# heng-hw/SpaCap3D

Hardware: AMD Instinct MI355X
Metric: scenes/sec (40k pts, 256 proposals) fwd+bwd (higher is better)
Workload: dtype f32; 1 GPU; cfg2: synthetic ScanRefer-shaped scans, 40000 pts x (xyz+1 ch), 256 proposals, 8 scenes/GPU; full training step (SpaCapNet fwd + loss + bwd + grad all-reduce + Adam); global_batch=8, parallelism=dp1, hip_graph=True, fps_prefetch_side_stream=True, prefetch_as_graph=True, reserved_cus_forward=8, geometry_prefetch=True, deferred_weight_gradients=True, params=9290918, allreduce_bytes=35572416

## Files before the change

### include/spacap_hip.h

```cpp
#ifndef SPACAP_HIP_H
#define SPACAP_HIP_H

#include <stddef.h>
#include <stdint.h>

#ifdef __cplusplus
extern "C" {
#endif

#define SPACAP_ABI_VERSION 5

#define SPACAP_OK 0
#define SPACAP_E_INVALID (-1)
#define SPACAP_E_LAUNCH (-2)
#define SPACAP_E_NO_DEVICE (-3)

typedef void *spacap_stream_t;

int spacap_abi_version(void);
const char *spacap_last_error(void);
int spacap_device_count(void);

int spacap_opt_n_threads(int work_size);

// ... 5 lines not shown
int spacap_gather_points_f32(const float *points, const int32_t *idx, int B, int C, int N, int m,
                             float *out, spacap_stream_t stream);
int spacap_gather_points_grad_f32(const float *grad_out, const int32_t *idx, int B, int C, int N,
                                  int m, float *grad_points, spacap_stream_t stream);


int spacap_ball_query_f32(const float *new_xyz, const float *xyz, int B, int N, int m,
                          float radius, int nsample, int32_t *idx, spacap_stream_t stream);

size_t spacap_ball_query_grid_workspace_bytes(int B, int N);
int spacap_ball_query_grid_f32(const float *new_xyz, const float *xyz, int B, int N, int m, float radius, int nsample,
                               int32_t *idx, void *workspace, size_t workspace_bytes, spacap_stream_t stream);


int spacap_group_points_f32(const float *points, const int32_t *idx, int B, int C, int N, int P,
                            int S, float *out, spacap_stream_t stream);
size_t spacap_group_points_grad_workspace_bytes(int B, int C, int N, int P, int S);
int spacap_group_points_grad_f32(const float *grad_out, const int32_t *idx, int B, int C, int N,
                                 int P, int S, float *grad_points, void *workspace,
                                 spacap_stream_t stream);


int spacap_group_max_f32(const float *x, long rows, int S, float *out, uint8_t *arg,
                         spacap_stream_t stream);
int spacap_group_max_grad_f32(const float *grad_out, const uint8_t *arg, long rows, int S,
                              float *grad_in, spacap_stream_t stream);


int spacap_three_nn_f32(const float *unknown, const float *known, int B, int n, int m,
                        float *dist2, int32_t *idx, spacap_stream_t stream);
int spacap_three_nn_weights_f32(const float *unknown, const float *known, int B, int n, int m,
                                float *weight, int32_t *idx, spacap_stream_t stream);
int spacap_gather_xyz_f32(const float *xyz, const int32_t *idx, int B, int N, int m, float *out, spacap_stream_t stream);
int spacap_three_interpolate_f32(const float *points, const int32_t *idx, const float *weight,
                                 int B, int C, int m, int n, float *out, spacap_stream_t stream);
int spacap_three_interpolate_grad_f32(const float *grad_out, const int32_t *idx,
                                      const float *weight, int B, int C, int n, int m,
                                      float *grad_points, spacap_stream_t stream);
int spacap_three_interpolate_grad_pm_f32(const float *grad_pm, const int32_t *idx, const float *weight, int B, int C,
                                         int n, int m, float *grad_points_pm, spacap_stream_t stream);
int spacap_fp_concat_fwd_f32(const float *known, int known_pm, const int32_t *idx, const float *weight, const float *skip, int B,
                             int K1, int K2, int m, int n, float *out, spacap_stream_t stream);
int spacap_fp_concat_bwd_f32(const float *g, int B, int K1, int K2, int n, float *g1, float *g2, spacap_stream_t stream);


int spacap_mha_fwd_f32(const float *q, const float *k, const float *v, long q_sb, long q_sh,
                       long q_sl, long k_sb, long k_sh, long k_sl, long v_sb, long v_sh, long v_sl,
                       const uint8_t *mask, long mask_sb, long mask_sq, const float *bias,
                       long bias_sb, long bias_sh, long bias_sq, int B, int h, int Lq, int Lk,
                       int d_k, float scale, float dropout_p, uint64_t seed, const uint64_t *seed_dev,
                       float *out, float *p_out, float *stats, spacap_stream_t stream);

size_t spacap_mha_bwd_workspace_bytes(int B, int h, int Lq);
int spacap_mha_bwd_f32(const float *q, const float *k, const float *v, long q_sb, long q_sh,
                       long q_sl, long k_sb, long k_sh, long k_sl, long v_sb, long v_sh, long v_sl,
                       const uint8_t *mask, long mask_sb, long mask_sq, const float *bias,
                       long bias_sb, long bias_sh, long bias_sq, int B, int h, int Lq, int Lk,
                       int d_k, float scale, float dropout_p, uint64_t seed, const uint64_t *seed_dev,
                       const float *stats, const float *d_out, const float *d_p, void *workspace,
                       float *dq, float *dk, float *dv, long grad_row_stride, spacap_stream_t stream);

int spacap_mha_bwd_delta_f32(const float *q, const float *k, const float *v, long q_sb, long q_sh,
                             long q_sl, long k_sb, long k_sh, long k_sl, long v_sb, long v_sh, long v_sl,
                             const uint8_t *mask, long mask_sb, long mask_sq, const float *bias,
                             long bias_sb, long bias_sh, long bias_sq, int B, int h, int Lq, int Lk,
                             int d_k, float scale, float dropout_p, uint64_t seed, const uint64_t *seed_dev,
// ... 161 lines not shown
                               float *out, spacap_stream_t stream);

int spacap_scene_aug_doubles(void);
int spacap_scene_sample_augment_f32(const float *const *scene_feat, const int32_t *const *scene_ins,
                                    const uint8_t *const *scene_isobj, const float *const *scene_color,
                                    const int32_t *choices, const double *aug, int B, int P, int C, int augment,
                                    float *pc, int32_t *ins_out, uint8_t *isobj_out, float *color_out,
                                    spacap_stream_t stream);
int spacap_scene_sample_augment_map_f32(const float *const *scene_feat, const int32_t *const *scene_ins,
                                        const uint8_t *const *scene_isobj, const float *const *scene_color,
                                        const int32_t *choices, const double *aug, int B, int P, int C, int augment,
                                        int C_out, const int *dst_off, float *pc, int32_t *ins_out, uint8_t *isobj_out,
                                        float *color_out, spacap_stream_t stream);
int spacap_scene_gather_rows_f32(const float *const *src, const int32_t *choices, int B, int P, int W, float *out,
                                 int out_stride, int out_off, spacap_stream_t stream);
size_t spacap_scene_votes_workspace_bytes(int B, int max_inst);
int spacap_scene_votes_f32(const float *pc, const int32_t *ins, const uint8_t *isobj, int B, int P, int C,
                           int max_inst, void *workspace, float *votes, int64_t *vmask, spacap_stream_t stream);

int spacap_adam_flat_f32(float *p, const float *g, float *m, float *v, long n, float lr, float beta1, float beta2,
                         float eps, float weight_decay, const float *step, float grad_scale,
                         const int64_t *skip_if_nonzero, spacap_stream_t stream);

int spacap_det_npart(void);
int spacap_det_losses_fwd_f32(const float *net, const float *center, const float *agg_xyz, const float *gt_center,
                              const float *box_mask, const int64_t *heading_cls_label, const float *heading_res_label,
                              const int64_t *size_cls_label, const float *size_res_label, const int64_t *sem_cls_label,
                              const float *mean_size, const float *seed_xyz, const float *vote_xyz,
                              const int32_t *seed_inds, const float *vote_label, const int64_t *vote_mask, int B, int K,
                              int M, int NSEED, int N, int NH, int NS, int NC, float near_thr, float far_thr, float w0,
                              float w1, int64_t *obj_label, float *obj_mask, int64_t *assignment, float *dnet_num,
                              float *dcenter_num, float *dvote_num, float *part, float *losses, float *inv_den,
                              spacap_stream_t stream);
int spacap_det_losses_bwd_f32(const float *dnet_num, const float *dcenter_num, const float *dvote_num,
                              const float *grad_losses, const float *inv_den, int B, int K, int NSEED, int NH, int NS,
                              int NC, float *dnet, float *dcenter, float *dvote, spacap_stream_t stream);

long spacap_rel_loss_nparts(int B, int K);
int spacap_rel_loss_fwd_f32(const float *pred, const int64_t *assignment, const int64_t *box_mask_int,
                            const int64_t *obj_label, const int64_t *x_label, const int64_t *y_label,
                            const int64_t *z_label, int B, int K, int M, float *dnum, float *part, float *out,
                            spacap_stream_t stream);
int spacap_rel_loss_bwd_f32(const float *dnum, const float *grad_losses, const float *out, int B, int K, float *dpred,
                            spacap_stream_t stream);

int spacap_sum_slabs_f32(const float *part, int nslab, long n, float *out, spacap_stream_t stream);
int spacap_sum_slabs_batched_f32(const float *const *parts, float *const *outs, const long *n, const int *nslabs, int nseg,
                                 spacap_stream_t stream);

int spacap_linear_dgrad_mask_f32(const float *g, const float *W, const float *y, float scale, long R, int CK, int CP,
                                 float *dx, spacap_stream_t stream);

int spacap_rel_tail_fwd_f32(const float *hid1, const float *W2, const float *b2, const float *W3, const float *b3, long R,
                            float *hid2, float *pred, spacap_stream_t stream);
int spacap_rel_tail_bwd_nparts(long R);
int spacap_rel_tail_bwd_f32(const float *dpred, const float *W3, const float *hid2, long R, float *dz2, float *part,
                            spacap_stream_t stream);

int spacap_conv1x1_wgrad_slabs(int B, int CO, int CI, int N);
int spacap_conv1x1_wgrad_f32(const float *g, const float *x, int B, int CO, int CI, int N, float *part,
                             spacap_stream_t stream);
int spacap_conv1x1_wgrad_slabs_batched(int B, int CO, int CI, int N);
int spacap_conv1x1_wgrad_batched_f32(const float *const *g, const float *const *x, const int *B, const int *CO, const int *CI,
                                     const int *N, const int *nslabs, const int *with_bias, float *const *part, int njobs,
                                     spacap_stream_t stream);

// ... 15 lines not shown

int spacap_gemm_bf3_supported(int K, int N);
int spacap_gemm_bf3_split_w_f32(const float *W, long ldw, int N, int K, int trans, void *Wp, spacap_stream_t stream);
int spacap_gemm_bf3_f32(const float *A, long lda, const void *Wp, const float *bias, long R, int K, int N, int relu, float *out, long ldo,
                        spacap_stream_t stream);
int spacap_gemm_bf3_wgrad_slabs(long R, int N, int K);
int spacap_rel_wide_tail_supported(int C);
int spacap_rel_wide_tail_nparts(long R);
int spacap_rel_wide_tail_bwd_f32(const float *dpred, const float *W3, const float *hid2, long R, int C, int nparts, float *dz2, float *part,
                                 spacap_stream_t stream);
int spacap_rel_wide_l1_supported(int H, int K, int C);
int spacap_rel_wide_transpose_f32(const float *in, float *out, int B, int H, int K, int to_t, spacap_stream_t stream);
int spacap_rel_wide_l1_fwd_f32(const float *Pt, const float *U, const float *b1, int B, int H, int K, int C, float *hid1,
                               spacap_stream_t stream);
int spacap_rel_wide_l1_bwd_f32(const float *dh1, const float *hid1, const float *Pt, const float *U, int B, int H, int K, int C,
                               float *dPt, float *dU, float *db_part, spacap_stream_t stream);

int spacap_linear_rows_supported(long R, int K, int CO);
int spacap_linear_rows_f32(const float *a, const float *W, const float *bias, long R, int K, int CO, int trans_w,
                           float *out, spacap_stream_t stream);

int spacap_l2norm_rows_fwd_f32(const float *x, long rows, int D, float *y, float *inv_norm, spacap_stream_t stream);
int spacap_l2norm_rows_bwd_f32(const float *g, const float *y, const float *inv_norm, long rows, int D, float *dx,
                               spacap_stream_t stream);

int spacap_cap_loss_fwd_f32(const float *logits, const int64_t *target, const uint8_t *good, int B, int W, int V, int tstride,
                            float *logp, float *rowstat, float *out, spacap_stream_t stream);
int spacap_cap_loss_bwd_f32(const float *logp, const int64_t *target, const uint8_t *good, const float *out, const float *gloss,
                            int B, int W, int V, int tstride, float *dlogits, spacap_stream_t stream);

int spacap_proposal_decode_fwd_f32(const float *net, const float *agg_xyz, const float *mean_size, const double *mean_size_f64,
                                   int B, int K, int NH, int NS, int NC, float *nt, float *center, float *heading_res, float *size_res, double *corners,
                                   int64_t *bbox_mask, int64_t *sem_cls, int64_t *size_cls, spacap_stream_t stream);
int spacap_proposal_decode_bwd_f32(const float *g_nt, const float *g_center, const float *g_heading_res, const float *g_size_res,
                                   const float *mean_size, int B, int K, int NH, int NS, int NC, float *d_net, spacap_stream_t stream);

int spacap_loss_tail_fwd_f32(const float *det, const float *cap, const float *rel, const int64_t *obj_label, const float *obj_mask,
                             const int64_t *bbox_mask, int n, float *out, float *loss, spacap_stream_t stream);
int spacap_loss_tail_bwd_f32(const float *g_loss, float *g_det, float *g_cap, float *g_rel, spacap_stream_t stream);

typedef struct {
  int mode;
  long R;
  const float *a1;
  const float *w1;
  const float *bias1;
  int k1;
  float drop_p;
  float eps;
  uint64_t seed;
  const uint64_t *seed_dev;
  const float *res;
  float *x_out;
  const float *ln_a;
  const float *ln_b;
  float *n_out;
  float *stats;
  const float *x_ln;
  const float *g;
  float *part;
  const float *w2;
  const float *bias2;
  float *out2;
  int n2;
  int nparts;
  const float *attn_out;
// ... 8 lines not shown
                      float drop_p, uint64_t seed, const uint64_t *seed_dev, float *hid, float *part, spacap_stream_t stream);
long spacap_tf_ffn_pieces_elems(int dff);
int spacap_tf_ffn_split_f32(const float *const *w1, const float *const *w2, void *const *pieces, int nlayers, int dff,
                            spacap_stream_t stream);
int spacap_tf_ffn_bf3_f32(int mode, const float *x, const void *pieces, const float *bias, const float *y, long R, int dff, float drop_p,
                          uint64_t seed, const uint64_t *seed_dev, float *hid, float *part, spacap_stream_t stream);
int spacap_decode_attn_f32(const float *qkv, float *kcache, float *vcache, long R, int h, int d_k, int T, int t, float scale,
                           float *out, spacap_stream_t stream);
size_t spacap_decode_word_workspace_bytes(long R, int V);
int spacap_decode_word_f32(const float *x, const void *Wp, const float *bias, long R, int V, const float *lut, float scale,
                           const float *pe_row, int64_t *ys, int ys_ld, int t_out, float *x_next, void *workspace,
                           spacap_stream_t stream);
size_t spacap_beam_topw_workspace_bytes(long rows, int V, int W);
int spacap_beam_topw_f32(const float *x, const void *Wp, const float *bias, long rows, int V, int W, float *top_logp, int32_t *top_word,
                         void *workspace, spacap_stream_t stream);
int spacap_decode_attn_beam_f32(const float *qkv, float *kcache, float *vcache, const int8_t *anc, long R, int W, int h, int d_k, int T,
                                int t, float scale, float *out, spacap_stream_t stream);
int spacap_beam_step_f32(const float *top_logp, const int32_t *top_word, long R, int W, int V, int T, int t, int eos, const float *score_in,
                         const int32_t *fin_in, const int32_t *len_in, float *score_out, int32_t *fin_out, int32_t *len_out,
                         const int8_t *anc_old, int8_t *anc_new, int8_t *trace_parent, int32_t *trace_word, const float *lut, float scale,
                         const float *pe_row, float *x_next, spacap_stream_t stream);
int spacap_beam_finish_f32(const float *score, const int32_t *len, const int8_t *trace_parent, const int32_t *trace_word, long R, int W,
                           int n_words, double alpha, int64_t *ys, float *best_score, int64_t *all_tokens, float *all_scores,
                           int32_t *all_len, spacap_stream_t stream);
int spacap_tf_gemm_splits(long R, int K, int N);
int spacap_tf_gemm_f32(const float *a, const float *W, long R, int K, int N, int trans_w, int nsplit, float *out,
                       spacap_stream_t stream);
int spacap_tf_dgrad_mask_f32(const float *g, const float *W, const float *y, float scale, long R, int K, int N, float *out,
                             spacap_stream_t stream);

int spacap_conv1x1_cm_supported(int CI, int CO, long N);
int spacap_conv1x1_cm_f32(int mode, const float *W, const float *in, const float *bias, int B, int CI, int CO, long N,
                          float *out, spacap_stream_t stream);

int spacap_vote_assemble_fwd_f32(const float *net, const float *seed_xyz, const float *seed_feat, int B, int C, int N,
                                 float *vote_xyz, float *vote_feat, spacap_stream_t stream);
int spacap_vote_assemble_bwd_f32(const float *g_xyz, const float *g_feat, int B, int C, int N, float *d_net, float *d_seed,
                                 spacap_stream_t stream);

int spacap_copy_batched(const void *const *src, void *const *dst, const long *nbytes, int njobs, spacap_stream_t stream);

int spacap_stream_delay(int microseconds, spacap_stream_t stream);
int spacap_stream_wait_ge(const int64_t *flag, int64_t value, int timeout_ms, int64_t *err, spacap_stream_t stream);
int spacap_stream_signal(int64_t *flag, const int64_t *value, spacap_stream_t stream);

int spacap_lab_stamp(uint64_t *slot, spacap_stream_t stream);


size_t spacap_points_in_box_workspace_bytes(int B, int N, int K);
int spacap_points_in_box_f32(const float *point_clouds, int B, int N, int C, const double *bbox_corner, int K, void *workspace,
                             size_t workspace_bytes, spacap_stream_t stream);

#define SPACAP_PP_REMOVE_EMPTY 1
#define SPACAP_PP_CLS_NMS 2
#define SPACAP_PP_OLD_TYPE 4
#define SPACAP_PP_GT_F32 8

int spacap_detection_nms_f32(const float *objectness, const int64_t *sem_cls, const float *sem_cls_scores, int NC,
                             const double *bbox_corner, const void *workspace, int B, int N, int K, const double *gt_corner,
                             int M, const int64_t *object_assignment, int flags, int min_points, double nms_iou,
                             float conf_thresh, double min_iou, float *obj_prob, int32_t *count, uint8_t *nonempty,
                             uint8_t *pred_mask, float *conf, uint8_t *valid, double *iou, uint8_t *good,
                             spacap_stream_t stream);


#define SPACAP_AP_EXISTS 0x80

int spacap_detection_match_f32(const double *bbox_corner, const uint8_t *valid, const float *conf, const float *obj_prob,
                               const int64_t *sem_cls, int B, int K, int NC, const double *gt_corner,
                               const int64_t *sem_cls_label, const uint8_t *box_label_mask, int M, const double *thresholds,
                               int T, float *score, uint8_t *flags, int16_t *index, int32_t *npos, spacap_stream_t stream);

int spacap_ap_curve_f64(const uint8_t *flags, int64_t L, const int64_t *count, const int32_t *npos, int NC, int T, double *rec,
// ... 60 lines not shown
```

### spacap3d_amd/_native.py

```python
import ctypes
import os

import torch

_HERE = os.path.dirname(os.path.abspath(__file__))
LIB_PATH = os.path.join(_HERE, "lib", "libspacap_hip.so")
ABI_VERSION = 5

_i = ctypes.c_int
_l = ctypes.c_long
_f = ctypes.c_float
_p = ctypes.c_void_p
_u64 = ctypes.c_uint64

SIGNATURES = {
    "spacap_abi_version": (_i, []),
    "spacap_last_error": (ctypes.c_char_p, []),
    "spacap_device_count": (_i, []),
    "spacap_opt_n_threads": (_i, [_i]),
    "spacap_fps_workspace_bytes": (ctypes.c_size_t, [_i, _i]),
    "spacap_fps_f32": (_i, [_p, _i, _i, _i, _p, _p, _p]),
    "spacap_gather_points_f32": (_i, [_p, _p, _i, _i, _i, _i, _p, _p]),
    "spacap_gather_points_grad_f32": (_i, [_p, _p, _i, _i, _i, _i, _p, _p]),
    "spacap_ball_query_f32": (_i, [_p, _p, _i, _i, _i, _f, _i, _p, _p]),
    "spacap_ball_query_grid_workspace_bytes": (ctypes.c_size_t, [_i, _i]),
    "spacap_ball_query_grid_f32": (_i, [_p, _p, _i, _i, _i, _f, _i, _p, _p, ctypes.c_size_t, _p]),
    "spacap_group_points_f32": (_i, [_p, _p, _i, _i, _i, _i, _i, _p, _p]),
    "spacap_group_points_grad_workspace_bytes": (ctypes.c_size_t, [_i, _i, _i, _i, _i]),
    "spacap_group_points_grad_f32": (_i, [_p, _p, _i, _i, _i, _i, _i, _p, _p, _p]),
    "spacap_group_max_f32": (_i, [_p, _l, _i, _p, _p, _p]),
    "spacap_group_max_grad_f32": (_i, [_p, _p, _l, _i, _p, _p]),
    "spacap_three_nn_f32": (_i, [_p, _p, _i, _i, _i, _p, _p, _p]),
    "spacap_three_nn_weights_f32": (_i, [_p, _p, _i, _i, _i, _p, _p, _p]),
    "spacap_gather_xyz_f32": (_i, [_p, _p, _i, _i, _i, _p, _p]),
    "spacap_three_interpolate_f32": (_i, [_p, _p, _p, _i, _i, _i, _i, _p, _p]),
    "spacap_three_interpolate_grad_f32": (_i, [_p, _p, _p, _i, _i, _i, _i, _p, _p]),
    "spacap_three_interpolate_grad_pm_f32": (_i, [_p, _p, _p, _i, _i, _i, _i, _p, _p]),
    "spacap_bn_workspace_bytes": (ctypes.c_size_t, [_i]),
    "spacap_bn_set_single_launch": (_i, [_i]),
    "spacap_bn_stats_f32": (_i, [_p, _i, _i, _l, _f, _f, _p, _p, _p, _p, _p]),
    "spacap_bn_relu_apply_f32": (_i, [_p, _p, _p, _p, _i, _i, _l, _p, _p]),
    "spacap_bn_relu_train_f32": (_i, [_p, _i, _i, _l, _f, _f, _p, _p, _p, _p, _p, _p, _p, _p]),
    "spacap_bn_relu_max_f32": (_i, [_p, _p, _p, _p, _i, _i, _i, _i, _p, _p, _p]),
    "spacap_bn_relu_bwd_f32": (_i, [_p, _p, _p, _p, _p, _i, _i, _l, _p, _p, _p, _p, _p]),
    "spacap_bn_relu_max_bwd_f32": (_i, [_p, _p, _p, _p, _p, _p, _i, _i, _i, _i, _p, _p, _p, _p, _p]),
    "spacap_relation_feature_fwd_f32": (_i, [_p, _p, _l, _l, _l, _i, _i, _i, _i, _p, _p]),
    "spacap_relation_feature_bwd_f32": (_i, [_p, _p, _p, _l, _l, _l, _i, _i, _i, _i, _p, _p, _p]),
    "spacap_relation_l1_isplit": (_i, []),
    "spacap_relation_l1_supported": (_i, [_i, _i, _i]),
    "spacap_relation_l1_blocks": (_i, [_i, _i, _i]),
    "spacap_relation_l1_fwd_f32": (_i, [_p, _p, _p, _i, _i, _i, _i, _p, _p]),
    "spacap_relation_l1_bwd_f32": (_i, [_p, _p, _p, _p, _i, _i, _i, _i, _p, _p, _p, _p]),
    "spacap_relation_fused_supported": (_i, [_i, _i, _i, _i]),
    "spacap_relation_fused_leave_cus": (_i, [_i]),
    "spacap_relation_fused_zsplit": (_i, [_i, _i, _i]),
    "spacap_relation_fused_nparts": (_i, [_i, _i]),
    "spacap_relation_fused_part_floats": (_i, []),
    "spacap_relation_fused_fwd_f32": (_i, [_p] * 7 + [_i, _i, _p, _p, _p]),
    "spacap_relation_fused_bwd_f32": (_i, [_p] * 7 + [_i, _i, _i, _i, _p, _p, _p, _p]),
    "spacap_caption_prep_fwd_f32": (_i, [_p] * 7 + [_i] * 5 + [_f, _u64, _p] + [_p] * 7 + [_p]),
    "spacap_caption_prep_bwd_f32": (_i, [_p] * 3 + [_i] * 5 + [_f, _u64, _p, _p, _p, _p]),
    "spacap_conv1x1_cm_supported": (_i, [_i, _i, _l]),
    "spacap_conv1x1_cm_f32": (_i, [_i, _p, _p, _p, _i, _i, _i, _l, _p, _p]),
    "spacap_sa_l1_stats_f32": (_i, [_p, _p, _p, _p, _p, _i, _f, _i, _i, _i, _i, _i, _p, _p, _p]),
    "spacap_sa_l1_moments_f32": (_i, [_p, _p, _p, _p, _f, _i, _i, _i, _i, _p, _p, _p]),
    "spacap_sa_l1_moments_finalize_f32": (_i, [_p, _p, _i, _i, _i, _l, _f, _f, _p, _p, _p, _p, _p, _p]),
    "spacap_sa_mid_fwd_l1in_f32": (_i, [_p, _p, _i, _i, _p, _p, _l, _p, _p, _p]),
    "spacap_sa_wgrad_l1in_f32": (_i, [_p, _p, _p, _p, _p, _i, _i, _p, _l, _p, _p]),
    "spacap_sa_dgrad_l1in_f32": (_i, [_p, _p, _p, _p, _p, _p, _i, _i, _p, _i, _i, _i, _p, _p, _p]),
    "spacap_sa_dgrad_wgrad_l1in_slabs": (_i, [_l]),
    "spacap_sa_dgrad_wgrad_l1in_f32": (_i, [_p, _p, _p, _p, _p, _p, _i, _i, _p, _i, _i, _i, _p, _p, _p, _p]),
    "spacap_sa_l1_dw_f32": (_i, [_p, _i, _p, _i, _i, _p, _p]),
    "spacap_vote_assemble_fwd_f32": (_i, [_p, _p, _p, _i, _i, _i, _p, _p, _p]),
    "spacap_vote_assemble_bwd_f32": (_i, [_p, _p, _i, _i, _i, _p, _p, _p]),
    "spacap_copy_batched": (_i, [_p, _p, _p, _i, _p]),
    "spacap_lab_stamp": (_i, [_p, _p]),
    "spacap_points_in_box_workspace_bytes": (ctypes.c_size_t, [_i, _i, _i]),
    "spacap_points_in_box_f32": (_i, [_p, _i, _i, _i, _p, _i, _p, ctypes.c_size_t, _p]),
    "spacap_detection_nms_f32": (_i, [_p, _p, _p, _i, _p, _p, _i, _i, _i, _p, _i, _p, _i, _i, ctypes.c_double, _f,
                                      ctypes.c_double] + [_p] * 8 + [_p]),
    "spacap_detection_match_f32": (_i, [_p] * 5 + [_i, _i, _i] + [_p] * 3 + [_i, _p, _i] + [_p] * 4 + [_p]),
    "spacap_ap_curve_f64": (_i, [_p, ctypes.c_int64, _p, _p, _i, _i] + [_p] * 4 + [_p]),
    "spacap_caption_select_i32": (_i, [_p] * 6 + [_i] * 4 + [_p] + [_i] * 5 + [_p] * 4 + [_p]),
    "spacap_caption_score_f64": (_i, [_p, _p, _i, _p, ctypes.c_int64, _p, _p, ctypes.c_int64, _p, _p, _p, _p,
                                      ctypes.c_double, _p, _p, _p, _p]),
    "spacap_dense_caption_select": (_i, [_p] * 5 + [_i] * 5 + [_p] * 7 + [_p]),
    "spacap_multiview_workspace_bytes": (ctypes.c_size_t, [_i]),
    "spacap_multiview_map_f32": (_i, [_p, _i, _p, _p, _i, _i, _i] + [_f] * 7 + [_p, _p, ctypes.c_size_t, _p, _p]),
    "spacap_multiview_features_f32": (_i, [_p, _i, _p, _p, _i, _i, _i] + [_f] * 7 + [_p, _p, _i, _i, _p, ctypes.c_size_t, _p, _p]),
    "spacap_multiview_vote_i32": (_i, [_p, _i, _p, _p, _i, _i, _i] + [_f] * 7 + [_p, _p, _p, ctypes.c_size_t, _p, _p, _p]),
    "spacap_enet_param_floats": (ctypes.c_size_t, []),
    "spacap_enet_bottleneck_param_floats": (ctypes.c_size_t, [_i, _i, _i]),
    "spacap_enet_workspace_bytes": (ctypes.c_size_t, [_i, _i, _i]),
    "spacap_enet_initial_f32": (_i, [_p, _i, _i, _i, _p, _p, _p]),
    "spacap_enet_bottleneck_f32": (_i, [_p, _i, _i, _i, _i, _i, _i, _i, _p, _p, ctypes.c_size_t, _p, _p]),
    "spacap_enet_encode_f32": (_i, [_p, _i, _i, _i, _p, ctypes.c_size_t, _p, ctypes.c_size_t, _p, _p]),
    "spacap_enet_encode_u8": (_i, [_p, _i, _i, _i] + [_f] * 6 + [_p, ctypes.c_size_t, _p, ctypes.c_size_t, _p, _p]),
    "spacap_stream_delay": (_i, [_i, _p]),
    "spacap_stream_wait_ge": (_i, [_p, _l, _i, _p, _p]),
    "spacap_stream_signal": (_i, [_p, _p, _p]),
    "spacap_sa_nparts": (_i, []),
    "spacap_sa_wgrad_slabs": (_i, [_l, _i, _i, _i]),
    "spacap_sa_mlp_supported": (_i, [_i, _i, _i]),
    "spacap_sa_l1_fwd_f32": (_i, [_p, _p, _p, _p, _p, _p, _i, _f, _i, _i, _i, _i, _i, _p, _p, _p]),
    "spacap_sa_bn_finalize_f32": (_i, [_p, _i, _l, _f, _f, _p, _p, _p, _p, _p, _p]),
    "spacap_sa_mid_fwd_f32": (_i, [_p, _p, _p, _l, _i, _i, _p, _p, _p]),
    "spacap_sa_pool_fwd_f32": (_i, [_p, _p, _l, _i, _i, _p, _p, _p]),
    "spacap_gemm_rows_supported": (_i, [_i, _i]),
# ... 26 lines not shown
    "spacap_rel_wide_l1_bwd_f32": (_i, [_p, _p, _p, _p, _i, _i, _i, _i, _p, _p, _p, _p]),
    "spacap_sa_l3bwd_part_floats": (_l, [_i, _i]),
    "spacap_sa_l3bwd_dw_f32": (_i, [_p, _i, _p, _p, _i, _i, _p, _p, _p]),
    "spacap_sa_wgrad_pool_supported": (_i, [_i, _i, _i]),
    "spacap_sa_wgrad_pool_parts": (_i, [_l, _i, _i, _i]),
    "spacap_sa_wgrad_pool_f32": (_i, [_p, _p, _i, _p, _p, _p, _l, _i, _i, _p, _p]),
    "spacap_sa_bwd_finalize_f32": (_i, [_p, _i, _l, _p, _p, _p, _p, _p]),
    "spacap_sa_dgrad_f32": (_i, [_p, _p, _i, _p, _p, _p, _p, _p, _l, _i, _i, _p, _p, _p]),
    "spacap_sa_dgrad_l1_f32": (_i, [_p] * 10 + [_f] + [_i] * 6 + [_p, _p, _p]),
    "spacap_sa_wgrad_f32": (_i, [_p, _p, _i, _p, _p, _p, _p, _l, _i, _i, _p, _p]),
    "spacap_sa_l1_bwd_f32": (_i, [_p, _p, _p, _p, _p, _p, _p, _p, _i, _f, _i, _i, _i, _i, _i, _p, _p, _i, _p]),
    "spacap_sa_rows_scatter_workspace_bytes": (ctypes.c_size_t, [_i, _i, _l]),
    "spacap_sa_rows_scatter_f32": (_i, [_p, _p, _i, _i, _l, _i, _p, _p, _p]),
    "spacap_sa_rows_index_f32": (_i, [_p, _i, _i, _l, _p, _p]),
    "spacap_sa_rows_gather_f32": (_i, [_p, _i, _i, _l, _i, _p, _p, _p]),
    "spacap_sa_drel_sums_f32": (_i, [_p, _i, _i, _i, _i, _p, _p, _p, _p]),
    "spacap_sa_dw1_assemble_f32": (_i, [_p, _i, _p, _i, _i, _i, _p, _p]),
    "spacap_relu_dropout_fwd_f32": (_i, [_p, _l, _f, _u64, _p, _p, _p]),
    "spacap_relu_dropout_bwd_f32": (_i, [_p, _p, _l, _f, _p, _p]),
    "spacap_dropout_add_fwd_f32": (_i, [_p, _p, _l, _f, _u64, _p, _p, _p]),
    "spacap_dropout_add_bwd_f32": (_i, [_p, _l, _f, _u64, _p, _p, _p]),
    "spacap_scene_aug_doubles": (_i, []),
    "spacap_scene_sample_augment_f32": (_i, [_p, _p, _p, _p, _p, _p, _i, _i, _i, _i, _p, _p, _p, _p, _p]),
    "spacap_scene_sample_augment_map_f32": (_i, [_p, _p, _p, _p, _p, _p, _i, _i, _i, _i, _i, _p, _p, _p, _p, _p, _p]),
    "spacap_scene_gather_rows_f32": (_i, [_p, _p, _i, _i, _i, _p, _i, _i, _p]),
    "spacap_l2norm_rows_fwd_f32": (_i, [_p, _l, _i, _p, _p, _p]),
    "spacap_l2norm_rows_bwd_f32": (_i, [_p, _p, _p, _l, _i, _p, _p]),
    "spacap_cap_loss_fwd_f32": (_i, [_p, _p, _p, _i, _i, _i, _i, _p, _p, _p, _p]),
    "spacap_cap_loss_bwd_f32": (_i, [_p, _p, _p, _p, _p, _i, _i, _i, _i, _p, _p]),
    "spacap_scene_votes_workspace_bytes": (ctypes.c_size_t, [_i, _i]),
    "spacap_scene_votes_f32": (_i, [_p, _p, _p, _i, _i, _i, _i, _p, _p, _p, _p]),
    "spacap_det_npart": (_i, []),
    "spacap_det_losses_fwd_f32": (_i, [_p] * 16 + [_i] * 8 + [_f] * 4 + [_p] * 9 + [_p]),
    "spacap_det_losses_bwd_f32": (_i, [_p] * 5 + [_i] * 6 + [_p] * 3 + [_p]),
    "spacap_rel_loss_nparts": (_l, [_i, _i]),
    "spacap_rel_loss_fwd_f32": (_i, [_p] * 7 + [_i] * 3 + [_p] * 3 + [_p]),
    "spacap_rel_loss_bwd_f32": (_i, [_p] * 3 + [_i] * 2 + [_p, _p]),
    "spacap_sum_slabs_f32": (_i, [_p, _i, _l, _p, _p]),
    "spacap_sum_slabs_batched_f32": (_i, [_p, _p, _p, _p, _i, _p]),
    "spacap_adam_flat_f32": (_i, [_p, _p, _p, _p, _l, _f, _f, _f, _f, _f, _p, _f, _p, _p]),
    "spacap_linear_dgrad_mask_f32": (_i, [_p, _p, _p, _f, _l, _i, _i, _p, _p]),
    "spacap_rel_tail_fwd_f32": (_i, [_p, _p, _p, _p, _p, _l, _p, _p, _p]),
    "spacap_rel_tail_bwd_nparts": (_i, [_l]),
    "spacap_rel_tail_bwd_f32": (_i, [_p, _p, _p, _l, _p, _p, _p]),
    "spacap_conv1x1_wgrad_slabs": (_i, [_i, _i, _i, _i]),
    "spacap_conv1x1_wgrad_f32": (_i, [_p, _p, _i, _i, _i, _i, _p, _p]),
    "spacap_conv1x1_wgrad_slabs_batched": (_i, [_i, _i, _i, _i]),
    "spacap_conv1x1_wgrad_batched_f32": (_i, [_p, _p, _p, _p, _p, _p, _p, _p, _p, _i, _p]),
    "spacap_linear_rows_supported": (_i, [_l, _i, _i]),
    "spacap_linear_rows_f32": (_i, [_p, _p, _p, _l, _i, _i, _i, _p, _p]),
    "spacap_linear_wgrad_slabs": (_i, [_l, _i, _i]),
    "spacap_linear_wgrad_f32": (_i, [_p, _p, _l, _i, _i, _i, _p, _p]),
    "spacap_linear_wgrad_nslab_f32": (_i, [_p, _p, _l, _i, _i, _i, _i, _p, _p]),
    "spacap_linear_wgrad_slabs_batched": (_i, [_l, _i, _i]),
    "spacap_linear_wgrad_batched_f32": (_i, [_p, _p, _p, _p, _p, _p, _p, _p, _i, _p]),
    "spacap_layernorm_fwd_f32": (_i, [_p, _p, _p, _l, _i, _f, _p, _p, _p]),
    "spacap_layernorm_bwd_workspace_bytes": (ctypes.c_size_t, [_l, _i]),
    "spacap_layernorm_bwd_f32": (_i, [_p, _p, _p, _p, _l, _i, _f, _p, _p, _p, _p, _p]),
    "spacap_layernorm_bwd_add_f32": (_i, [_p, _p, _p, _p, _p, _l, _i, _f, _p, _p, _p, _p, _p]),
    "spacap_proposal_decode_fwd_f32": (_i, [_p, _p, _p, _p, _i, _i, _i, _i, _i, _p, _p, _p, _p, _p, _p, _p, _p, _p]),
    "spacap_proposal_decode_bwd_f32": (_i, [_p, _p, _p, _p, _p, _i, _i, _i, _i, _i, _p, _p]),
    "spacap_loss_tail_fwd_f32": (_i, [_p, _p, _p, _p, _p, _p, _i, _p, _p, _p]),
    "spacap_loss_tail_bwd_f32": (_i, [_p, _p, _p, _p, _p]),
    "spacap_tf_rows_f32": (_i, [_p, _p]),
    "spacap_tf_rows_parts": (_i, [_l]),
    "spacap_tf_ffn1_f32": (_i, [_p, _p, _p, _l, _i, _f, _u64, _p, _p, _p]),
    "spacap_tf_ffn_f32": (_i, [_i, _p, _p, _p, _p, _p, _l, _i, _f, _u64, _p, _p, _p, _p]),
    "spacap_tf_ffn_pieces_elems": (_l, [_i]),
    "spacap_tf_ffn_split_f32": (_i, [_p, _p, _p, _i, _i, _p]),
    "spacap_tf_ffn_bf3_f32": (_i, [_i, _p, _p, _p, _p, _l, _i, _f, _u64, _p, _p, _p, _p]),
    "spacap_decode_attn_f32": (_i, [_p, _p, _p, _l, _i, _i, _i, _i, _f, _p, _p]),
    "spacap_decode_word_workspace_bytes": (ctypes.c_size_t, [_l, _i]),
    "spacap_decode_word_f32": (_i, [_p, _p, _p, _l, _i, _p, _f, _p, _p, _i, _i, _p, _p, _p]),
    "spacap_beam_topw_workspace_bytes": (ctypes.c_size_t, [_l, _i, _i]),
    "spacap_beam_topw_f32": (_i, [_p, _p, _p, _l, _i, _i, _p, _p, _p, _p]),
    "spacap_decode_attn_beam_f32": (_i, [_p, _p, _p, _p, _l, _i, _i, _i, _i, _i, _f, _p, _p]),
    "spacap_beam_step_f32": (_i, [_p, _p, _l, _i, _i, _i, _i, _i] + [_p] * 6 + [_p] * 4 + [_p, _f, _p, _p, _p]),
    "spacap_beam_finish_f32": (_i, [_p, _p, _p, _p, _l, _i, _i, ctypes.c_double, _p, _p, _p, _p, _p, _p]),
    "spacap_tf_gemm_splits": (_i, [_l, _i, _i]),
    "spacap_tf_gemm_f32": (_i, [_p, _p, _l, _i, _i, _i, _i, _p, _p]),
    "spacap_tf_dgrad_mask_f32": (_i, [_p, _p, _p, _f, _l, _i, _i, _p, _p]),
    "spacap_mha_fwd_f32": (_i, [_p, _p, _p] + [_l] * 9 + [_p, _l, _l, _p, _l, _l, _l]
                           + [_i] * 5 + [_f, _f, _u64, _p, _p, _p, _p, _p]),
    "spacap_mha_bwd_workspace_bytes": (ctypes.c_size_t, [_i, _i, _i]),
    "spacap_mha_bwd_delta_f32": (_i, [_p, _p, _p] + [_l] * 9 + [_p, _l, _l, _p, _l, _l, _l]
                                 + [_i] * 5 + [_f, _f, _u64, _p, _p, _p, _p, _p, _p, _p, _l, _p]),
    "spacap_mha_bwd_f32": (_i, [_p, _p, _p] + [_l] * 9 + [_p, _l, _l, _p, _l, _l, _l]
                           + [_i] * 5 + [_f, _f, _u64, _p, _p, _p, _p, _p, _p, _p, _p, _l, _p]),
}


class TfRowsArgs(ctypes.Structure):
    _fields_ = [("mode", _i), ("R", _l), ("a1", _p), ("w1", _p), ("bias1", _p), ("k1", _i), ("drop_p", _f), ("eps", _f),
                ("seed", _u64), ("seed_dev", _p), ("res", _p), ("x_out", _p), ("ln_a", _p), ("ln_b", _p), ("n_out", _p),
                ("stats", _p), ("x_ln", _p), ("g", _p), ("part", _p), ("w2", _p), ("bias2", _p), ("out2", _p), ("n2", _i), ("nparts", _i), ("attn_out", _p), ("delta_out", _p), ("lq", _i)]


def _load():
    if not os.path.exists(LIB_PATH):
        raise ImportError(
            f"{LIB_PATH} not found: the HIP extension is not built. Run "
            "`python -c 'import __graft_entry__ as g; g.build()'` (or `make -C spacap3d_amd/csrc`). "
            "spacap3d_amd has no CPU or PyTorch fallback for its native operators.")
    lib = ctypes.CDLL(LIB_PATH)
    for name, (res, args) in SIGNATURES.items():
        fn = getattr(lib, name)
        fn.restype = res
        fn.argtypes = args
    got = lib.spacap_abi_version()
    if got != ABI_VERSION:
        raise ImportError(f"libspacap_hip.so ABI {got} != expected {ABI_VERSION}: rebuild the extension")
    return lib


lib = _load()


def check(rc: int, what: str) -> None:
    if rc != 0:
        msg = lib.spacap_last_error().decode("utf-8", "replace")
        raise RuntimeError(f"{what} failed (code {rc}): {msg}")


_DEFERRED = None


class deferred_slab_sums:

# ... 151 lines not shown

def conv1x1_wgrad_partials(g, x, B, CO, CI, N, deferrable=False, with_bias=False):
    import torch
    with torch.cuda.device(g.device):
        if deferrable and _DEFERRED is not None:
            nb = int(lib.spacap_conv1x1_wgrad_slabs_batched(B, CO, CI, N))
            part = torch.empty(nb, CO * CI + (((CO + 3) // 4) * 4 if with_bias else 0), dtype=torch.float32, device=g.device)
            _DEFERRED.conv_jobs.append((g, x, (B, CO, CI, N), part, bool(with_bias)))
            return part
        nslab = int(lib.spacap_conv1x1_wgrad_slabs(B, CO, CI, N))
        part = torch.empty(nslab, CO * CI, dtype=torch.float32, device=g.device)
        check(lib.spacap_conv1x1_wgrad_f32(g.data_ptr(), x.data_ptr(), B, CO, CI, N, part.data_ptr(),
                                           torch.cuda.current_stream(g.device).cuda_stream), "spacap_conv1x1_wgrad_f32")
    return part


def copy_batched(dsts, srcs):
    import torch
    ok = len(dsts) == len(srcs) and len(dsts) > 0 and all(
        d.is_cuda and s.is_cuda and d.device == s.device and d.dtype == s.dtype and d.shape == s.shape and d.is_contiguous()
        and s.is_contiguous() for d, s in zip(dsts, srcs))
    if not ok:
        if dsts:
            torch._foreach_copy_(list(dsts), list(srcs), non_blocking=True)
        return
    n = len(dsts)
    PA, LA = ctypes.c_void_p * n, ctypes.c_long * n
    src = PA(*[s.data_ptr() for s in srcs])
    dst = PA(*[d.data_ptr() for d in dsts])
    nb = LA(*[d.numel() * d.element_size() for d in dsts])
    dev = dsts[0].device
    with torch.cuda.device(dev):
        check(lib.spacap_copy_batched(src, dst, nb, n, torch.cuda.current_stream(dev).cuda_stream), "spacap_copy_batched")
```

### spacap3d_amd/attention.py

```python
import math

import torch
from torch.autograd import Function

from ._native import check, lib, sum_slabs


def _strides3(t):
    assert t.stride(3) == 1, "last (d_k) dimension must be contiguous"
    return t.stride(0), t.stride(1), t.stride(2)


def _prep_mask(mask, B, Lq, Lk):
    if mask is None:
        return None, 0, 0
    for ent in _MASK_CACHE:
        if ent[0] is mask and ent[1] == (mask._version, B, Lq, Lk):
            return ent[2]
    res = _prep_mask_uncached(mask, B, Lq, Lk)
    _MASK_CACHE.insert(0, (mask, (mask._version, B, Lq, Lk), res))
    del _MASK_CACHE[4:]
    return res


_MASK_CACHE = []


def _prep_mask_uncached(mask, B, Lq, Lk):
    m = mask
    if m.dim() == 4:
        assert m.size(1) == 1, "per-head masks are not used by the reference"
        m = m[:, 0]
    assert m.dim() == 3 and m.size(-1) == Lk and m.size(1) in (1, Lq)
    if m.dtype == torch.uint8 and m.size(0) == B and m.is_contiguous():
        return m, m.stride(0), (0 if m.size(1) == 1 else m.stride(1))
    m = (m != 0).to(torch.uint8)
    if m.size(0) != B:
        m = m.expand(B, -1, -1)
    m = m.contiguous()
    return m, m.stride(0), (0 if m.size(1) == 1 else m.stride(1))


_RNG_STATE = {}
_CALL_COUNTER = [None]


def rng_state(device):
    device = torch.device(device)
    if device.type == "cuda" and device.index is None:
        device = torch.device("cuda", torch.cuda.current_device())
    st = _RNG_STATE.get(device)
    if st is None:
        st = torch.zeros(1, dtype=torch.int64, device=device)
        _RNG_STATE[device] = st
    return st


def advance_rng(device):
    rng_state(device).add_(1)


def _next_seed():
# ... 321 lines not shown
```

### spacap3d_amd/backend.py

```python
import contextlib

_current = None


class HipBackend:

    name = "hip"

    def __init__(self):
        from . import ext
        from . import attention as _att
        self._ext = ext
        for n in ("gather_points", "gather_points_grad", "furthest_point_sampling", "three_nn",
                  "three_interpolate", "three_interpolate_grad", "ball_query", "group_points",
                  "group_points_grad", "group_max", "group_max_grad", "three_interpolate_grad_pm"):
            setattr(self, n, getattr(ext, n))
        self.attention = _att.attention
        self.self_attention_packed = _att.self_attention_packed
        self.layer_norm = _att.layer_norm
        self.layer_norm_residual = _att.layer_norm_residual
        self.relation_feature = _att.relation_feature
        self.relation_layer1 = _att.relation_layer1
        from . import fused_bn as _fbn
        self.bn_relu_train = _fbn.bn_relu_train
        self.bn_relu_eval = _fbn.bn_relu_eval
        from . import fused_losses as _fl
        self.detection_losses = _fl.detection_losses
        self.relation_losses = _fl.relation_losses
        self.caption_head_loss = _fl.caption_head_loss
        self.loss_tail = _fl.loss_tail
        self.proposal_decode = _fl.proposal_decode
        self.l2norm_rows = _fl.l2norm_rows
        self.vote_assemble = _fl.vote_assemble
        from . import fused_dropout as _fd
        self.relu_dropout = _fd.relu_dropout
        self.dropout_add = _fd.dropout_add
        from . import linear as _lin
        self.linear = _lin.linear
        self.ffn_tail = _lin.ffn_tail
        self.conv1x1 = _lin.conv1x1
        self.relation_tail = _lin.relation_tail
        self.relation_head = _lin.relation_head
        self.vocab_projection = _lin.vocab_projection
        from . import caption_prep as _cp
        self.caption_prep = _cp.caption_prep
        from . import tf_layer as _tf
        self.tf_stack = _tf
        from . import caption_decode as _cd
        self.caption_decode = _cd
        from . import sa_mlp as _sa
        self.sa_mlp_train = _sa.sa_mlp_train
        self.sa_mlp_eval = _sa.sa_mlp_eval


def ops():
    global _current
    if _current is None:
        _current = HipBackend()
    return _current


def set_backend(b):
    global _current
    prev = _current
    _current = b
    return prev


@contextlib.contextmanager
def use_backend(b):
    prev = set_backend(b)
    try:
        yield b
# ... 3 lines not shown
```

### spacap3d_amd/csrc/conv1x1.hip

```cpp
#include <stdlib.h>

#include "common.hpp"
#include "launch.hpp"
#include "mfma.hpp"

namespace {

using namespace spacap::mfma;

constexpr int TM = 64, TN = 64, KC = 32, LDN = TN + 4, LDW = TM + 4;

template <bool TRANS_A>
__global__ __launch_bounds__(256) void conv1x1_cm_kernel(const float *__restrict__ W, int lda, const float *__restrict__ in,
                                                         const float *__restrict__ bias, int M, int K, int N,
                                                         float *__restrict__ out) {
  __shared__ __attribute__((aligned(16))) float s_in[2][KC * LDN];
  __shared__ __attribute__((aligned(16))) float s_w[TRANS_A ? 2 * KC * LDW : 4];
  const int tid = threadIdx.x, lane = tid & 63, w = tid >> 6, l15 = lane & 15, lg = lane >> 4;
  const int n0 = blockIdx.x * TN, m0 = blockIdx.y * TM, b = blockIdx.z;
  const float *inb = in + (size_t)b * K * N;
  const int sr = tid >> 4, sc = (tid & 15) * 4;
  f32x4 pin[2], pw[2];
  auto request = [&](int k0) {
#pragma unroll
    for (int e = 0; e < 2; ++e) {
      const int k = k0 + sr + 16 * e;
      const f32x4 v = ld4(inb + (size_t)min(k, K - 1) * N + n0 + sc);
      pin[e] = k < K ? v : f32x4{0.f, 0.f, 0.f, 0.f};
      if (TRANS_A) {
        const float *p = W + (size_t)min(k, K - 1) * lda;
        f32x4 t;
        if (m0 + sc + 3 < M && (lda & 3) == 0) {
          t = ld4(p + m0 + sc);
        } else {
#pragma unroll
          for (int u = 0; u < 4; ++u) t[u] = p[min(m0 + sc + u, M - 1)];
        }
#pragma unroll
        for (int u = 0; u < 4; ++u) t[u] = (k < K && m0 + sc + u < M) ? t[u] : 0.f;
        pw[e] = t;
      }
    }
  };
  auto store = [&](int buf) {
#pragma unroll
    for (int e = 0; e < 2; ++e) {
      st4(&s_in[buf][(sr + 16 * e) * LDN + sc], pin[e]);
      if (TRANS_A) st4(&s_w[buf * KC * LDW + (sr + 16 * e) * LDW + sc], pw[e]);
// ... 6 lines not shown
  const int nchunks = (K + KC - 1) / KC;
  request(0);
  for (int c = 0; c < nchunks; ++c) {
    const int buf = c & 1, k0 = c * KC;
    store(buf);
    f32x4 a0, a1;
    if (!TRANS_A) {
      const float *p = W + (size_t)mrow * lda + k0 + 8 * lg;
      if (k0 + KC <= K && (lda & 3) == 0) {
        a0 = ld4(p), a1 = ld4(p + 4);
      } else {
#pragma unroll
        for (int u = 0; u < 4; ++u) {
          a0[u] = k0 + 8 * lg + u < K ? p[u] : 0.f;
          a1[u] = k0 + 8 * lg + 4 + u < K ? p[4 + u] : 0.f;
        }
      }
    }
    if (c + 1 < nchunks) request(k0 + KC);
    __syncthreads();
    const float *si = &s_in[buf][(8 * lg) * LDN + l15];
    if (TRANS_A) {
      const float *sw = &s_w[buf * KC * LDW + (8 * lg) * LDW + 16 * w + l15];
#pragma unroll
      for (int u = 0; u < 4; ++u) a0[u] = sw[u * LDW], a1[u] = sw[(4 + u) * LDW];
    }
#pragma unroll
    for (int s = 0; s < 8; ++s) {
      const float av = s < 4 ? a0[s] : a1[s - 4];
#pragma unroll
      for (int t = 0; t < 4; ++t) acc[t] = MFMA16(av, si[s * LDN + 16 * t], acc[t]);
    }
  }
#pragma unroll
  for (int u = 0; u < 4; ++u) {
    const int m = m0 + 16 * w + 4 * lg + u;
    if (m < M) {
      const float bv = bias ? bias[m] : 0.f;
      float *o = out + ((size_t)b * M + m) * N + n0 + l15;
#pragma unroll
      for (int t = 0; t < 4; ++t) o[16 * t] = acc[t][u] + bv;
    }
  }
}


constexpr int BLD = TN + 8;
constexpr int BIMG = KC * BLD;


template <bool TRANS_A>
__global__ __launch_bounds__(256) void conv1x1_cm_bf3_kernel(const float *__restrict__ W, int lda, const float *__restrict__ in,
                                                             const float *__restrict__ bias, int M, int K, int N,
                                                             float *__restrict__ out) {
  __shared__ __attribute__((aligned(16))) __bf16 s_b[2][3 * BIMG];
  __shared__ __attribute__((aligned(16))) __bf16 s_a[TRANS_A ? 2 * 3 * BIMG : 8];
  const int tid = threadIdx.x, lane = tid & 63, w = tid >> 6, l15 = lane & 15, lg = lane >> 4;
  const int n0 = blockIdx.x * TN, m0 = blockIdx.y * TM, b = blockIdx.z;
  const float *inb = in + (size_t)b * K * N;
  const int sr = tid >> 4, sc = (tid & 15) * 4;
  f32x4 pin[2], pw[2];
  auto request = [&](int k0) {
#pragma unroll
    for (int e = 0; e < 2; ++e) {
      const int k = k0 + sr + 16 * e;
      const f32x4 v = ld4(inb + (size_t)min(k, K - 1) * N + n0 + sc);
      pin[e] = k < K ? v : f32x4{0.f, 0.f, 0.f, 0.f};
      if (TRANS_A) {
        const float *p = W + (size_t)min(k, K - 1) * lda;
        f32x4 t;
        if (m0 + sc + 3 < M && (lda & 3) == 0) {
          t = ld4(p + m0 + sc);
        } else {
#pragma unroll
          for (int u = 0; u < 4; ++u) t[u] = p[min(m0 + sc + u, M - 1)];
        }
#pragma unroll
        for (int u = 0; u < 4; ++u) t[u] = (k < K && m0 + sc + u < M) ? t[u] : 0.f;
        pw[e] = t;
      }
    }
  };
  auto store = [&](int buf) {
#pragma unroll
    for (int e = 0; e < 2; ++e) {
      const int o = (sr + 16 * e) * BLD + sc;
      bf16x4 p0, p1, p2;
// ... 29 lines not shown
    }
  };
  request(0);
  wrequest(0);
  for (int c = 0; c < nchunks; ++c) {
    const int buf = c & 1, k0 = c * KC;
    store(buf);
    bf16x8 a[3];
    if (!TRANS_A) {
      bf16x4 l0, l1, l2, h0, h1, h2;
      split4(na0, l0, l1, l2);
      split4(na1, h0, h1, h2);
      a[0] = bf16x8{l0[0], l0[1], l0[2], l0[3], h0[0], h0[1], h0[2], h0[3]};
      a[1] = bf16x8{l1[0], l1[1], l1[2], l1[3], h1[0], h1[1], h1[2], h1[3]};
      a[2] = bf16x8{l2[0], l2[1], l2[2], l2[3], h2[0], h2[1], h2[2], h2[3]};
    }
    if (c + 1 < nchunks) {
      request(k0 + KC);
      wrequest(k0 + KC);
    }
    __syncthreads();
    if (TRANS_A) {
#pragma unroll
      for (int q = 0; q < 3; ++q) a[q] = tr_frag<BLD>(&s_a[buf * 3 * BIMG + q * BIMG], 16 * w, lane);
    }
#pragma unroll
    for (int t = 0; t < 4; ++t) {
      bf16x8 bq[3];
#pragma unroll
      for (int q = 0; q < 3; ++q) bq[q] = tr_frag<BLD>(&s_b[buf][q * BIMG], 16 * t, lane);
#pragma unroll
      for (int q = 0; q < 6; ++q) acc[t] = MFMA_B(a[PA[q]], bq[PB[q]], acc[t]);
    }
  }
#pragma unroll
  for (int u = 0; u < 4; ++u) {
    const int m = m0 + 16 * w + 4 * lg + u;
    if (m < M) {
      const float bv = bias ? bias[m] : 0.f;
      float *o = out + ((size_t)b * M + m) * N + n0 + l15;
#pragma unroll
      for (int t = 0; t < 4; ++t) o[16 * t] = acc[t][u] + bv;
    }
  }
}

}

extern "C" int spacap_conv1x1_cm_supported(int CI, int CO, long N) { return CI >= 1 && CO >= 1 && N >= 64 && N % 64 == 0; }

extern "C" int spacap_conv1x1_cm_f32(int mode, const float *W, const float *in, const float *bias, int B, int CI, int CO, long N,
                                     float *out, spacap_stream_t stream) {
  const char *what = "spacap_conv1x1_cm_f32";
  SPACAP_REQUIRE((mode == 0 || mode == 1 || mode == 2) && B >= 0 && spacap_conv1x1_cm_supported(CI, CO, N) && N <= 2147483647L && B <= 65535,
                 "%s: (mode=%d, B=%d, CI=%d, CO=%d, N=%ld) unsupported", what, mode, B, CI, CO, N);
  if (B == 0) return SPACAP_OK;
  SPACAP_REQUIRE(W && in && out && spacap::aligned16(in, out),
                 "%s: null or unaligned pointer", what);
  const bool f32fwd = mode == 2;
  if (f32fwd) mode = 0;
  const int M = mode == 0 ? CO : CI, K = mode == 0 ? CI : CO;
  const dim3 grid((unsigned)(N / TN), (unsigned)((M + TM - 1) / TM), (unsigned)B);
  hipStream_t s = spacap::as_stream(stream);
  if (mode == 0 && !f32fwd && !spacap::sa_f32_mfma_only())
    hipLaunchKernelGGL(conv1x1_cm_bf3_kernel<false>, grid, dim3(256), 0, s, W, CI, in, bias, M, K, (int)N, out);
  else if (mode == 0) hipLaunchKernelGGL(conv1x1_cm_kernel<false>, grid, dim3(256), 0, s, W, CI, in, bias, M, K, (int)N, out);
  else hipLaunchKernelGGL(conv1x1_cm_kernel<true>, grid, dim3(256), 0, s, W, CI, in, (const float *)nullptr, M, K, (int)N, out);
  SPACAP_CHECK_LAUNCH(what);
  return SPACAP_OK;
}
```

### spacap3d_amd/csrc/elementwise.hip

```cpp
#include "common.hpp"
#include "dropout.hpp"
#include "mfma.hpp"

namespace {

using namespace spacap;
using spacap::mfma::f32x4;

template <int MODE>
__global__ __launch_bounds__(256) void drop_kernel(const float *__restrict__ x, const float *__restrict__ res, long n,
                                                   unsigned thresh, float scale, unsigned long long seed,
                                                   const unsigned long long *__restrict__ seed_dev, float *__restrict__ out) {
  const DropSeed sd = make_seed(seed, seed_dev);
  const long n4 = n >> 2;
  for (long i = (long)blockIdx.x * 256 + threadIdx.x; i < n4; i += (long)gridDim.x * 256) {
    f32x4 v = *reinterpret_cast<const f32x4 *>(x + 4 * i);
    f32x4 r = {0.f, 0.f, 0.f, 0.f};
    if (MODE == 1) r = *reinterpret_cast<const f32x4 *>(res + 4 * i);
#pragma unroll
    for (int u = 0; u < 4; ++u) {
      const bool keep = thresh == 0u || hash32((unsigned long long)(4 * i + u), sd) >= thresh;
      float a = MODE == 0 ? fmaxf(v[u], 0.f) : v[u];
      a = keep ? a * scale : 0.f;
      v[u] = MODE == 1 ? r[u] + a : a;
// ... 300 lines not shown
  if (J.vec) {
    for (long o = beg + 16 * threadIdx.x; o < end; o += 16 * 256)
      *reinterpret_cast<f32x4 *>(J.dst + o) = *reinterpret_cast<const f32x4 *>(J.src + o);
  } else {
    for (long o = beg + threadIdx.x; o < end; o += 256) J.dst[o] = J.src[o];
  }
}
}
extern "C" int spacap_copy_batched(const void *const *src, void *const *dst, const long *nbytes, int njobs, spacap_stream_t stream) {
  const char *what = "spacap_copy_batched";
  SPACAP_REQUIRE(njobs >= 0 && (njobs == 0 || (src && dst && nbytes)), "%s: bad arguments", what);
  hipStream_t s = spacap::as_stream(stream);
  int i = 0;
  while (i < njobs) {
    CopyTable T;
    T.njobs = 0, T.pad = 0;
    long blocks = 0;
    for (; i < njobs && T.njobs < CPJ_MAX; ++i) {
      SPACAP_REQUIRE(nbytes[i] >= 0 && (nbytes[i] == 0 || (src[i] && dst[i])), "%s: job %d: null pointer or negative size", what, i);
      if (nbytes[i] == 0) continue;
      CopyJob &J = T.job[T.njobs++];
      J.src = static_cast<const char *>(src[i]), J.dst = static_cast<char *>(dst[i]), J.nbytes = nbytes[i], J.block0 = (int)blocks;
      J.vec = ((reinterpret_cast<uintptr_t>(src[i]) | reinterpret_cast<uintptr_t>(dst[i]) | (uintptr_t)nbytes[i]) & 15) == 0;
      blocks += (nbytes[i] + CPJ_BLOCK_BYTES - 1) / CPJ_BLOCK_BYTES;
      SPACAP_REQUIRE(blocks < 2147483647L, "%s: too many blocks", what);
    }
    if (T.njobs) hipLaunchKernelGGL(copy_batched_kernel, dim3((unsigned)blocks), dim3(256), 0, s, T);
  }
  SPACAP_CHECK_LAUNCH(what);
  return SPACAP_OK;
}

namespace {
__global__ void delay_kernel(unsigned long long ticks) {
  const unsigned long long t0 = wall_clock64();
  while (wall_clock64() - t0 < ticks) __builtin_amdgcn_s_sleep(8);
}
}
extern "C" int spacap_stream_delay(int microseconds, spacap_stream_t stream) {
  SPACAP_REQUIRE(microseconds >= 0 && microseconds <= 100000, "spacap_stream_delay: %d us out of range", microseconds);
  if (microseconds == 0) return SPACAP_OK;
  hipLaunchKernelGGL(delay_kernel, dim3(1), dim3(1), 0, spacap::as_stream(stream), (unsigned long long)microseconds * 100ull);
  SPACAP_CHECK_LAUNCH("spacap_stream_delay");
  return SPACAP_OK;
}

namespace {
__global__ void wait_ge_kernel(const long long *flag, long long value, unsigned long long ticks, unsigned long long *err) {
  const unsigned long long t0 = wall_clock64();
  while (__hip_atomic_load(flag, __ATOMIC_ACQUIRE, __HIP_MEMORY_SCOPE_AGENT) < value) {
    if (wall_clock64() - t0 > ticks) {
      atomicCAS(err, 0ull, (unsigned long long)(value > 0 ? value : 1));
      __threadfence_system();
      return;
    }
    __builtin_amdgcn_s_sleep(16);
  }
}
__global__ void signal_set_kernel(long long *flag, const long long *value) {
  __hip_atomic_store(flag, *value, __ATOMIC_RELEASE, __HIP_MEMORY_SCOPE_AGENT);
}
}
extern "C" int spacap_stream_wait_ge(const int64_t *flag, int64_t value, int timeout_ms, int64_t *err, spacap_stream_t stream) {
  SPACAP_REQUIRE(flag && err && timeout_ms >= 1 && timeout_ms <= 600000, "spacap_stream_wait_ge: bad arguments");
  hipLaunchKernelGGL(wait_ge_kernel, dim3(1), dim3(1), 0, spacap::as_stream(stream), reinterpret_cast<const long long *>(flag),
                     (long long)value, (unsigned long long)timeout_ms * 100000ull, reinterpret_cast<unsigned long long *>(err));
// ... 21 lines not shown
```

### spacap3d_amd/csrc/interpolate.hip

```cpp
#include <math.h>

#include "common.hpp"

#pragma clang fp contract(off)

namespace {

template <bool WEIGHTS>
__global__ __launch_bounds__(64) void three_nn_kernel(const float *__restrict__ unknown_all,
                                                      const float *__restrict__ known_all, int n, int m,
                                                      float *__restrict__ dist2_all,
                                                      int32_t *__restrict__ idx_all) {
  constexpr int KT = 512;
  __shared__ float s_k[KT * 3];
  const int b = blockIdx.y;
  const int j = blockIdx.x * 64 + threadIdx.x;
  const float *__restrict__ known = known_all + (size_t)b * m * 3;
  const int jj = j < n ? j : n - 1;
  const float *__restrict__ u = unknown_all + ((size_t)b * n + jj) * 3;
  const float ux = u[0], uy = u[1], uz = u[2];
  float best1 = INFINITY, best2 = INFINITY, best3 = INFINITY;
  int besti1 = 0, besti2 = 0, besti3 = 0;
  for (int k0 = 0; k0 < m; k0 += KT) {
    const int kn = min(KT, m - k0);
// ... 7 lines not shown
      const int kk = k0 + k;
      const bool l1 = d < best1, l2 = d < best2, l3 = d < best3;
      best3 = l2 ? best2 : (l3 ? d : best3);
      besti3 = l2 ? besti2 : (l3 ? kk : besti3);
      best2 = l1 ? best1 : (l2 ? d : best2);
      besti2 = l1 ? besti1 : (l2 ? kk : besti2);
      best1 = l1 ? d : best1;
      besti1 = l1 ? kk : besti1;
    }
  }
  if (j < n) {
    float *__restrict__ dd = dist2_all + ((size_t)b * n + j) * 3;
    int32_t *__restrict__ ii = idx_all + ((size_t)b * n + j) * 3;
    if (WEIGHTS) {
      const float r1 = 1.0f / (sqrtf(best1) + 1e-8f), r2 = 1.0f / (sqrtf(best2) + 1e-8f), r3 = 1.0f / (sqrtf(best3) + 1e-8f);
      const float norm = (r1 + r3) + r2;
      dd[0] = r1 / norm; dd[1] = r2 / norm; dd[2] = r3 / norm;
    } else {
      dd[0] = best1; dd[1] = best2; dd[2] = best3;
    }
    ii[0] = besti1; ii[1] = besti2; ii[2] = besti3;
  }
}

__global__ __launch_bounds__(256) void gather_xyz_kernel(const float *__restrict__ xyz, const int32_t *__restrict__ idx, int N, int m,
                                                         long total, float *__restrict__ out) {
  const long i = (long)blockIdx.x * 256 + threadIdx.x;
  if (i >= total) return;
  const long b = i / m;
  const float *p = xyz + ((size_t)b * N + idx[i]) * 3;
  out[i * 3 + 0] = p[0], out[i * 3 + 1] = p[1], out[i * 3 + 2] = p[2];
}

constexpr int CHUNK = 8;

__global__ __launch_bounds__(256) void three_interpolate_kernel(const float *__restrict__ points,
                                                                const int32_t *__restrict__ idx,
                                                                const float *__restrict__ weight, int C,
                                                                int m, int n, float *__restrict__ out) {
  const int b = blockIdx.z;
  const int j = blockIdx.x * 256 + threadIdx.x;
  if (j >= n) return;
  const size_t r = ((size_t)b * n + j) * 3;
  const float w1 = weight[r + 0], w2 = weight[r + 1], w3 = weight[r + 2];
  const int i1 = idx[r + 0], i2 = idx[r + 1], i3 = idx[r + 2];
  const int c0 = blockIdx.y * CHUNK, c1 = min(c0 + CHUNK, C);
  const float *__restrict__ p = points + ((size_t)b * C + c0) * m;
  float *__restrict__ o = out + ((size_t)b * C + c0) * n + j;
  for (int c = c0; c < c1; ++c, p += m, o += n) *o = p[i1] * w1 + p[i2] * w2 + p[i3] * w3;
}

__global__ __launch_bounds__(256) void three_interpolate_grad_kernel(const float *__restrict__ grad_out,
                                                                     const int32_t *__restrict__ idx,
                                                                     const float *__restrict__ weight,
                                                                     int C, int n, int m,
                                                                     float *__restrict__ grad_points) {
  const int b = blockIdx.z;
  const int j = blockIdx.x * 256 + threadIdx.x;
  if (j >= n) return;
  const size_t r = ((size_t)b * n + j) * 3;
  const float w1 = weight[r + 0], w2 = weight[r + 1], w3 = weight[r + 2];
  const int i1 = idx[r + 0], i2 = idx[r + 1], i3 = idx[r + 2];
  const int c0 = blockIdx.y * CHUNK, c1 = min(c0 + CHUNK, C);
  float *__restrict__ g = grad_points + ((size_t)b * C + c0) * m;
  const float *__restrict__ go = grad_out + ((size_t)b * C + c0) * n + j;
  for (int c = c0; c < c1; ++c, g += m, go += n) {
// ... 155 lines not shown
  SPACAP_REQUIRE(B >= 0 && n >= 0 && m >= 0, "%s: bad sizes", what);
  if (B == 0 || n == 0) return SPACAP_OK;
  SPACAP_REQUIRE(unknown && out && idx && (known || m == 0), "%s: null pointer", what);
  SPACAP_REQUIRE(B <= 65535, "%s: B out of range", what);
  dim3 grid((n + 63) / 64, B);
  if (weights) hipLaunchKernelGGL(three_nn_kernel<true>, grid, dim3(64), 0, spacap::as_stream(stream), unknown, known, n, m, out, idx);
  else hipLaunchKernelGGL(three_nn_kernel<false>, grid, dim3(64), 0, spacap::as_stream(stream), unknown, known, n, m, out, idx);
  SPACAP_CHECK_LAUNCH(what);
  return SPACAP_OK;
}

extern "C" int spacap_three_nn_f32(const float *unknown, const float *known, int B, int n, int m,
                                   float *dist2, int32_t *idx, spacap_stream_t stream) {
  return three_nn_launch("spacap_three_nn_f32", false, unknown, known, B, n, m, dist2, idx, stream);
}

extern "C" int spacap_three_nn_weights_f32(const float *unknown, const float *known, int B, int n, int m,
                                           float *weight, int32_t *idx, spacap_stream_t stream) {
  return three_nn_launch("spacap_three_nn_weights_f32", true, unknown, known, B, n, m, weight, idx, stream);
}

extern "C" int spacap_gather_xyz_f32(const float *xyz, const int32_t *idx, int B, int N, int m, float *out, spacap_stream_t stream) {
  const char *what = "spacap_gather_xyz_f32";
  SPACAP_REQUIRE(B >= 0 && N >= 0 && m >= 0, "%s: bad sizes", what);
  const long total = (long)B * m;
  if (total == 0) return SPACAP_OK;
  SPACAP_REQUIRE(xyz && idx && out && N > 0, "%s: null pointer", what);
  hipLaunchKernelGGL(gather_xyz_kernel, dim3((unsigned)((total + 255) / 256)), dim3(256), 0, spacap::as_stream(stream), xyz, idx, N, m,
                     total, out);
  SPACAP_CHECK_LAUNCH(what);
  return SPACAP_OK;
}

extern "C" int spacap_three_interpolate_f32(const float *points, const int32_t *idx, const float *weight,
                                            int B, int C, int m, int n, float *out,
                                            spacap_stream_t stream) {
  SPACAP_REQUIRE(B >= 0 && C >= 0 && m >= 0 && n >= 0, "spacap_three_interpolate_f32: bad sizes");
  if (B == 0 || C == 0 || n == 0) return SPACAP_OK;
  SPACAP_REQUIRE(points && idx && weight && out, "spacap_three_interpolate_f32: null pointer");
  SPACAP_REQUIRE(B <= 65535, "spacap_three_interpolate_f32: B out of range");
  dim3 grid((n + 255) / 256, (C + CHUNK - 1) / CHUNK, B);
  hipLaunchKernelGGL(three_interpolate_kernel, grid, dim3(256), 0, spacap::as_stream(stream), points, idx,
                     weight, C, m, n, out);
  SPACAP_CHECK_LAUNCH("spacap_three_interpolate_f32");
  return SPACAP_OK;
}

extern "C" int spacap_three_interpolate_grad_f32(const float *grad_out, const int32_t *idx,
                                                 const float *weight, int B, int C, int n, int m,
                                                 float *grad_points, spacap_stream_t stream) {
  SPACAP_REQUIRE(B >= 0 && C >= 0 && m >= 0 && n >= 0, "spacap_three_interpolate_grad_f32: bad sizes");
  if (B == 0 || C == 0 || m == 0) return SPACAP_OK;
  SPACAP_REQUIRE(grad_points, "spacap_three_interpolate_grad_f32: null pointer");
  hipStream_t s = spacap::as_stream(stream);
  if (n == 0) {
    SPACAP_CHECK_HIP(hipMemsetAsync(grad_points, 0, sizeof(float) * (size_t)B * C * m, s),
                     "spacap_three_interpolate_grad_f32(memset)");
    return SPACAP_OK;
  }
  SPACAP_REQUIRE(grad_out && idx && weight, "spacap_three_interpolate_grad_f32: null pointer");
  SPACAP_REQUIRE(B <= 65535, "spacap_three_interpolate_grad_f32: B out of range");
  hipLaunchKernelGGL(three_interpolate_grad_gather_kernel, dim3((m + IG_JT - 1) / IG_JT, B), dim3(256), 0, s, grad_out, idx,
                     weight, C, n, m, grad_points);
  SPACAP_CHECK_LAUNCH("spacap_three_interpolate_grad_f32");
  return SPACAP_OK;
}
// ... 97 lines not shown
```

### spacap3d_amd/csrc/losses.hip

```cpp
#include <math.h>

#include "common.hpp"

namespace {

constexpr int MAXM = 256;
constexpr int NPARTL = 12;

struct DetArgs {
  const float *net;
  const float *center;
  const float *agg_xyz;
  const float *gt_center;
  const float *box_mask;
  const int64_t *heading_cls_label, *size_cls_label, *sem_cls_label;
  const float *heading_res_label;
  const float *size_res_label;
  const float *mean_size;
  int B, K, M, CH, NH, NS, NC;
  float near_thr, far_thr, w0, w1, heading_scale;
  int64_t *obj_label, *assignment;
  float *obj_mask;
  float *dnet;
  float *dcenter;
// ... 166 lines not shown
      }
      num_sr += sr / 3.0f * obj;
    } else if (l4 == 2) {
      num_sc += ce_grad(row + o_ss, A.NS, s_sl[i1], obj, g + o_ss) * obj;
    } else {
      num_sem += ce_grad(row + o_sem, A.NC, s_se[i1], obj, g + o_sem) * obj;
    }
  }
  const float v[NPARTL] = {0.f, num_obj, num_c1, num_c2, num_hc, num_hr, num_sc, num_sr, num_sem, n_obj, n_mask, n_box};
#pragma unroll
  for (int i = 1; i < NPARTL; ++i) {
    const float w = spacap::wave_sum(v[i]);
    if ((tid & 63) == 0) s_red[tid >> 6][i] = w;
  }
  __syncthreads();
  if (STAGED) {
    float *dst = A.dnet + (size_t)b * K * CH;
    if ((((size_t)K * CH) & 3) == 0 && (reinterpret_cast<uintptr_t>(dst) & 15) == 0 && (reinterpret_cast<uintptr_t>(s_net) & 15) == 0) {
      for (int i = tid; i < K * CH / 4; i += DET_THREADS)
        reinterpret_cast<float4 *>(dst)[i] = reinterpret_cast<const float4 *>(s_net)[i];
    } else {
      for (int i = tid; i < K * CH; i += DET_THREADS) dst[i] = s_net[i];
    }
  }
  if (tid >= 1 && tid < NPARTL) {
    float a = 0.f;
#pragma unroll
    for (int w = 0; w < 16; ++w) a += s_red[w][tid];
    A.part[(size_t)b * NPARTL + tid] = a;
  }
}

__global__ __launch_bounds__(256) void det_vote_kernel(const float *__restrict__ seed_xyz, const float *__restrict__ vote_xyz,
                                                       const int32_t *__restrict__ seed_inds,
                                                       const float *__restrict__ vote_label,
                                                       const int64_t *__restrict__ vote_mask, int NS, int N,
                                                       float *__restrict__ dvote, float *__restrict__ part) {
  __shared__ float s_red[4];
  const int b = blockIdx.x;
  float num = 0.f, cnt = 0.f;
  for (int s = threadIdx.x; s < NS; s += 256) {
    const size_t bs = (size_t)b * NS + s;
    const int p = seed_inds[bs];
    const float m = (float)vote_mask[(size_t)b * N + p];
    const float *vl = vote_label + ((size_t)b * N + p) * 9, *sx = seed_xyz + bs * 3, *vx = vote_xyz + bs * 3;
    float best = INFINITY;
    int bi = 0;
    for (int v = 0; v < 3; ++v) {
      const float d = (fabsf(vx[0] - (vl[3 * v] + sx[0])) + fabsf(vx[1] - (vl[3 * v + 1] + sx[1]))) +
                      fabsf(vx[2] - (vl[3 * v + 2] + sx[2]));
      if (d < best) best = d, bi = v;
    }
    num += best * m;
    cnt += m;
    for (int d = 0; d < 3; ++d) {
      const float e = vx[d] - (vl[3 * bi + d] + sx[d]);
      dvote[bs * 3 + d] = (e > 0.f ? 1.f : (e < 0.f ? -1.f : 0.f)) * m;
    }
  }
  const float a = block_sum(num, s_red), c = block_sum(cnt, s_red);
  if (threadIdx.x == 0) part[(size_t)b * 2] = a, part[(size_t)b * 2 + 1] = c;
}

__global__ void det_finalize_kernel(const float *__restrict__ part, const float *__restrict__ vpart, int B,
                                    float *__restrict__ losses, float *__restrict__ inv_den) {
  if (threadIdx.x != 0) return;
  float s[NPARTL] = {0.f}, vn = 0.f, vc = 0.f;
  for (int b = 0; b < B; ++b) {
    for (int i = 1; i < NPARTL; ++i) s[i] += part[(size_t)b * NPARTL + i];
    vn += vpart[2 * b], vc += vpart[2 * b + 1];
  }
  const float d_vote = vc + 1e-6f, d_mask = s[10] + 1e-6f, d_obj = s[9] + 1e-6f, d_box = s[11] + 1e-6f;
  losses[0] = vn / d_vote;
  losses[1] = s[1] / d_mask;
  losses[2] = s[2] / d_obj + s[3] / d_box;
  losses[3] = s[4] / d_obj;
// ... 107 lines not shown
extern "C" long spacap_rel_loss_nparts(int B, int K) { return (long)B * (((long)K * K + REL_THREADS - 1) / REL_THREADS); }

extern "C" int spacap_rel_loss_fwd_f32(const float *pred, const int64_t *assignment, const int64_t *box_mask_int,
                                       const int64_t *obj_label, const int64_t *x_label, const int64_t *y_label,
                                       const int64_t *z_label, int B, int K, int M, float *dnum, float *part, float *out,
                                       spacap_stream_t stream) {
  const char *what = "spacap_rel_loss_fwd_f32";
  SPACAP_REQUIRE(B >= 1 && K >= 1 && M >= 1 && B <= 65535, "%s: bad sizes", what);
  SPACAP_REQUIRE(pred && assignment && box_mask_int && obj_label && x_label && y_label && z_label && dnum && part && out,
                 "%s: null pointer", what);
  hipStream_t s = spacap::as_stream(stream);
  const unsigned gx = (unsigned)(((long)K * K + REL_THREADS - 1) / REL_THREADS);
  hipLaunchKernelGGL(rel_loss_kernel, dim3(gx, B), dim3(REL_THREADS), 0, s, pred, assignment, box_mask_int, obj_label, x_label,
                     y_label, z_label, K, M, dnum, part);
  hipLaunchKernelGGL(rel_finalize_kernel, dim3(1), dim3(256), 0, s, part, (int)(gx * B), out);
  SPACAP_CHECK_LAUNCH(what);
  return SPACAP_OK;
}

extern "C" int spacap_rel_loss_bwd_f32(const float *dnum, const float *grad_losses, const float *out, int B, int K,
                                       float *dpred, spacap_stream_t stream) {
  const char *what = "spacap_rel_loss_bwd_f32";
  SPACAP_REQUIRE(dnum && grad_losses && out && dpred && B >= 1 && K >= 1, "%s: bad arguments", what);
  const long n = (long)B * K * K * 9;
  long g = (n + 255) / 256;
  if (g > 4096) g = 4096;
  hipLaunchKernelGGL(rel_scale_kernel, dim3((unsigned)g), dim3(256), 0, spacap::as_stream(stream), dnum, grad_losses, out, n, dpred);
  SPACAP_CHECK_LAUNCH(what);
  return SPACAP_OK;
}

extern "C" int spacap_det_npart(void) { return NPARTL; }

extern "C" int spacap_det_losses_fwd_f32(
    const float *net, const float *center, const float *agg_xyz, const float *gt_center, const float *box_mask,
    const int64_t *heading_cls_label, const float *heading_res_label, const int64_t *size_cls_label,
    const float *size_res_label, const int64_t *sem_cls_label, const float *mean_size, const float *seed_xyz,
    const float *vote_xyz, const int32_t *seed_inds, const float *vote_label, const int64_t *vote_mask, int B, int K,
    int M, int NSEED, int N, int NH, int NS, int NC, float near_thr, float far_thr, float w0, float w1,
    int64_t *obj_label, float *obj_mask, int64_t *assignment, float *dnet_num, float *dcenter_num, float *dvote_num,
    float *part, float *losses, float *inv_den, spacap_stream_t stream) {
  const char *what = "spacap_det_losses_fwd_f32";
  SPACAP_REQUIRE(B >= 1 && K >= 1 && M >= 1 && M <= MAXM && NSEED >= 1 && NH >= 1 && NS >= 1 && NC >= 1 && B <= 65535,
                 "%s: bad sizes", what);
  SPACAP_REQUIRE(net && center && agg_xyz && gt_center && box_mask && heading_cls_label && heading_res_label &&
                     size_cls_label && size_res_label && sem_cls_label && mean_size && seed_xyz && vote_xyz && seed_inds &&
                     vote_label && vote_mask && obj_label && obj_mask && assignment && dnet_num && dcenter_num &&
                     dvote_num && part && losses && inv_den, "%s: null pointer", what);
  DetArgs A;
  A.net = net; A.center = center; A.agg_xyz = agg_xyz; A.gt_center = gt_center; A.box_mask = box_mask;
  A.heading_cls_label = heading_cls_label; A.size_cls_label = size_cls_label; A.sem_cls_label = sem_cls_label;
  A.heading_res_label = heading_res_label; A.size_res_label = size_res_label; A.mean_size = mean_size;
  A.B = B; A.K = K; A.M = M; A.NH = NH; A.NS = NS; A.NC = NC; A.CH = 5 + 2 * NH + 4 * NS + NC;
  A.near_thr = near_thr; A.far_thr = far_thr; A.w0 = w0; A.w1 = w1; A.heading_scale = (float)(M_PI / NH);
  A.obj_label = obj_label; A.assignment = assignment; A.obj_mask = obj_mask; A.dnet = dnet_num; A.dcenter = dcenter_num;
  A.part = part;
  hipStream_t s = spacap::as_stream(stream);
  const size_t lds = sizeof(float) * (12 * (size_t)M + 6 * (size_t)K + 3 * (size_t)NS + 4);
  SPACAP_REQUIRE(lds <= 60000, "%s: K=%d too large", what, K);
  const size_t lds_staged = lds + sizeof(float) * (size_t)K * A.CH;
  if (lds_staged <= 150 * 1024) {
    static unsigned long long lds_ok = 0;
    SPACAP_CHECK_HIP(spacap::allow_dynamic_lds(reinterpret_cast<const void *>(&det_proposal_kernel<true>), 150 * 1024, lds_ok), what);
    hipLaunchKernelGGL(det_proposal_kernel<true>, dim3(B), dim3(DET_THREADS), lds_staged, s, A);
  } else {
    hipLaunchKernelGGL(det_proposal_kernel<false>, dim3(B), dim3(DET_THREADS), lds, s, A);
  }
  float *vpart = part + (size_t)B * NPARTL;
  hipLaunchKernelGGL(det_vote_kernel, dim3(B), dim3(256), 0, s, seed_xyz, vote_xyz, seed_inds, vote_label, vote_mask, NSEED, N,
                     dvote_num, vpart);
  hipLaunchKernelGGL(det_finalize_kernel, dim3(1), dim3(64), 0, s, part, vpart, B, losses, inv_den);
  SPACAP_CHECK_LAUNCH(what);
  return SPACAP_OK;
}

extern "C" int spacap_det_losses_bwd_f32(const float *dnet_num, const float *dcenter_num, const float *dvote_num,
                                         const float *grad_losses, const float *inv_den, int B, int K, int NSEED, int NH,
                                         int NS, int NC, float *dnet, float *dcenter, float *dvote,
                                         spacap_stream_t stream) {
  const char *what = "spacap_det_losses_bwd_f32";
  SPACAP_REQUIRE(dnet_num && dcenter_num && dvote_num && grad_losses && inv_den && dnet && dcenter && dvote && B >= 1 && K >= 1,
                 "%s: bad arguments", what);
  const int CH = 5 + 2 * NH + 4 * NS + NC;
  const long rows = (long)B * K, nvote = (long)B * NSEED * 3, total = rows * CH + rows * 3 + nvote;
  long g = (total + 255) / 256;
  if (g > 2048) g = 2048;
  hipLaunchKernelGGL(det_scale_kernel, dim3((unsigned)g), dim3(256), 0, spacap::as_stream(stream), dnet_num, dcenter_num,
                     dvote_num, grad_losses, inv_den, rows, CH, NH, NS, nvote, dnet, dcenter, dvote);
  SPACAP_CHECK_LAUNCH(what);
  return SPACAP_OK;
}

namespace {
constexpr int CAP_T = 256;
__global__ __launch_bounds__(CAP_T) void cap_rows_kernel(const float *__restrict__ logits, const int64_t *__restrict__ target,
                                                        const uint8_t *__restrict__ good, int W, int V, int tstride,
                                                        float *__restrict__ logp, float *__restrict__ rowstat) {
  __shared__ float s_f[CAP_T / 64];
  __shared__ int s_i[CAP_T / 64];
  const int r = blockIdx.x, tid = threadIdx.x, lane = tid & 63, wv = tid >> 6;
  const float *x = logits + (size_t)r * V;
  float m = -INFINITY;
  int am = 0;
  for (int v = tid; v < V; v += CAP_T) {
    const float a = x[v];
    if (a > m) m = a, am = v;
// ... 146 lines not shown
```

### spacap3d_amd/csrc/proposal_decode.hip

```cpp
#include <math.h>

#include "common.hpp"

namespace {

__global__ __launch_bounds__(256) void proposal_decode_fwd_kernel(const float *__restrict__ net, const float *__restrict__ agg_xyz,
                                                                  const float *__restrict__ msa, const double *__restrict__ msa64,
                                                                  int K, int NH, int NS, int NC,
                                                                  float *__restrict__ nt, float *__restrict__ center,
                                                                  float *__restrict__ hres, float *__restrict__ sres,
                                                                  double *__restrict__ corners, int64_t *__restrict__ bbox_mask,
                                                                  int64_t *__restrict__ sem_cls, int64_t *__restrict__ size_cls) {
  extern __shared__ float s_x[];
  const int b = blockIdx.y, k0 = blockIdx.x * 64, tid = threadIdx.x;
  const int CH = 5 + 2 * NH + 4 * NS + NC, LD = CH + 1, nk = min(64, K - k0);
  float *s_c = s_x + 64 * LD;
  for (int i = tid; i < CH * 64; i += 256) {
    const int c = i >> 6, kk = i & 63;
    if (kk < nk) s_x[kk * LD + c] = net[((size_t)b * CH + c) * K + k0 + kk];
  }
  __syncthreads();
  for (int i = tid; i < nk * CH; i += 256) nt[((size_t)b * K + k0) * CH + i] = s_x[(i / CH) * LD + i % CH];
  if (tid < nk) {
    const float *row = s_x + tid * LD;
    const size_t p = (size_t)b * K + k0 + tid;
    bbox_mask[p] = row[1] > row[0] ? 1 : 0;
#pragma unroll
    for (int d = 0; d < 3; ++d) {
      const float c = agg_xyz[p * 3 + d] + row[2 + d];
      center[p * 3 + d] = c;
      s_c[tid * 4 + d] = c;
    }
    const float *ss = row + 5 + 2 * NH;
    int sc = 0;
    float best = ss[0];
    for (int j = 1; j < NS; ++j)
      if (ss[j] > best) best = ss[j], sc = j;
    size_cls[p] = sc;
    s_c[tid * 4 + 3] = __int_as_float(sc);
    const float *cl = ss + 4 * NS;
    int am = 0;
    best = cl[0];
    for (int j = 1; j < NC; ++j)
      if (cl[j] > best) best = cl[j], am = j;
    sem_cls[p] = am;
  }
  __syncthreads();
  const float hs = (float)(M_PI / (double)NH);
  const size_t p0 = (size_t)b * K + k0;
  for (int i = tid; i < nk * NH; i += 256) hres[p0 * NH + i] = s_x[(i / NH) * LD + 5 + NH + i % NH] * hs;
  const int S3 = 3 * NS, so = 5 + 2 * NH + NS;
  for (int i = tid; i < nk * S3; i += 256) sres[p0 * S3 + i] = s_x[(i / S3) * LD + so + i % S3] * msa[i % S3];
  for (int i = tid; i < nk * 24; i += 256) {
    const int kk = i / 24, e = i % 24, c = e / 3, d = e % 3;
    const int sc = __float_as_int(s_c[kk * 4 + 3]);
    const float mine = s_x[kk * LD + so + 3 * sc + d] * msa[3 * sc + d];
    const double half = ((msa64 ? msa64[3 * sc + d] : (double)msa[3 * sc + d]) + (double)mine) / 2.0;
    const double sgn = d == 0 ? ((c & 3) < 2 ? 1.0 : -1.0) : d == 1 ? (((c & 3) == 0 || (c & 3) == 3) ? 1.0 : -1.0) : (c < 4 ? 1.0 : -1.0);
    corners[p0 * 24 + i] = (double)s_c[kk * 4 + d] + sgn * half;
  }
}

__global__ __launch_bounds__(256) void proposal_decode_bwd_kernel(const float *__restrict__ g_nt, const float *__restrict__ g_center,
                                                                 const float *__restrict__ g_hres, const float *__restrict__ g_sres,
                                                                 const float *__restrict__ msa, int K, int NH, int NS, int NC,
                                                                 float *__restrict__ d_net) {
  extern __shared__ float s_x[];
  const int b = blockIdx.y, k0 = blockIdx.x * 64;
  const int CH = 5 + 2 * NH + 4 * NS + NC, LD = CH + 1, nk = min(64, K - k0);
  const float hs = (float)(M_PI / (double)NH);
  const int s0 = 5 + 2 * NH + NS;
  for (int i = threadIdx.x; i < nk * CH; i += 256) {
    const int kk = i / CH, c = i % CH;
    const size_t p = (size_t)b * K + k0 + kk;
    float v = g_nt ? g_nt[p * CH + c] : 0.f;
    if (g_center && c >= 2 && c < 5) v += g_center[p * 3 + (c - 2)];
    if (g_hres && c >= 5 + NH && c < 5 + 2 * NH) v += g_hres[p * NH + (c - 5 - NH)] * hs;
    if (g_sres && c >= s0 && c < s0 + 3 * NS) v += g_sres[p * NS * 3 + (c - s0)] * msa[c - s0];
    s_x[kk * LD + c] = v;
  }
  __syncthreads();
  for (int i = threadIdx.x; i < CH * 64; i += 256) {
    const int c = i >> 6, kk = i & 63;
    if (kk < nk) d_net[((size_t)b * CH + c) * K + k0 + kk] = s_x[kk * LD + c];
  }
}

}

extern "C" int spacap_proposal_decode_fwd_f32(const float *net, const float *agg_xyz, const float *mean_size,
                                              const double *mean_size_f64, int B, int K, int NH, int NS, int NC, float *nt, float *center, float *heading_res, float *size_res,
                                              double *corners, int64_t *bbox_mask, int64_t *sem_cls, int64_t *size_cls,
                                              spacap_stream_t stream) {
  const char *what = "spacap_proposal_decode_fwd_f32";
  SPACAP_REQUIRE(B >= 0 && K >= 1 && NH >= 1 && NS >= 1 && NC >= 1, "%s: bad sizes", what);
  if (B == 0) return SPACAP_OK;
  SPACAP_REQUIRE(net && agg_xyz && mean_size && nt && center && heading_res && size_res && corners && bbox_mask && sem_cls && size_cls,
                 "%s: null pointer", what);
  const int CH = 5 + 2 * NH + 4 * NS + NC;
  SPACAP_REQUIRE((size_t)64 * (CH + 1) * sizeof(float) <= 64 * 1024, "%s: too many channels (%d)", what, CH);
  hipLaunchKernelGGL(proposal_decode_fwd_kernel, dim3((K + 63) / 64, B), dim3(256), (size_t)(64 * (CH + 1) + 256) * sizeof(float),
                     spacap::as_stream(stream), net, agg_xyz, mean_size,
                     mean_size_f64, K, NH, NS, NC, nt, center, heading_res, size_res, corners, bbox_mask, sem_cls, size_cls);
  SPACAP_CHECK_LAUNCH(what);
  return SPACAP_OK;
}

extern "C" int spacap_proposal_decode_bwd_f32(const float *g_nt, const float *g_center, const float *g_heading_res,
                                              const float *g_size_res, const float *mean_size, int B, int K, int NH, int NS, int NC,
                                              float *d_net, spacap_stream_t stream) {
  const char *what = "spacap_proposal_decode_bwd_f32";
  SPACAP_REQUIRE(B >= 0 && K >= 1 && NH >= 1 && NS >= 1 && NC >= 1, "%s: bad sizes", what);
  if (B == 0) return SPACAP_OK;
  SPACAP_REQUIRE(mean_size && d_net, "%s: null pointer", what);
  const int CH = 5 + 2 * NH + 4 * NS + NC;
  SPACAP_REQUIRE((size_t)64 * (CH + 1) * sizeof(float) <= 64 * 1024, "%s: too many channels (%d)", what, CH);
  hipLaunchKernelGGL(proposal_decode_bwd_kernel, dim3((K + 63) / 64, B), dim3(256), (size_t)64 * (CH + 1) * sizeof(float),
                     spacap::as_stream(stream), g_nt, g_center,
                     g_heading_res, g_size_res, mean_size, K, NH, NS, NC, d_net);
  SPACAP_CHECK_LAUNCH(what);
  return SPACAP_OK;
}

namespace {
__global__ __launch_bounds__(256) void vote_assemble_fwd_kernel(const float *__restrict__ net, const float *__restrict__ seed_xyz,
                                                                const float *__restrict__ seed_feat, int C, int N,
                                                                float *__restrict__ vote_xyz, float *__restrict__ vote_feat) {
  __shared__ float s[32][33];
  const int b = blockIdx.z, c0 = blockIdx.y * 32, n0 = blockIdx.x * 32, tx = threadIdx.x & 31, ty = threadIdx.x >> 5;
  const float *nb = net + (size_t)b * (3 + C) * N;
#pragma unroll
  for (int i = 0; i < 4; ++i) {
    const int c = c0 + ty + 8 * i, n = n0 + tx;
    s[ty + 8 * i][tx] = (c < C && n < N) ? seed_feat[((size_t)b * C + c) * N + n] + nb[(size_t)(3 + c) * N + n] : 0.f;
  }
  __syncthreads();
#pragma unroll
  for (int i = 0; i < 4; ++i) {
// ... 61 lines not shown
```

### spacap3d_amd/detector.py

```python
import math

import numpy as np
import torch
import torch.nn as nn
import torch.nn.functional as F

from .pointnet2_modules import PointnetFPModule, PointnetSAModuleVotes
from .layout import ChannelMajorOf, point_major_of


SA_NPOINTS = (2048, 1024, 512, 256)


def sampling_pyramid(xyz, npoints=SA_NPOINTS):
    from . import pointnet2_utils as pu
    inds_all = []
    cur = xyz
    for n in npoints:
        inds = pu.furthest_point_sample(cur, n)
        inds_all.append(inds)
        cur = pu.gather_operation(cur.transpose(1, 2).contiguous(), inds).transpose(1, 2).contiguous()
    return inds_all


# ... 16 lines not shown
        inds = pu.furthest_point_sample(cur, n)
        new_xyz = _centres(cur, inds)
        idx_all.append(pu.ball_query(r, ns, cur, new_xyz))
        inds_all.append(inds)
        xyzs.append(new_xyz)
        cur = new_xyz
    fp1 = PointnetFPModule.neighbours(xyzs[3], xyzs[4])
    fp2 = PointnetFPModule.neighbours(xyzs[2], xyzs[3])
    out = tuple(inds_all) + tuple(idx_all) + (fp1[0], fp1[1], fp2[0], fp2[1])
    if xyz.is_cuda:
        from .sa_mlp import rows_index
        out = out + tuple(rows_index(idx_all[l], xyzs[l].shape[1]) for l in (1, 2, 3))
        out = out + tuple(x.contiguous() for x in xyzs[1:])
    return out


class Pointnet2Backbone(nn.Module):

    def __init__(self, input_feature_dim=0):
        super().__init__()
        self.input_feature_dim = input_feature_dim
        self.sa1 = PointnetSAModuleVotes(npoint=2048, radius=0.2, nsample=64,
                                         mlp=[input_feature_dim, 64, 64, 128], use_xyz=True, normalize_xyz=True)
        self.sa2 = PointnetSAModuleVotes(npoint=1024, radius=0.4, nsample=32,
                                         mlp=[128, 128, 128, 256], use_xyz=True, normalize_xyz=True)
        self.sa3 = PointnetSAModuleVotes(npoint=512, radius=0.8, nsample=16,
                                         mlp=[256, 128, 128, 256], use_xyz=True, normalize_xyz=True)
        self.sa4 = PointnetSAModuleVotes(npoint=256, radius=1.2, nsample=16,
                                         mlp=[256, 128, 128, 256], use_xyz=True, normalize_xyz=True)
        self.fp1 = PointnetFPModule(mlp=[256 + 256, 256, 256])
        self.fp2 = PointnetFPModule(mlp=[256 + 256, 256, 256])

    @staticmethod
    def _break_up_pc(pc):
        xyz = pc[..., :3].contiguous()
        if pc.size(-1) <= 3:
            return xyz, None
        if pc.is_cuda and pc.size(-1) > 4 and pc.is_contiguous() and not pc.requires_grad:
            from .layout import ChannelMajorOf
            return xyz, ChannelMajorOf.wrap(pc[..., 3:])
        return xyz, pc[..., 3:].transpose(1, 2).contiguous()

    overlap_sampling = True
    _side_streams = {}

    def _sample_ahead(self, xyz):
        from . import pointnet2_utils as pu
        dev = xyz.device
        side = Pointnet2Backbone._side_streams.get(dev)
        if side is None:
            side = Pointnet2Backbone._side_streams[dev] = torch.cuda.Stream(device=dev)
        side.wait_stream(torch.cuda.current_stream(dev))
        levels = []
        from ._native import check, lib
        check(lib.spacap_sa_reserve_cus(min(64, int(xyz.shape[0]))), "spacap_sa_reserve_cus")
        with torch.cuda.stream(side), torch.no_grad():
            cur = xyz
            for n in SA_NPOINTS:
                inds = pu.furthest_point_sample(cur, n)
                cur = _centres(cur, inds)
                ev = torch.cuda.Event()
                ev.record(side)
                levels.append((inds, cur, ev))
        return levels

    def forward(self, data_dict):
        xyz, features = self._break_up_pc(data_dict["point_clouds"])
        pyr = tuple(data_dict.get("fps_pyramid") or ())
        pyr = pyr + (None,) * (19 - len(pyr))
        if pyr[0] is None and xyz.is_cuda and self.overlap_sampling and not xyz.requires_grad:
            levels = self._sample_ahead(xyz)
            data_dict["_sampling_levels"] = levels
            cur = torch.cuda.current_stream(xyz.device)
            pyr = list(pyr)
            for l, (inds, new_xyz, ev) in enumerate(levels):
                pyr[l], pyr[15 + l] = inds, new_xyz
            waits = [ev for _, _, ev in levels]
        else:
            waits = [None] * 4
            cur = None
        if waits[0] is not None:
            cur.wait_event(waits[0])
        xyz, features, fps_inds = self.sa1(xyz, features, pyr[0], pyr[4], None, pyr[15])
        data_dict["sa1_inds"], data_dict["sa1_xyz"], data_dict["sa1_features"] = fps_inds, xyz, features
        if waits[1] is not None:
            cur.wait_event(waits[1])
        xyz, features, fps_inds = self.sa2(xyz, features, pyr[1], pyr[5], pyr[12], pyr[16])
        data_dict["sa2_inds"], data_dict["sa2_xyz"], data_dict["sa2_features"] = fps_inds, xyz, features
        if waits[2] is not None:
            cur.wait_event(waits[2])
        xyz, features, fps_inds = self.sa3(xyz, features, pyr[2], pyr[6], pyr[13], pyr[17])
        data_dict["sa3_xyz"], data_dict["sa3_features"] = xyz, features
        if waits[3] is not None:
            cur.wait_event(waits[3])
        xyz, features, fps_inds = self.sa4(xyz, features, pyr[3], pyr[7], pyr[14], pyr[18])
        data_dict["sa4_xyz"], data_dict["sa4_features"] = xyz, features
        features = self.fp1(data_dict["sa3_xyz"], data_dict["sa4_xyz"], data_dict["sa3_features"],
                            data_dict["sa4_features"], nn=(pyr[8], pyr[9]) if pyr[8] is not None else None)
        features = self.fp2(data_dict["sa2_xyz"], data_dict["sa3_xyz"], data_dict["sa2_features"], features,
                            nn=(pyr[10], pyr[11]) if pyr[10] is not None else None)
# ... 177 lines not shown
```

### spacap3d_amd/engine.py

```python
import os

import torch

from . import synthetic as S
from .detector import geometry_pyramid, sampling_pyramid
from .distributed import FlatGradBucket, broadcast_parameters, used_parameters
from .loss_helper import get_scene_cap_loss, start_detection_losses


_STREAMS = {}


def _role_stream(device, role):
    device = torch.device(device)
    key = (device.type, device.index if device.index is not None else torch.cuda.current_device())
    if key not in _STREAMS:
        dev = torch.device("cuda", key[1])
        _STREAMS[key] = {r: torch.cuda.Stream(device=dev) for r in ("side", "capture", "comm", "wgrad", "relation")}
    return _STREAMS[key][role]


class Trainer:
    def __init__(self, model: torch.nn.Module, mean_size_arr, lr: float = 1e-3, weight_decay: float = 1e-5,
                 use_relation: bool = True, split_optimizer: bool = False,
                 adam_eps: float = 1e-8):
        self.model = model
        self.mean_size_arr = mean_size_arr
        self.use_relation = use_relation
        self.lr, self.weight_decay, self.adam_eps = lr, weight_decay, adam_eps
        self.bucket = None
        self.optimizer = None
        self.side_stream = None
        self.prefetch_geometry = True
        self.prefetch_skew_us = 80
        self.graph = None
        self.graph_error = None
        self._static = None
        self._static_loss = None
        self._eager_steps = 0
        self._eager_checks = 2
        self._graph_grads = None
        self._capture_stream = None
        self.last_losses = {}
        self._bn_counters = None
        self._grad_slots = {}
        self.grad_scale = 1.0
        self._recapture = False
        self._overlap_armed = False
        self.split_optimizer = split_optimizer
        self.prefetch_graph = os.environ.get("SPACAP_PREFETCH_GRAPH", "1") != "0"
        self.fork_relation = os.environ.get("SPACAP_FORK_RELATION", "1") != "0"
        self.flush_mid = os.environ.get("SPACAP_FLUSH_MID", "1") != "0"
        self._flush_mid, self._mid_done = False, 0
        self._mid_stream = None
        self.overlap_allreduce = os.environ.get("SPACAP_OVERLAP_ALLREDUCE", "0") == "1"
        self.overlap_timeout_ms = 20000
        self._cap_start = None
        self._comm_stream = None
        self._sig = None
        self._sig_host = 0
        self._sig_resync = False
        self._err_host = None
        self._err_event = None
        self._boundary_done = False
        self._armed_step = False
        self.boundary_launches = 0
        self.force_comm_wait = False
        if next(model.parameters()).is_cuda:
            from ._native import check, lib
            check(lib.spacap_sa_reserve_cus(0), "spacap_sa_reserve_cus")
            self._fork_relation(next(model.parameters()).device)
        self._prefetch_graph_key = self._prefetch_graph_obj = self._prefetch_in = self._prefetch_out = None
        broadcast_parameters(model)

    def prefetch(self, next_data):
        pc = next_data["point_clouds"]
        if not pc.is_cuda:
            return
        if self.side_stream is None:
            self.side_stream = _role_stream(pc.device, "side")
            from ._native import check, lib
            check(lib.spacap_sa_reserve_cus(min(64, int(pc.shape[0]))), "spacap_sa_reserve_cus")
        cur = torch.cuda.current_stream(pc.device)
        self.side_stream.wait_stream(cur)
        fn = geometry_pyramid if self.prefetch_geometry else sampling_pyramid
        if self.graph is not None and self.prefetch_graph and not torch.cuda.is_current_stream_capturing():
            key = (tuple(pc.shape), fn is geometry_pyramid)
            if self._prefetch_graph_key != key:
                with torch.cuda.stream(self.side_stream), torch.no_grad():
                    self._prefetch_in = pc[..., :3].contiguous().clone()
                    for _ in range(2):
                        fn(self._prefetch_in)
                self.side_stream.synchronize()
                g = torch.cuda.CUDAGraph()
                with torch.no_grad(), torch.cuda.graph(g, stream=self.side_stream):
                    self._prefetch_out = fn(self._prefetch_in)
                self._prefetch_graph_obj, self._prefetch_graph_key = g, key
                self.side_stream.wait_stream(cur)
            with torch.cuda.stream(self.side_stream), torch.no_grad():
                self._prefetch_in.copy_(pc[..., :3], non_blocking=True)
                skew = int(self.prefetch_skew_us)
                if skew > 0:
                    from ._native import check, lib
                    check(lib.spacap_stream_delay(skew, self.side_stream.cuda_stream), "spacap_stream_delay")
                self._prefetch_graph_obj.replay()
                ev = torch.cuda.Event()
                ev.record(self.side_stream)
            next_data["_fps_prefetch"] = (self._prefetch_out, ev)
            return
        with torch.cuda.stream(self.side_stream), torch.no_grad():
            pyr = fn(pc[..., :3].contiguous())
            ev = torch.cuda.Event()
            ev.record(self.side_stream)
        next_data["_fps_prefetch"] = (pyr, ev)

    @staticmethod
    def _consume_prefetch(data_dict):
        pre = data_dict.pop("_fps_prefetch", None)
        if pre is None:
            return data_dict
        pyr, ev = pre
        cur = torch.cuda.current_stream(pyr[0].device)
        cur.wait_event(ev)
        for t in pyr:
            t.record_stream(cur)
        d = dict(data_dict)
        d["fps_pyramid"] = pyr
        return d

    def loss(self, data_dict):
        kw = dict(num_heading_bin=S.NUM_HEADING_BIN, num_size_cluster=S.NUM_SIZE_CLUSTER, mean_size_arr=self.mean_size_arr)
        need = ("vote_label", "center_label")
        early = (lambda d: start_detection_losses(d, **kw)) if all(k in data_dict for k in need) else None
        d = self.model(dict(data_dict), after_proposal=early)
        det_vec = d.get("_det_vec")
        d = get_scene_cap_loss(d, use_relation=self.use_relation, **kw)
        if self._overlap_armed or self._flush_mid:
            marks = [t for t in (det_vec, d.get("aggregated_vote_features"), d.get("aggregated_vote_xyz"))
                     if torch.is_tensor(t) and t.requires_grad]
            for t in marks:
                t.register_hook(self._boundary_hook if self._overlap_armed else self._mid_flush_hook)
        return d

    def _mid_flush_hook(self, grad):
# ... 81 lines not shown
            if all(id(p) in pos for p in ws + bs):
                groups.append(ws + bs)
                moved.update(id(p) for p in ws + bs)
        rest = [p for p in used if id(p) not in moved]
        return rest + [p for g in groups for p in g]

    def _register_grad_slots(self):
        self._grad_slots = {}
        ps, flat, offs = self.bucket.params, self.bucket.flat, self.bucket.offsets
        pos = {id(p): i for i, p in enumerate(ps)}
        for m in self.model.modules():
            if isinstance(m, torch.nn.Linear) and m.bias is not None:
                iw, ib = pos.get(id(m.weight)), pos.get(id(m.bias))
                if iw is not None and ib == iw + 1 and offs[ib] == offs[iw] + m.weight.numel():
                    self._grad_slots[m.weight.data_ptr()] = flat[offs[iw]:offs[iw] + m.weight.numel() + m.bias.numel()]
        for m in self._attention_modules():
            pk = getattr(m, "_packed_qkv", None)
            ws, bs = [l.weight for l in m.linears[:3]], [l.bias for l in m.linears[:3]]
            if pk is None or not all(id(t) in pos for t in ws + bs):
                continue
            i0 = pos[id(ws[0])]
            n = sum(t.numel() for t in ws + bs)
            if [pos[id(t)] for t in ws + bs] == list(range(i0, i0 + 6)) and offs[i0 + 5] + bs[2].numel() == offs[i0] + n:
                self._grad_slots[pk[0].data_ptr()] = flat[offs[i0]:offs[i0] + n]

    def _attach_packed_qkv(self):
        from .linear import packed_views
        for m in self._attention_modules():
            pk = packed_views(self.optimizer.flat_p, [l.weight for l in m.linears[:3]], [l.bias for l in m.linears[:3]])
            m._packed_qkv = pk

    def _core(self, data_dict, with_optimizer=True):
        pc = data_dict["point_clouds"]
        if pc.is_cuda:
            from .attention import advance_rng
            advance_rng(pc.device)
        self.bucket.zero()
        if self._bn_counters is not None:
            self._bn_counters.add_(1)
        self._overlap_armed = self._overlap_possible(pc)
        if pc.is_cuda and (self.fork_relation and self.use_relation and not self._overlap_armed) != getattr(self, "_fork_on", False):
            self._fork_relation(pc.device, armed=self._overlap_armed)
        self._armed_step = self._overlap_armed
        self._boundary_done = False
        self._mid_done, self._mid_stream = 0, None
        self._flush_mid = self.flush_mid and pc.is_cuda and not self._overlap_armed
        if self._overlap_armed:
            self._sig[:1].add_(1)
        d = self.loss(data_dict)
        if pc.is_cuda:
            from ._native import deferred_slab_sums, grad_slots
            if all(p.grad is None for p in self.bucket.params):
                with grad_slots(getattr(self, "_grad_slots", None)), deferred_slab_sums() as dq:
                    d["loss"].backward(self._seed_grad(d["loss"]))
                    if self._mid_stream is not None:
                        torch.cuda.current_stream(pc.device).wait_stream(self._mid_stream)
                        self._mid_stream = None
                    if self._eager_checks > 0:
                        self._eager_checks -= 1
                        spans = sorted((g.data_ptr(), g.data_ptr() + g.numel() * g.element_size())
                                       for g in (p.grad for p in self.model.parameters()) if g is not None)
                        merged = []
                        for lo, hi in spans:
                            if merged and lo <= merged[-1][1]:
                                merged[-1][1] = max(merged[-1][1], hi)
                            else:
                                merged.append([lo, hi])
                        def covered(o):
                            lo, hi = o.data_ptr(), o.data_ptr() + o.numel() * o.element_size()
                            got = sum(max(0, min(hi, b) - max(lo, a)) for a, b in merged)
                            return got >= (hi - lo) - 15 * o.element_size()
                        lost = [tuple(o.shape) for o in dq.outputs() if not covered(o)]
                        if lost:
                            raise RuntimeError(f"deferred weight-gradient sums did not land in a leaf .grad: {lost}")
            else:
                d["loss"].backward()
        else:
            d["loss"].backward()
        self._overlap_armed = False
        if with_optimizer:
            self._optimizer_step(None)
        self.last_losses = {k: d[k].detach() for k in ("loss", "vote_loss", "objectness_loss", "box_loss", "sem_cls_loss",
                                                       "cap_loss", "relation_loss") if k in d and torch.is_tensor(d[k])}
        return d["loss"].detach()

    def _seed_grad(self, loss):
        one = getattr(self, "_one", None)
        if one is None or one.device != loss.device or one.dtype != loss.dtype or one.shape != loss.shape:
            one = self._one = torch.ones_like(loss)
        return one

    def _optimizer_step(self, sources):
        flat = not isinstance(self.optimizer, torch.optim.Optimizer)
        if getattr(self, "_armed_step", False):
            if self._sig_resync:
                torch.cuda.synchronize(self._sig.device)
                self._sig_host = int(self._sig[0].item())
                self._sig_resync = False
            else:
                self._sig_host += 1
        if flat and self._boundary_done:
            self._overlapped_tail(sources)
            return
        scale = self.bucket.all_reduce(sources=sources, force_pack=self.split_optimizer or flat, average=not flat)
        self.grad_scale = scale
        if flat:
            self.optimizer.step(grad_scale=scale)
        else:
            self.optimizer.step()

    def _find_captioner_suffix(self):
        names = {id(p): n for n, p in self.model.named_parameters()}
        ps = self.bucket.params
        i = len(ps)
        while i > 0 and names.get(id(ps[i - 1]), "").startswith("caption."):
            i -= 1
        ok = 0 < i < len(ps) and not any(names.get(id(p), "").startswith("caption.") for p in ps[:i])
        self._cap_start = i if ok else None

    def _overlap_possible(self, pc):
        if not (self.overlap_allreduce and pc.is_cuda and self._cap_start is not None and self.bucket is not None
                and not self.bucket.views_mode and not isinstance(self.optimizer, torch.optim.Optimizer)):
            return False
        import torch.distributed as dist
        multi = dist.is_available() and dist.is_initialized() and dist.get_world_size() > 1
        if not (multi or self.split_optimizer):
            return False
        return self._sig is not None

    def _boundary_hook(self, grad):
        if self._overlap_armed and not self._boundary_done:
            self._boundary_done = True
            self._boundary()
        return None

    def _boundary(self):
        from . import _native
        from ._native import check, copy_batched, lib
        dq = _native._DEFERRED
        if dq is not None:
# ... 12 lines not shown

    def _overlapped_tail(self, sources):
        import torch.distributed as dist
        from ._native import check, copy_batched, lib
        b, i0 = self.bucket, self._cap_start
        dev = b.flat.device
        multi = dist.is_available() and dist.is_initialized() and dist.get_world_size() > 1
        off = b.offsets[i0]
        main = torch.cuda.current_stream(dev)
        err = self._sig[2:3]
        if multi or self.force_comm_wait:
            comm = self._comm_stream
            with torch.cuda.stream(comm):
                check(lib.spacap_stream_wait_ge(self._sig[1:2].data_ptr(), self._sig_host, int(self.overlap_timeout_ms),
                                                err.data_ptr(), comm.cuda_stream), "spacap_stream_wait_ge")
                if multi:
                    dist.all_reduce(b.flat[off:], op=dist.ReduceOp.SUM)
                    dist.all_reduce(err, op=dist.ReduceOp.MAX)
        if sources is None:
            sources = [p.grad for p in b.params]
        pairs = [(v, s_) for v, s_ in zip(b.views[:i0], sources[:i0]) if s_ is not None and s_.data_ptr() != v.data_ptr()]
        if pairs:
            copy_batched([v for v, _ in pairs], [s_.contiguous() for _, s_ in pairs])
        none = [v for v, s_ in zip(b.views[:i0], sources[:i0]) if s_ is None]
        if none:
            torch._foreach_zero_(none)
        for p, v in zip(b.params, b.views):
            p.grad = v
        if multi:
            dist.all_reduce(b.flat[:off], op=dist.ReduceOp.SUM)
        if multi or self.force_comm_wait:
            main.wait_stream(self._comm_stream)
        self.grad_scale = 1.0 / dist.get_world_size() if multi else 1.0
        self.optimizer.step(grad_scale=self.grad_scale, skip_word=err)
        self._err_host.copy_(err, non_blocking=True)
        self._err_event = torch.cuda.Event()
        self._err_event.record(main)

    def check_health(self, wait=True):
        if self._sig is None or self._err_event is None:
            return
        if wait:
            self._err_event.synchronize()
        elif not self._err_event.query():
            return
        bad = int(self._err_host[0])
        if bad:
            raise RuntimeError(
                f"overlapped gradient all-reduce: the wait for step {bad}'s captioner gradients timed out after "
                f"{self.overlap_timeout_ms} ms on some rank; that step's optimizer update was skipped on every rank and "
                "the exchange cannot be trusted any more (set SPACAP_OVERLAP_ALLREDUCE=0 for the serial tail)")

    def enable_graph(self, example, warmup=3):
        import torch.distributed as dist
        dev = example["point_clouds"].device
        if dev.type != "cuda":
            return False
        world = dist.get_world_size() if (dist.is_available() and dist.is_initialized()) else 1
        self._graph_with_opt = (world == 1) and not self.split_optimizer
        try:
            if self.bucket is None:
                self._setup({k: v for k, v in example.items() if k != "_fps_prefetch"})
            ex = self._consume_prefetch(dict(example))
            static = {}
            for k, v in ex.items():
                if k == "fps_pyramid":
                    static[k] = [t.clone() for t in v]
# ... 242 lines not shown
```

### spacap3d_amd/ext.py

```python
import torch

from . import _native
from ._native import check, lib


def _chk_contig(t, name):
    if not t.is_contiguous():
        raise RuntimeError(f"{name} must be a contiguous tensor")


def _chk_float(t, name):
    if t.dtype != torch.float32:
        raise RuntimeError(f"{name} must be a float tensor")


def _chk_int(t, name):
    if t.dtype != torch.int32:
        raise RuntimeError(f"{name} must be an int tensor")


def _chk_gpu(t, name, like=None):
    if not t.is_cuda:
        if like is None:
            raise RuntimeError("CPU not supported")
# ... 58 lines not shown
    m = knows.shape[1]
    with torch.cuda.device(unknowns.device):
        idx = torch.empty(B, n, 3, dtype=torch.int32, device=unknowns.device)
        dist2 = torch.empty(B, n, 3, dtype=torch.float32, device=unknowns.device)
        check(lib.spacap_three_nn_f32(unknowns.data_ptr(), knows.data_ptr(), B, n, m, dist2.data_ptr(),
                                      idx.data_ptr(), _stream(unknowns)), "three_nn")
    return [dist2, idx]


def three_nn_weights(unknowns, knows):
    _chk_contig(unknowns, "unknowns"); _chk_contig(knows, "knows")
    _chk_float(unknowns, "unknowns"); _chk_float(knows, "knows")
    _chk_gpu(unknowns, "unknowns"); _chk_gpu(knows, "knows", unknowns)
    B, n, _ = unknowns.shape
    m = knows.shape[1]
    with torch.cuda.device(unknowns.device):
        idx = torch.empty(B, n, 3, dtype=torch.int32, device=unknowns.device)
        weight = torch.empty(B, n, 3, dtype=torch.float32, device=unknowns.device)
        check(lib.spacap_three_nn_weights_f32(unknowns.data_ptr(), knows.data_ptr(), B, n, m, weight.data_ptr(),
                                              idx.data_ptr(), _stream(unknowns)), "three_nn_weights")
    return idx, weight


def gather_xyz(xyz, idx):
    _chk_contig(xyz, "xyz"); _chk_contig(idx, "idx")
    _chk_float(xyz, "xyz"); _chk_int(idx, "idx")
    _chk_gpu(xyz, "xyz"); _chk_gpu(idx, "idx", xyz)
    B, N, _ = xyz.shape
    m = idx.shape[1]
    with torch.cuda.device(xyz.device):
        out = torch.empty(B, m, 3, dtype=torch.float32, device=xyz.device)
        check(lib.spacap_gather_xyz_f32(xyz.data_ptr(), idx.data_ptr(), B, N, m, out.data_ptr(), _stream(xyz)), "gather_xyz")
    return out


def three_interpolate(points, idx, weight):
    _chk_contig(points, "points"); _chk_contig(idx, "idx"); _chk_contig(weight, "weight")
    _chk_float(points, "points"); _chk_int(idx, "idx"); _chk_float(weight, "weight")
    _chk_gpu(points, "points"); _chk_gpu(idx, "idx", points); _chk_gpu(weight, "weight", points)
    B, C, m = points.shape
    n = idx.shape[1]
    with torch.cuda.device(points.device):
        out = torch.empty(B, C, n, dtype=torch.float32, device=points.device)
        check(lib.spacap_three_interpolate_f32(points.data_ptr(), idx.data_ptr(), weight.data_ptr(), B, C, m, n,
                                               out.data_ptr(), _stream(points)), "three_interpolate")
    return out


def three_interpolate_grad(grad_out, idx, weight, m):
    _chk_contig(grad_out, "grad_out"); _chk_contig(idx, "idx"); _chk_contig(weight, "weight")
    _chk_float(grad_out, "grad_out"); _chk_int(idx, "idx"); _chk_float(weight, "weight")
    _chk_gpu(grad_out, "grad_out"); _chk_gpu(idx, "idx", grad_out); _chk_gpu(weight, "weight", grad_out)
    B, C, n = grad_out.shape
    with torch.cuda.device(grad_out.device):
        out = torch.empty(B, C, int(m), dtype=torch.float32, device=grad_out.device)
        check(lib.spacap_three_interpolate_grad_f32(grad_out.data_ptr(), idx.data_ptr(), weight.data_ptr(), B, C,
                                                    n, int(m), out.data_ptr(), _stream(grad_out)),
              "three_interpolate_grad")
    return out


def three_interpolate_grad_pm(grad_pm, idx, weight, m):
    _chk_contig(grad_pm, "grad_pm"); _chk_contig(idx, "idx"); _chk_contig(weight, "weight")
    _chk_float(grad_pm, "grad_pm"); _chk_float(weight, "weight")
    _chk_gpu(grad_pm, "grad_pm"); _chk_gpu(idx, "idx", grad_pm); _chk_gpu(weight, "weight", grad_pm)
    B, n, C = grad_pm.shape
# ... 83 lines not shown
```

### spacap3d_amd/fused_losses.py

```python
import torch
from torch.autograd import Function

from ._native import check, lib


class DetectionLosses(Function):

    @staticmethod
    def forward(ctx, net, center, vote_xyz, agg_xyz, gt_center, box_mask, heading_cls_label, heading_res_label,
                size_cls_label, size_res_label, sem_cls_label, mean_size, seed_xyz, seed_inds, vote_label, vote_mask,
                NH, NS, near_thr, far_thr, w0, w1):
        dev = net.device
        net, center, vote_xyz = net.contiguous(), center.contiguous(), vote_xyz.contiguous()
        B, K, CH = net.shape
        M, NSEED, N = gt_center.shape[1], seed_xyz.shape[1], vote_label.shape[1]
        NC = CH - 5 - 2 * NH - 4 * NS
        f32 = dict(dtype=torch.float32, device=dev)
        c = lambda t: t.contiguous()
        with torch.cuda.device(dev):
            obj_label = torch.empty(B, K, dtype=torch.int64, device=dev)
            assignment = torch.empty(B, K, dtype=torch.int64, device=dev)
            obj_mask = torch.empty(B, K, **f32)
            dnet_n = torch.empty(B, K, CH, **f32)
            dcen_n = torch.empty(B, K, 6, **f32)
            dvote_n = torch.empty(B, NSEED, 3, **f32)
            part = torch.empty(B * (int(lib.spacap_det_npart()) + 2), **f32)
            losses = torch.empty(8, **f32)
            inv_den = torch.empty(4, **f32)
            args = [c(agg_xyz), c(gt_center[:, :, 0:3]), c(box_mask), c(heading_cls_label), c(heading_res_label),
                    c(size_cls_label), c(size_res_label), c(sem_cls_label), c(mean_size), c(seed_xyz)]
            si, vl, vm = c(seed_inds.to(torch.int32)), c(vote_label), c(vote_mask)
            check(lib.spacap_det_losses_fwd_f32(
                net.data_ptr(), center.data_ptr(), *[a.data_ptr() for a in args], vote_xyz.data_ptr(), si.data_ptr(),
                vl.data_ptr(), vm.data_ptr(), B, K, M, NSEED, N, int(NH), int(NS), int(NC), float(near_thr), float(far_thr),
                float(w0), float(w1), obj_label.data_ptr(), obj_mask.data_ptr(), assignment.data_ptr(), dnet_n.data_ptr(),
                dcen_n.data_ptr(), dvote_n.data_ptr(), part.data_ptr(), losses.data_ptr(), inv_den.data_ptr(),
                torch.cuda.current_stream(dev).cuda_stream), "spacap_det_losses_fwd_f32")
        ctx.save_for_backward(dnet_n, dcen_n, dvote_n, inv_den)
        ctx.meta = (B, K, NSEED, int(NH), int(NS), int(NC))
        ctx.mark_non_differentiable(obj_label, obj_mask, assignment)
        ctx.set_materialize_grads(False)
        return losses, obj_label, obj_mask, assignment

    @staticmethod
    def backward(ctx, g_losses, _a, _b, _c):
        dnet_n, dcen_n, dvote_n, inv_den = ctx.saved_tensors
        B, K, NSEED, NH, NS, NC = ctx.meta
        dev = dnet_n.device
        g = g_losses.contiguous()
        with torch.cuda.device(dev):
            dnet = torch.empty_like(dnet_n)
            dcenter = torch.empty(B, K, 3, dtype=torch.float32, device=dev)
            dvote = torch.empty_like(dvote_n)
            check(lib.spacap_det_losses_bwd_f32(dnet_n.data_ptr(), dcen_n.data_ptr(), dvote_n.data_ptr(), g.data_ptr(),
                                                inv_den.data_ptr(), B, K, NSEED, NH, NS, NC, dnet.data_ptr(),
                                                dcenter.data_ptr(), dvote.data_ptr(),
                                                torch.cuda.current_stream(dev).cuda_stream), "spacap_det_losses_bwd_f32")
        return (dnet, dcenter, dvote) + (None,) * 19


def detection_losses(d, num_heading_bin, num_size_cluster, mean_size_f32, near_thr, far_thr, w):
    losses, label, mask, oa = DetectionLosses.apply(
        d["_proposal_net"], d["center"], d["vote_xyz"], d["aggregated_vote_xyz"], d["center_label"], d["box_label_mask"],
        d["heading_class_label"], d["heading_residual_label"], d["size_class_label"], d["size_residual_label"],
        d["sem_cls_label"], mean_size_f32, d["seed_xyz"], d["seed_inds"], d["vote_label"], d["vote_label_mask"],
        num_heading_bin, num_size_cluster, near_thr, far_thr, w[0], w[1])
    d["_det_vec"] = losses
    vote, objn, center, hcls, hreg, scls, sreg, sem = losses.unbind(0)
    return vote, objn, label, mask, oa, center, hcls, hreg, scls, sreg, sem, None

# ... 18 lines not shown
        ctx.save_for_backward(dnum, out)
        ctx.bk = (B, K)
        return out

    @staticmethod
    def backward(ctx, g):
        dnum, out = ctx.saved_tensors
        B, K = ctx.bk
        g3 = g[0:3].contiguous()
        with torch.cuda.device(dnum.device):
            dpred = torch.empty_like(dnum)
            check(lib.spacap_rel_loss_bwd_f32(dnum.data_ptr(), g3.data_ptr(), out.data_ptr(), B, K, dpred.data_ptr(),
                                              torch.cuda.current_stream(dnum.device).cuda_stream), "spacap_rel_loss_bwd_f32")
        return dpred, None, None, None, None, None, None


def relation_losses(d):
    out = RelationLoss.apply(d["relation_pred"], d["object_assignment"], d["box_label_mask_int"], d["objectness_label"],
                             d["x_label"], d["y_label"], d["z_label"])
    d["_rel_vec"] = out
    return {"x_loss": out[0], "y_loss": out[1], "z_loss": out[2], "x_acc": out[3], "y_acc": out[4], "z_acc": out[5]}


class CaptionHeadLoss(Function):

    @staticmethod
    def forward(ctx, logits, lang_ids, good):
        if not logits.is_cuda:
            raise RuntimeError("CPU not supported")
        logits = logits.contiguous()
        B, W, V = logits.shape
        ids = lang_ids.contiguous()
        assert ids.dtype == torch.int64 and ids.shape[0] == B and ids.shape[1] >= W + 1
        g8 = good.to(torch.uint8).contiguous()
        dev = logits.device
        with torch.cuda.device(dev):
            logp = torch.empty_like(logits)
            rowstat = torch.empty(B * W, 4, dtype=torch.float32, device=dev)
            out = torch.empty(4, dtype=torch.float32, device=dev)
            check(lib.spacap_cap_loss_fwd_f32(logits.data_ptr(), ids.data_ptr() + 8, g8.data_ptr(), B, W, V, ids.shape[1],
                                              logp.data_ptr(), rowstat.data_ptr(), out.data_ptr(),
                                              torch.cuda.current_stream(dev).cuda_stream), "spacap_cap_loss_fwd_f32")
        ctx.save_for_backward(logp, ids, g8, out)
        ctx.mark_non_differentiable(logp)
        ctx.set_materialize_grads(False)
        return logp, out

    @staticmethod
    def backward(ctx, _g_logp, g_out):
        logp, ids, g8, out = ctx.saved_tensors
        B, W, V = logp.shape
        dev = logp.device
        gl = g_out[0:1].contiguous()
        with torch.cuda.device(dev):
            dlogits = torch.empty_like(logp)
            check(lib.spacap_cap_loss_bwd_f32(logp.data_ptr(), ids.data_ptr() + 8, g8.data_ptr(), out.data_ptr(), gl.data_ptr(),
                                              B, W, V, ids.shape[1], dlogits.data_ptr(),
                                              torch.cuda.current_stream(dev).cuda_stream), "spacap_cap_loss_bwd_f32")
        return dlogits, None, None


def caption_head_loss(logits, lang_ids, good):
    logp, out = CaptionHeadLoss.apply(logits, lang_ids, good)
    return logp, out[0], out[1], out


class ProposalDecode(Function):

    @staticmethod
    def forward(ctx, net, agg_xyz, mean_size, mean_size_f64, NH, NS):
        if not net.is_cuda:
            raise RuntimeError("CPU not supported")
        net, agg, msa = net.contiguous(), agg_xyz.contiguous(), mean_size.contiguous()
        B, CH, K = net.shape
        NC = CH - 5 - 2 * NH - 4 * NS
        dev = net.device
        f32 = dict(dtype=torch.float32, device=dev)
        i64 = dict(dtype=torch.int64, device=dev)
        with torch.cuda.device(dev):
            nt, center = torch.empty(B, K, CH, **f32), torch.empty(B, K, 3, **f32)
            hres, sres = torch.empty(B, K, NH, **f32), torch.empty(B, K, NS, 3, **f32)
            corners = torch.empty(B, K, 8, 3, dtype=torch.float64, device=dev)
            bm, sem, sc = torch.empty(B, K, **i64), torch.empty(B, K, **i64), torch.empty(B, K, **i64)
            check(lib.spacap_proposal_decode_fwd_f32(net.data_ptr(), agg.data_ptr(), msa.data_ptr(),
                                                     mean_size_f64.contiguous().data_ptr() if mean_size_f64 is not None else None, B, K, int(NH), int(NS), int(NC),
                                                     nt.data_ptr(), center.data_ptr(), hres.data_ptr(), sres.data_ptr(),
                                                     corners.data_ptr(), bm.data_ptr(), sem.data_ptr(), sc.data_ptr(),
                                                     torch.cuda.current_stream(dev).cuda_stream), "spacap_proposal_decode_fwd_f32")
        ctx.save_for_backward(msa)
        ctx.meta = (B, K, CH, int(NH), int(NS), int(NC))
        ctx.mark_non_differentiable(corners, bm, sem, sc)
        ctx.set_materialize_grads(False)
        return nt, center, hres, sres, corners, bm, sem, sc

    @staticmethod
    def backward(ctx, g_nt, g_center, g_hres, g_sres, *_):
        (msa,) = ctx.saved_tensors
        B, K, CH, NH, NS, NC = ctx.meta
        dev = msa.device
        c = lambda t: t.contiguous() if t is not None else None
        g_nt, g_center, g_hres, g_sres = c(g_nt), c(g_center), c(g_hres), c(g_sres)
        p = lambda t: t.data_ptr() if t is not None else None
        with torch.cuda.device(dev):
            d_net = torch.empty(B, CH, K, dtype=torch.float32, device=dev)
            check(lib.spacap_proposal_decode_bwd_f32(p(g_nt), p(g_center), p(g_hres), p(g_sres), msa.data_ptr(), B, K, NH, NS, NC,
                                                     d_net.data_ptr(), torch.cuda.current_stream(dev).cuda_stream),
                  "spacap_proposal_decode_bwd_f32")
        return d_net, g_center, None, None, None, None


def proposal_decode(net, agg_xyz, mean_size, mean_size_f64, NH, NS):
    return ProposalDecode.apply(net, agg_xyz, mean_size, mean_size_f64, NH, NS)


class LossTail(Function):

    @staticmethod
    def forward(ctx, det, cap, rel, obj_label, obj_mask, bbox_mask):
        dev = det.device
        with torch.cuda.device(dev):
            out = torch.empty(8, dtype=torch.float32, device=dev)
            loss = torch.empty((), dtype=torch.float32, device=dev)
            ol = obj_label.to(torch.int64).contiguous().view(-1)
            om = obj_mask.to(torch.float32).contiguous().view(-1)
            bm = bbox_mask.to(torch.int64).contiguous().view(-1)
            if not (ol.numel() == om.numel() == bm.numel()):
                raise RuntimeError("loss_tail: objectness_label, objectness_mask and bbox_mask must have one entry per proposal")
            check(lib.spacap_loss_tail_fwd_f32(det.contiguous().data_ptr(), cap.contiguous().data_ptr(),
                                               rel.contiguous().data_ptr() if rel is not None else None, ol.data_ptr(),
                                               om.data_ptr(), bm.data_ptr(), ol.numel(), out.data_ptr(), loss.data_ptr(),
                                               torch.cuda.current_stream(dev).cuda_stream), "spacap_loss_tail_fwd_f32")
        ctx.has_rel = rel is not None
        ctx.mark_non_differentiable(out)
        ctx.set_materialize_grads(False)
        return loss, out

    @staticmethod
    def backward(ctx, g_loss, _g_out):
        dev = g_loss.device
        with torch.cuda.device(dev):
            gdet = torch.empty(8, dtype=torch.float32, device=dev)
            gcap = torch.empty(4, dtype=torch.float32, device=dev)
            grel = torch.empty(7, dtype=torch.float32, device=dev) if ctx.has_rel else None
            check(lib.spacap_loss_tail_bwd_f32(g_loss.contiguous().data_ptr(), gdet.data_ptr(), gcap.data_ptr(),
                                               grel.data_ptr() if grel is not None else None,
# ... 79 lines not shown
```

### spacap3d_amd/linear.py

```python
import torch
import torch.nn.functional as F
from torch.autograd import Function

from ._native import check, conv1x1_wgrad_partials, grad_slot, lib, linear_wgrad_partials, sum_slabs


def rows_product(a2, W, bias, trans_w):
    R, K = a2.shape
    CO = W.shape[0] if trans_w else W.shape[1]
    dev = a2.device
    with torch.cuda.device(dev):
        out = torch.empty(R, CO, dtype=torch.float32, device=dev)
        check(lib.spacap_linear_rows_f32(a2.data_ptr(), W.data_ptr(), bias.data_ptr() if bias is not None else None, R, K, CO,
                                         1 if trans_w else 0, out.data_ptr(), torch.cuda.current_stream(dev).cuda_stream),
              "spacap_linear_rows_f32")
    return out


def use_rows(R, K, CO):
    return bool(lib.spacap_linear_rows_supported(R, K, CO)) and _ROWS_RULE(R, K, CO)


_ROWS_RULE = lambda R, K, CO: R <= 512

# ... 148 lines not shown
        else:
            s = sum_slabs(part, deferrable=True, out=grad_slot(weight, CK * CP + CK))
            dw, db = s[:CK * CP].view(CK, CP), s[CK * CP:]
        a, b, _ = ctx.split
        return (dx, None, None, dw[:a], dw[a:a + b], dw[a + b:], db[:a], db[a:a + b], db[a + b:])


def packed_views(flat, params_w, params_b):
    def adjacent(ps):
        lo, hi = flat.data_ptr(), flat.data_ptr() + flat.numel() * flat.element_size()
        return all(p.is_contiguous() and lo <= p.data_ptr() < hi for p in ps) and \
            all(ps[i + 1].data_ptr() == ps[i].data_ptr() + ps[i].numel() * ps[i].element_size() for i in range(len(ps) - 1))
    if not (adjacent(params_w) and adjacent(params_b)) or any(p.shape[1:] != params_w[0].shape[1:] for p in params_w):
        return None
    rows, cols = sum(p.shape[0] for p in params_w), params_w[0].shape[1]
    ow = (params_w[0].data_ptr() - flat.data_ptr()) // flat.element_size()
    ob = (params_b[0].data_ptr() - flat.data_ptr()) // flat.element_size()
    return flat[ow:ow + rows * cols].view(rows, cols), flat[ob:ob + rows]


class Conv1x1(Function):

    @staticmethod
    def forward(ctx, x, weight, bias):
        ctx.save_for_backward(x, weight)
        ctx.has_bias = bias is not None
        y = conv1x1_cm(0, weight, x, bias, weight.shape[0])
        if y is not None:
            return y
        return F.conv2d(x, weight, bias) if x.dim() == 4 else F.conv1d(x, weight, bias)

    @staticmethod
    def backward(ctx, g):
        x, weight = ctx.saved_tensors
        B, CI = x.shape[0], x.shape[1]
        CO = weight.shape[0]
        N = x.numel() // (B * CI)
        g = g.contiguous()
        dx = None
        if ctx.needs_input_grad[0]:
            dx = conv1x1_cm(1, weight, g, None, CI)
            if dx is None:
                dx = torch.ops.aten.convolution_backward(g, x, weight, None, [1] * (x.dim() - 2), [0] * (x.dim() - 2),
                                                         [1] * (x.dim() - 2), False, [0] * (x.dim() - 2), 1,
                                                         [True, False, False])[0]
        if not ctx.needs_input_grad[1]:
            db = g.sum(dim=[0] + list(range(2, g.dim()))) if (ctx.has_bias and ctx.needs_input_grad[2]) else None
            return dx, None, db
        if int(lib.spacap_conv1x1_wgrad_slabs(B, CO, CI, N)):
            part = conv1x1_wgrad_partials(g, x, B, CO, CI, N, deferrable=True, with_bias=ctx.has_bias)
            s = sum_slabs(part, deferrable=True)
            if part.shape[1] != CO * CI:
                return dx, s[:CO * CI].view_as(weight), s[CO * CI:CO * CI + CO]
            dw = s.view_as(weight)
        else:
            dw = torch.ops.aten.convolution_backward(g, x, weight, None, [1] * (x.dim() - 2), [0] * (x.dim() - 2),
                                                     [1] * (x.dim() - 2), False, [0] * (x.dim() - 2), 1,
                                                     [False, True, False])[1]
        db = g.sum(dim=[0] + list(range(2, g.dim()))) if ctx.has_bias else None
        return dx, dw, db


CONV_FWD_EXACT_F32 = False


def conv1x1_cm(mode, weight, t, bias, M):
    B, C = t.shape[0], t.shape[1]
    N = t.numel() // max(B * C, 1)
    CO, CI = weight.shape[0], weight.shape[1]
    if not (t.is_cuda and t.dtype == torch.float32 and t.is_contiguous() and weight.is_contiguous() and B > 0 and
            lib.spacap_conv1x1_cm_supported(CI, CO, N)) or t.data_ptr() % 16:
        return None
    with torch.cuda.device(t.device):
        out = torch.empty((B, M) + tuple(t.shape[2:]), dtype=torch.float32, device=t.device)
        check(lib.spacap_conv1x1_cm_f32(2 if (mode == 0 and CONV_FWD_EXACT_F32) else mode, weight.data_ptr(), t.data_ptr(),
                                        bias.data_ptr() if bias is not None else None,
                                        B, CI, CO, N, out.data_ptr(), torch.cuda.current_stream(t.device).cuda_stream),
              "spacap_conv1x1_cm_f32")
    return out


def conv1x1(x, conv):
    if not (x.is_cuda and x.dtype == torch.float32) or any(k != 1 for k in conv.kernel_size) or not x.is_contiguous():
        return None
    needs = torch.is_grad_enabled() and (x.requires_grad or conv.weight.requires_grad
                                         or (conv.bias is not None and conv.bias.requires_grad))
    if not needs:
        return conv1x1_cm(0, conv.weight, x, conv.bias, conv.out_channels)
    B, CI = x.shape[0], x.shape[1]
    N = x.numel() // max(B * CI, 1)
    if int(lib.spacap_conv1x1_wgrad_slabs(B, conv.out_channels, CI, N)) == 0:
        return None
    return Conv1x1.apply(x, conv.weight, conv.bias)
# ... 309 lines not shown
```

### spacap3d_amd/optim.py

```python
import torch

from ._native import check, lib


class FlatAdam:
    def __init__(self, bucket, lr=1e-3, betas=(0.9, 0.999), eps=1e-8, weight_decay=0.0):
        self.bucket = bucket
        self.lr, self.betas, self.eps, self.weight_decay = float(lr), (float(betas[0]), float(betas[1])), float(eps), float(weight_decay)
        flat_g = bucket.flat
        if not flat_g.is_cuda:
            raise RuntimeError("CPU not supported")
        self.flat_p = torch.zeros_like(flat_g)
        with torch.no_grad():
            for p, off in zip(bucket.params, bucket.offsets):
                view = self.flat_p[off:off + p.numel()].view_as(p)
                view.copy_(p)
                p.data = view
        self.m = torch.zeros_like(flat_g)
        self.v = torch.zeros_like(flat_g)
        self.step_t = torch.zeros((), dtype=torch.float32, device=flat_g.device)

    @torch.no_grad()
    def step(self, grad_scale=1.0, skip_word=None):
        dev = self.flat_p.device
        self.step_t += 1
        with torch.cuda.device(dev):
            check(lib.spacap_adam_flat_f32(self.flat_p.data_ptr(), self.bucket.flat.data_ptr(), self.m.data_ptr(),
                                           self.v.data_ptr(), self.flat_p.numel(), self.lr, self.betas[0], self.betas[1],
                                           self.eps, self.weight_decay, self.step_t.data_ptr(), float(grad_scale),
                                           skip_word.data_ptr() if skip_word is not None else None,
                                           torch.cuda.current_stream(dev).cuda_stream), "spacap_adam_flat_f32")
```

### spacap3d_amd/pointnet2_modules.py

```python
from typing import List

import torch
import torch.nn as nn
import torch.nn.functional as F

from . import pointnet2_utils


class _BN2d(nn.Sequential):

    def __init__(self, channels: int):
        super().__init__()
        self.add_module("bn", nn.BatchNorm2d(channels))
        nn.init.constant_(self[0].weight, 1.0)
        nn.init.constant_(self[0].bias, 0.0)


class _ConvBNReLU2d(nn.Sequential):

    def __init__(self, cin: int, cout: int, bn: bool):
        super().__init__()
        conv = nn.Conv2d(cin, cout, kernel_size=(1, 1), stride=(1, 1), padding=(0, 0), bias=not bn)
        nn.init.kaiming_normal_(conv.weight)
        if not bn:
# ... 37 lines not shown
        return x


class PointnetSAModuleVotes(nn.Module):

    def __init__(self, *, mlp: List[int], npoint: int = None, radius: float = None, nsample: int = None,
                 bn: bool = True, use_xyz: bool = True, pooling: str = "max", normalize_xyz: bool = False):
        super().__init__()
        assert pooling == "max", "only max pooling is on the SpaCap3D path"
        assert npoint is not None, "GroupAll is not on the SpaCap3D path"
        self.npoint, self.radius, self.nsample = npoint, radius, nsample
        self.use_xyz, self.normalize_xyz = use_xyz, normalize_xyz
        self.grouper = pointnet2_utils.QueryAndGroup(radius, nsample, use_xyz=use_xyz, ret_grouped_xyz=True,
                                                     normalize_xyz=normalize_xyz)
        mlp_spec = list(mlp)
        if use_xyz and len(mlp_spec) > 0:
            mlp_spec[0] += 3
        self.mlp_module = SharedMLP(mlp_spec, bn=bn)

    def forward(self, xyz: torch.Tensor, features: torch.Tensor = None, inds: torch.Tensor = None,
                idx: torch.Tensor = None, rows_idx: torch.Tensor = None, new_xyz: torch.Tensor = None):
        if inds is None:
            inds = pointnet2_utils.furthest_point_sample(xyz, self.npoint)
        else:
            assert inds.shape[1] == self.npoint
        from .backend import ops
        fused = getattr(ops(), "sa_mlp_train", None) if self.training else None
        if new_xyz is not None and not xyz.requires_grad:
            assert new_xyz.shape == (xyz.shape[0], self.npoint, 3)
        elif fused is not None and xyz.is_cuda:
            if not xyz.requires_grad and inds.dtype == torch.int32:
                from . import ext
                new_xyz = ext.gather_xyz(xyz.contiguous(), inds.contiguous())
            else:
                new_xyz = torch.gather(xyz, 1, inds.long().unsqueeze(-1).expand(-1, -1, 3))
        else:
            xyz_flipped = xyz.transpose(1, 2).contiguous()
            new_xyz = pointnet2_utils.gather_operation(xyz_flipped, inds).transpose(1, 2).contiguous()
        if idx is None:
            idx = pointnet2_utils.ball_query(self.radius, self.nsample, xyz, new_xyz)
        else:
            assert idx.shape[1:] == (self.npoint, self.nsample)
        if fused is not None:
            out = fused(xyz, new_xyz, features, idx, self.mlp_module, self.radius if self.normalize_xyz else 1.0,
                        self.use_xyz, rows_idx)
            if out is not None:
                return new_xyz, out, inds
        fused_eval = getattr(ops(), "sa_mlp_eval", None) if (not self.training and not torch.is_grad_enabled()) else None
        if fused_eval is not None and xyz.is_cuda:
            out = fused_eval(xyz, new_xyz, features, idx, self.mlp_module, self.radius if self.normalize_xyz else 1.0,
                             self.use_xyz)
            if out is not None:
                return new_xyz, out, inds
        if features is not None:
            features = features.contiguous()
        grouped_features, _grouped_xyz = self.grouper(xyz, new_xyz, features, idx=idx)
        new_features = self.mlp_module(grouped_features, pool=True)
        return new_xyz, new_features, inds


class PointnetFPModule(nn.Module):

    def __init__(self, *, mlp: List[int], bn: bool = True):
        super().__init__()
        self.mlp = SharedMLP(list(mlp), bn=bn)

# ... 26 lines not shown
```

### spacap3d_amd/transformer_captioner.py

```python
import copy
import math

import torch
import torch.nn as nn
import torch.nn.functional as F

from .backend import ops
from .loss_helper import nn_distance

MAX_DES_LEN = 30
PROPOSAL_FEATURE_DIM = 128


def subsequent_mask(size, device=None):
    return torch.ones(1, size, size, dtype=torch.bool, device=device).tril()


def clones(module, N):
    return nn.ModuleList([copy.deepcopy(module) for _ in range(N)])


def attention(query, key, value, mask=None, dropout=None, need_p=True):
    p = dropout.p if dropout is not None else 0.0
    training = dropout.training if dropout is not None else False
# ... 175 lines not shown


class PositionalEncoding(nn.Module):
    def __init__(self, d_model, dropout, max_len=5000):
        super().__init__()
        self.dropout = nn.Dropout(p=dropout)
        pe = torch.zeros(max_len, d_model)
        position = torch.arange(0, max_len).unsqueeze(1).float()
        div_term = torch.exp(torch.arange(0, d_model, 2).float() * -(math.log(10000.0) / d_model))
        pe[:, 0::2] = torch.sin(position * div_term)
        pe[:, 1::2] = torch.cos(position * div_term)
        self.register_buffer("pe", pe.unsqueeze(0))

    def forward(self, x, src_pos=None):
        return self.dropout(x + self.pe[:, :x.size(1)])


class PositionalEncodingLearned(nn.Module):
    def __init__(self, input_channel, d_model=128):
        super().__init__()
        self.position_embedding_head = nn.Sequential(
            nn.Conv1d(input_channel, d_model, kernel_size=1), nn.BatchNorm1d(d_model), nn.ReLU(inplace=True),
            nn.Conv1d(d_model, d_model, kernel_size=1))

    def forward(self, x, xyz):
        h = self.position_embedding_head
        t = xyz.transpose(1, 2).contiguous()
        if self.training and t.is_cuda and getattr(ops(), "bn_relu_train", None) is not None:
            conv = getattr(ops(), "conv1x1", None)

            def c(m, v):
                y = conv(v, m) if conv is not None else None
                return m(v) if y is None else y
            t = c(h[3], ops().bn_relu_train(c(h[0], t), h[1]))
        elif t.is_cuda and not torch.is_grad_enabled() and getattr(ops(), "conv1x1", None) is not None:
            conv = ops().conv1x1

            def c(m, v):
                y = conv(v, m)
                return m(v) if y is None else y
            g = getattr(ops(), "bn_relu_eval", None)
            u = c(h[0], t)
            v = g(u, h[1]) if g is not None else None
            t = c(h[3], h[2](h[1](u)) if v is None else v)
        else:
            t = h(t)
        return x + t.transpose(1, 2).contiguous()


class Encoder(nn.Module):
    def __init__(self, layer, N):
        super().__init__()
        self.layers = clones(layer, N)
        self.norm = LayerNorm(layer.size)

    def forward(self, x, mask):
        st = getattr(ops(), "tf_stack", None)
        if st is not None and st.stack_supported(self.layers, x):
            return st.run_stack(self.layers, self.norm, x, mask)
        for layer in self.layers:
            x = layer(x, mask)
        return self.norm(x)


class EncoderLayer(nn.Module):
    def __init__(self, size, self_attn, feed_forward, dropout):
        super().__init__()
# ... 145 lines not shown
            if isinstance(m, nn.BatchNorm1d):
                m.momentum = bn_momentum
        return model

    def _prepare_feature(self, seq):
        seq = seq[:, :-1] if self.early_guide else seq[:, 1:-1]
        seq_mask = (seq > 0).unsqueeze(-2)
        seq_mask = seq_mask & subsequent_mask(seq.size(-1), device=seq.device)
        return (seq[:, 1:] if self.early_guide else seq), seq_mask

    def forward(self, data_dict, is_eval=False):
        return self.forward_eval(data_dict) if is_eval else self.forward_train(data_dict)

    def _src_pos(self, ep):
        if self.src_pos_type == "xyz":
            return ep["aggregated_vote_xyz"]
        if self.src_pos_type == "center":
            return ep["center"]
        if self.src_pos_type == "loc":
            return torch.cat([ep["center"], ep["pred_size"]], -1)
        return None

    def relation_feature(self):
        sa = self.model.encoder.layers[-1].self_attn
        return ops().relation_feature(sa.attn, sa.value)

    def forward_train(self, ep):
        src = ep["aggregated_vote_features"]
        if self.token_proj is not None:
            src = _linear(src, self.token_proj)
        src_pos = self._src_pos(ep)
        prep = getattr(ops(), "caption_prep", None) if (src.is_cuda and self.early_guide and self.model.encoder is not None) else None
        src_mask = ep["bbox_mask"].unsqueeze(1)
        x0 = out_full = None
        if prep is not None:
            memory = self.model.encode(src, src_pos, src_mask)
            if self.check_relation:
                self._relation_head_forked(ep)
            te = self.model.tgt_embed
            got = prep(ep["aggregated_vote_xyz"], ep["ref_center_label"], src, memory, ep["lang_label"], te[0], te[1])
            if got is not None:
                x0, m8, idx1, dist, good, pred_ious = got
                ep["match_idx"] = idx1
                out_full = self.model.decoder(x0, None, None, m8)
                out = out_full[:, 1:, :]
        if x0 is None:
            _, _, target_ious, idx = nn_distance(ep["aggregated_vote_xyz"], ep["ref_center_label"].unsqueeze(1))
            ep["match_idx"] = idx.squeeze(1)
            ref_obj_feature = torch.gather(src, 1, idx.repeat(1, src.size(-1)).unsqueeze(1))
            seq, seq_mask = self._prepare_feature(ep["lang_label"])
            if prep is None:
                memory = None
                if self.model.encoder is not None:
                    memory = self.model.encode(src, src_pos, src_mask)
                    if self.check_relation:
                        self._relation_head(ep)
            out = self.model(src=src, tgt=seq, src_mask=src_mask, tgt_mask=seq_mask,
                             obj_indicator=ref_obj_feature, src_pos=src_pos,
                             obj_idx=idx if self.use_transformer_encoder else None, memory=memory)
            out = out[:, 1:, :] if self.early_guide else out
            good = (target_ious > -1).squeeze(1)
            pred_ious = (target_ious.squeeze(1) * good).sum() / good.sum().clamp(min=1)
        fused = getattr(ops(), "caption_head_loss", None) if (out.is_cuda and self.training and "lang_ids" in ep) else None
        if fused is not None and ep["lang_ids"].shape[1] >= out.shape[1] + 1:
            vp = getattr(ops(), "vocab_projection", None) if out_full is not None else None
            logits = vp(out_full, self.model.generator.proj, 1) if vp is not None else None
# ... 166 lines not shown
```

Baseline: 1166 scenes/s.

## Fuse positional-encoding conv with residual add, add glue batching and misc kernel fusions

Adds a conv1x1 variant that writes point-major output with the bias and residual added in its epilogue, so the positional encoding skips a separate transpose, contiguous copy and add. The proposal decoder now also emits a uint8 bbox mask that attention uses directly instead of converting the int64 mask. Also adds a custom gather_xyz backward kernel, a det-loss entry point that takes a leading dimension for seed indices, a batched glue kernel for small copies and adds, and an optional step bump in Adam. These cut small kernel launches and conversions in the training step, at the cost of more native code paths and attaching side tensors to masks through ad-hoc attributes.

```diff
diff --git a/include/spacap_hip.h b/include/spacap_hip.h
--- a/include/spacap_hip.h
+++ b/include/spacap_hip.h
@@ -61,6 +61,8 @@
 int spacap_three_nn_weights_f32(const float *unknown, const float *known, int B, int n, int m,
                                 float *weight, int32_t *idx, spacap_stream_t stream);
 int spacap_gather_xyz_f32(const float *xyz, const int32_t *idx, int B, int N, int m, float *out, spacap_stream_t stream);
+int spacap_gather_xyz_grad_f32(const float *g, long g_sb, long g_sj, long g_sc, const int32_t *idx, int B, int N, int m, float *dxyz,
+                               spacap_stream_t stream);
 int spacap_three_interpolate_f32(const float *points, const int32_t *idx, const float *weight,
                                  int B, int C, int m, int n, float *out, spacap_stream_t stream);
 int spacap_three_interpolate_grad_f32(const float *grad_out, const int32_t *idx,
@@ -288,6 +290,15 @@
                               float w1, int64_t *obj_label, float *obj_mask, int64_t *assignment, float *dnet_num,
                               float *dcenter_num, float *dvote_num, float *part, float *losses, float *inv_den,
                               spacap_stream_t stream);
+int spacap_det_losses_fwd_ld_f32(const float *net, const float *center, const float *agg_xyz, const float *gt_center,
+                                 const float *box_mask, const int64_t *heading_cls_label, const float *heading_res_label,
+                                 const int64_t *size_cls_label, const float *size_res_label, const int64_t *sem_cls_label,
+                                 const float *mean_size, const float *seed_xyz, const float *vote_xyz,
+                                 const int32_t *seed_inds, int seed_inds_ld, const float *vote_label, const int64_t *vote_mask,
+                                 int B, int K, int M, int NSEED, int N, int NH, int NS, int NC, float near_thr, float far_thr,
+                                 float w0, float w1, int64_t *obj_label, float *obj_mask, int64_t *assignment, float *dnet_num,
+                                 float *dcenter_num, float *dvote_num, float *part, float *losses, float *inv_den,
+                                 spacap_stream_t stream);
 int spacap_det_losses_bwd_f32(const float *dnet_num, const float *dcenter_num, const float *dvote_num,
                               const float *grad_losses, const float *inv_den, int B, int K, int NSEED, int NH, int NS,
                               int NC, float *dnet, float *dcenter, float *dvote, spacap_stream_t stream);
@@ -369,6 +380,10 @@
 int spacap_proposal_decode_fwd_f32(const float *net, const float *agg_xyz, const float *mean_size, const double *mean_size_f64,
                                    int B, int K, int NH, int NS, int NC, float *nt, float *center, float *heading_res, float *size_res, double *corners,
                                    int64_t *bbox_mask, int64_t *sem_cls, int64_t *size_cls, spacap_stream_t stream);
+int spacap_proposal_decode_fwd_mask_f32(const float *net, const float *agg_xyz, const float *mean_size, const double *mean_size_f64,
+                                        int B, int K, int NH, int NS, int NC, float *nt, float *center, float *heading_res,
+                                        float *size_res, double *corners, int64_t *bbox_mask, int64_t *sem_cls, int64_t *size_cls,
+                                        uint8_t *bbox_mask_u8, spacap_stream_t stream);
 int spacap_proposal_decode_bwd_f32(const float *g_nt, const float *g_center, const float *g_heading_res, const float *g_size_res,
                                    const float *mean_size, int B, int K, int NH, int NS, int NC, float *d_net, spacap_stream_t stream);
 
@@ -443,6 +458,8 @@
 int spacap_conv1x1_cm_supported(int CI, int CO, long N);
 int spacap_conv1x1_cm_f32(int mode, const float *W, const float *in, const float *bias, int B, int CI, int CO, long N,
                           float *out, spacap_stream_t stream);
+int spacap_conv1x1_cm_pm_f32(int mode, const float *W, const float *in, const float *bias, const float *addend_pm, int B, int CI,
+                             int CO, long N, float *out_pm, spacap_stream_t stream);
 
 int spacap_vote_assemble_fwd_f32(const float *net, const float *seed_xyz, const float *seed_feat, int B, int C, int N,
                                  float *vote_xyz, float *vote_feat, spacap_stream_t stream);
@@ -450,6 +467,15 @@
                                  spacap_stream_t stream);
 
 int spacap_copy_batched(const void *const *src, void *const *dst, const long *nbytes, int njobs, spacap_stream_t stream);
+
+enum { SPACAP_GLUE_COPY = 0, SPACAP_GLUE_ADD_I64 = 1, SPACAP_GLUE_ADD_F32 = 2, SPACAP_GLUE_COLS_32 = 3 };
+typedef struct spacap_glue_job {
+  const void *src;
+  void *dst;
+  long n, imm;
+  int kind, w, ld, c0;
+} spacap_glue_job;
+int spacap_glue_batched(const spacap_glue_job *jobs, int njobs, spacap_stream_t stream);
 
 int spacap_stream_delay(int microseconds, spacap_stream_t stream);
 int spacap_stream_wait_ge(const int64_t *flag, int64_t value, int timeout_ms, int64_t *err, spacap_stream_t stream);
diff --git a/spacap3d_amd/_native.py b/spacap3d_amd/_native.py
--- a/spacap3d_amd/_native.py
+++ b/spacap3d_amd/_native.py
@@ -33,6 +33,7 @@
     "spacap_three_nn_f32": (_i, [_p, _p, _i, _i, _i, _p, _p, _p]),
     "spacap_three_nn_weights_f32": (_i, [_p, _p, _i, _i, _i, _p, _p, _p]),
     "spacap_gather_xyz_f32": (_i, [_p, _p, _i, _i, _i, _p, _p]),
+    "spacap_gather_xyz_grad_f32": (_i, [_p, _l, _l, _l, _p, _i, _i, _i, _p, _p]),
     "spacap_three_interpolate_f32": (_i, [_p, _p, _p, _i, _i, _i, _i, _p, _p]),
     "spacap_three_interpolate_grad_f32": (_i, [_p, _p, _p, _i, _i, _i, _i, _p, _p]),
     "spacap_three_interpolate_grad_pm_f32": (_i, [_p, _p, _p, _i, _i, _i, _i, _p, _p]),
@@ -62,6 +63,7 @@
     "spacap_caption_prep_bwd_f32": (_i, [_p] * 3 + [_i] * 5 + [_f, _u64, _p, _p, _p, _p]),
     "spacap_conv1x1_cm_supported": (_i, [_i, _i, _l]),
     "spacap_conv1x1_cm_f32": (_i, [_i, _p, _p, _p, _i, _i, _i, _l, _p, _p]),
+    "spacap_conv1x1_cm_pm_f32": (_i, [_i, _p, _p, _p, _p, _i, _i, _i, _l, _p, _p]),
     "spacap_sa_l1_stats_f32": (_i, [_p, _p, _p, _p, _p, _i, _f, _i, _i, _i, _i, _i, _p, _p, _p]),
     "spacap_sa_l1_moments_f32": (_i, [_p, _p, _p, _p, _f, _i, _i, _i, _i, _p, _p, _p]),
     "spacap_sa_l1_moments_finalize_f32": (_i, [_p, _p, _i, _i, _i, _l, _f, _f, _p, _p, _p, _p, _p, _p]),
@@ -74,6 +76,7 @@
     "spacap_vote_assemble_fwd_f32": (_i, [_p, _p, _p, _i, _i, _i, _p, _p, _p]),
     "spacap_vote_assemble_bwd_f32": (_i, [_p, _p, _i, _i, _i, _p, _p, _p]),
     "spacap_copy_batched": (_i, [_p, _p, _p, _i, _p]),
+    "spacap_glue_batched": (_i, [_p, _i, _p]),
     "spacap_lab_stamp": (_i, [_p, _p]),
     "spacap_points_in_box_workspace_bytes": (ctypes.c_size_t, [_i, _i, _i]),
     "spacap_points_in_box_f32": (_i, [_p, _i, _i, _i, _p, _i, _p, ctypes.c_size_t, _p]),
@@ -166,6 +169,7 @@
     "spacap_scene_votes_f32": (_i, [_p, _p, _p, _i, _i, _i, _i, _p, _p, _p, _p]),
     "spacap_det_npart": (_i, []),
     "spacap_det_losses_fwd_f32": (_i, [_p] * 16 + [_i] * 8 + [_f] * 4 + [_p] * 9 + [_p]),
+    "spacap_det_losses_fwd_ld_f32": (_i, [_p] * 14 + [_i] + [_p] * 2 + [_i] * 8 + [_f] * 4 + [_p] * 9 + [_p]),
     "spacap_det_losses_bwd_f32": (_i, [_p] * 5 + [_i] * 6 + [_p] * 3 + [_p]),
     "spacap_rel_loss_nparts": (_l, [_i, _i]),
     "spacap_rel_loss_fwd_f32": (_i, [_p] * 7 + [_i] * 3 + [_p] * 3 + [_p]),
@@ -193,6 +197,7 @@
     "spacap_layernorm_bwd_f32": (_i, [_p, _p, _p, _p, _l, _i, _f, _p, _p, _p, _p, _p]),
     "spacap_layernorm_bwd_add_f32": (_i, [_p, _p, _p, _p, _p, _l, _i, _f, _p, _p, _p, _p, _p]),
     "spacap_proposal_decode_fwd_f32": (_i, [_p, _p, _p, _p, _i, _i, _i, _i, _i, _p, _p, _p, _p, _p, _p, _p, _p, _p]),
+    "spacap_proposal_decode_fwd_mask_f32": (_i, [_p, _p, _p, _p, _i, _i, _i, _i, _i, _p, _p, _p, _p, _p, _p, _p, _p, _p, _p]),
     "spacap_proposal_decode_bwd_f32": (_i, [_p, _p, _p, _p, _p, _i, _i, _i, _i, _i, _p, _p]),
     "spacap_loss_tail_fwd_f32": (_i, [_p, _p, _p, _p, _p, _p, _i, _p, _p, _p]),
     "spacap_loss_tail_bwd_f32": (_i, [_p, _p, _p, _p, _p]),
@@ -228,6 +233,13 @@
     _fields_ = [("mode", _i), ("R", _l), ("a1", _p), ("w1", _p), ("bias1", _p), ("k1", _i), ("drop_p", _f), ("eps", _f),
                 ("seed", _u64), ("seed_dev", _p), ("res", _p), ("x_out", _p), ("ln_a", _p), ("ln_b", _p), ("n_out", _p),
                 ("stats", _p), ("x_ln", _p), ("g", _p), ("part", _p), ("w2", _p), ("bias2", _p), ("out2", _p), ("n2", _i), ("nparts", _i), ("attn_out", _p), ("delta_out", _p), ("lq", _i)]
+
+
+class GlueJob(ctypes.Structure):
+    _fields_ = [("src", _p), ("dst", _p), ("n", _l), ("imm", _l), ("kind", _i), ("w", _i), ("ld", _i), ("c0", _i)]
+
+
+GLUE_COPY, GLUE_ADD_I64, GLUE_ADD_F32, GLUE_COLS_32 = 0, 1, 2, 3
 
 
 def _load():
@@ -445,3 +457,25 @@
     dev = dsts[0].device
     with torch.cuda.device(dev):
         check(lib.spacap_copy_batched(src, dst, nb, n, torch.cuda.current_stream(dev).cuda_stream), "spacap_copy_batched")
+
+
+def glue_batched(jobs, device):
+    import torch
+    arr = (GlueJob * len(jobs))()
+    for j, (kind, dst, src, imm, w, c0) in zip(arr, jobs):
+        assert dst.is_cuda and dst.is_contiguous() and (src is None or (src.is_cuda and src.is_contiguous()))
+        j.kind, j.dst, j.src, j.imm, j.w, j.c0, j.ld = kind, dst.data_ptr(), (src.data_ptr() if src is not None else None), int(imm), int(w), int(c0), 0
+        if kind == GLUE_COPY:
+            assert src.dtype == dst.dtype and src.numel() == dst.numel()
+            j.n = dst.numel() * dst.element_size()
+        elif kind == GLUE_ADD_I64:
+            assert dst.dtype == torch.int64
+            j.n = dst.numel()
+        elif kind == GLUE_ADD_F32:
+            assert dst.dtype == torch.float32
+            j.n = dst.numel()
+        else:
+            assert src.dtype == dst.dtype and src.element_size() == 4 and dst.numel() * src.shape[-1] == src.numel() * int(w)
+            j.n, j.ld = dst.numel(), src.shape[-1]
+    with torch.cuda.device(device):
+        check(lib.spacap_glue_batched(arr, len(jobs), torch.cuda.current_stream(device).cuda_stream), "spacap_glue_batched")
diff --git a/spacap3d_amd/attention.py b/spacap3d_amd/attention.py
--- a/spacap3d_amd/attention.py
+++ b/spacap3d_amd/attention.py
@@ -28,6 +28,9 @@
 
 def _prep_mask_uncached(mask, B, Lq, Lk):
     m = mask
+    u8 = getattr(mask, "_spacap_u8", None)
+    if u8 is not None and u8.shape == mask.shape and u8.dtype == torch.uint8 and u8.device == mask.device:
+        m = u8
     if m.dim() == 4:
         assert m.size(1) == 1, "per-head masks are not used by the reference"
         m = m[:, 0]
diff --git a/spacap3d_amd/backend.py b/spacap3d_amd/backend.py
--- a/spacap3d_amd/backend.py
+++ b/spacap3d_amd/backend.py
@@ -39,6 +39,7 @@
         self.linear = _lin.linear
         self.ffn_tail = _lin.ffn_tail
         self.conv1x1 = _lin.conv1x1
+        self.conv1x1_add_pm = _lin.conv1x1_add_pm
         self.relation_tail = _lin.relation_tail
         self.relation_head = _lin.relation_head
         self.vocab_projection = _lin.vocab_projection
diff --git a/spacap3d_amd/csrc/conv1x1.hip b/spacap3d_amd/csrc/conv1x1.hip
--- a/spacap3d_amd/csrc/conv1x1.hip
+++ b/spacap3d_amd/csrc/conv1x1.hip
@@ -10,10 +10,38 @@
 
 constexpr int TM = 64, TN = 64, KC = 32, LDN = TN + 4, LDW = TM + 4;
 
+__device__ __forceinline__ void pm_epilogue(const f32x4 (&acc)[4], const float *__restrict__ bias, const float *__restrict__ addend_pm,
+                                            float *__restrict__ out_pm, int b, int M, int N, int mb, int nb) {
+  if (mb >= M) return;
+  const bool vec = mb + 3 < M && (M & 3) == 0;
+#pragma unroll
+  for (int t = 0; t < 4; ++t) {
+    const size_t o = ((size_t)b * N + nb + 16 * t) * M + mb;
+    if (vec) {
+      f32x4 v;
+#pragma unroll
+      for (int u = 0; u < 4; ++u) v[u] = acc[t][u] + (bias ? bias[mb + u] : 0.f);
+      if (addend_pm) {
+        const f32x4 r = ld4(addend_pm + o);
+#pragma unroll
+        for (int u = 0; u < 4; ++u) v[u] = r[u] + v[u];
+      }
+      st4(out_pm + o, v);
+    } else {
+      for (int u = 0; u < 4 && mb + u < M; ++u) {
+        float v = acc[t][u] + (bias ? bias[mb + u] : 0.f);
+        if (addend_pm) v = addend_pm[o + u] + v;
+        out_pm[o + u] = v;
+      }
+    }
+  }
+}
+
 template <bool TRANS_A>
 __global__ __launch_bounds__(256) void conv1x1_cm_kernel(const float *__restrict__ W, int lda, const float *__restrict__ in,
                                                          const float *__restrict__ bias, int M, int K, int N,
-                                                         float *__restrict__ out) {
+                                                         float *__restrict__ out, float *__restrict__ out_pm,
+                                                         const float *__restrict__ addend_pm) {
   __shared__ __attribute__((aligned(16))) float s_in[2][KC * LDN];
   __shared__ __attribute__((aligned(16))) float s_w[TRANS_A ? 2 * KC * LDW : 4];
   const int tid = threadIdx.x, lane = tid & 63, w = tid >> 6, l15 = lane & 15, lg = lane >> 4;
@@ -86,6 +114,10 @@
       for (int t = 0; t < 4; ++t) acc[t] = MFMA16(av, si[s * LDN + 16 * t], acc[t]);
     }
   }
+  if (out_pm) {
+    pm_epilogue(acc, bias, addend_pm, out_pm, b, M, N, m0 + 16 * w + 4 * lg, n0 + l15);
+    return;
+  }
 #pragma unroll
   for (int u = 0; u < 4; ++u) {
     const int m = m0 + 16 * w + 4 * lg + u;
@@ -106,7 +138,8 @@
 template <bool TRANS_A>
 __global__ __launch_bounds__(256) void conv1x1_cm_bf3_kernel(const float *__restrict__ W, int lda, const float *__restrict__ in,
                                                              const float *__restrict__ bias, int M, int K, int N,
-                                                             float *__restrict__ out) {
+                                                             float *__restrict__ out, float *__restrict__ out_pm,
+                                                             const float *__restrict__ addend_pm) {
   __shared__ __attribute__((aligned(16))) __bf16 s_b[2][3 * BIMG];
   __shared__ __attribute__((aligned(16))) __bf16 s_a[TRANS_A ? 2 * 3 * BIMG : 8];
   const int tid = threadIdx.x, lane = tid & 63, w = tid >> 6, l15 = lane & 15, lg = lane >> 4;
@@ -202,6 +235,10 @@
 #pragma unroll
       for (int q = 0; q < 6; ++q) acc[t] = MFMA_B(a[PA[q]], bq[PB[q]], acc[t]);
     }
+  }
+  if (out_pm) {
+    pm_epilogue(acc, bias, addend_pm, out_pm, b, M, N, m0 + 16 * w + 4 * lg, n0 + l15);
+    return;
   }
 #pragma unroll
   for (int u = 0; u < 4; ++u) {
@@ -233,9 +270,30 @@
   const dim3 grid((unsigned)(N / TN), (unsigned)((M + TM - 1) / TM), (unsigned)B);
   hipStream_t s = spacap::as_stream(stream);
   if (mode == 0 && !f32fwd && !spacap::sa_f32_mfma_only())
-    hipLaunchKernelGGL(conv1x1_cm_bf3_kernel<false>, grid, dim3(256), 0, s, W, CI, in, bias, M, K, (int)N, out);
-  else if (mode == 0) hipLaunchKernelGGL(conv1x1_cm_kernel<false>, grid, dim3(256), 0, s, W, CI, in, bias, M, K, (int)N, out);
-  else hipLaunchKernelGGL(conv1x1_cm_kernel<true>, grid, dim3(256), 0, s, W, CI, in, (const float *)nullptr, M, K, (int)N, out);
+    hipLaunchKernelGGL(conv1x1_cm_bf3_kernel<false>, grid, dim3(256), 0, s, W, CI, in, bias, M, K, (int)N, out, (float *)nullptr, (const float *)nullptr);
+  else if (mode == 0) hipLaunchKernelGGL(conv1x1_cm_kernel<false>, grid, dim3(256), 0, s, W, CI, in, bias, M, K, (int)N, out, (float *)nullptr, (const float *)nullptr);
+  else hipLaunchKernelGGL(conv1x1_cm_kernel<true>, grid, dim3(256), 0, s, W, CI, in, (const float *)nullptr, M, K, (int)N, out, (float *)nullptr,
+                            (const float *)nullptr);
   SPACAP_CHECK_LAUNCH(what);
   return SPACAP_OK;
 }
+
+extern "C" int spacap_conv1x1_cm_pm_f32(int mode, const float *W, const float *in, const float *bias, const float *addend_pm, int B, int CI,
+                                        int CO, long N, float *out_pm, spacap_stream_t stream) {
+  const char *what = "spacap_conv1x1_cm_pm_f32";
+  SPACAP_REQUIRE((mode == 0 || mode == 2) && B >= 0 && spacap_conv1x1_cm_supported(CI, CO, N) && N <= 2147483647L && B <= 65535,
+                 "%s: (mode=%d, B=%d, CI=%d, CO=%d, N=%ld) unsupported", what, mode, B, CI, CO, N);
+  if (B == 0) return SPACAP_OK;
+  SPACAP_REQUIRE(W && in && out_pm && spacap::aligned16(in, out_pm) && (!addend_pm || spacap::aligned16(addend_pm)),
+                 "%s: null or unaligned pointer", what);
+  const dim3 grid((unsigned)(N / TN), (unsigned)((CO + TM - 1) / TM), (unsigned)B);
+  hipStream_t s = spacap::as_stream(stream);
+  if (mode == 0 && !spacap::sa_f32_mfma_only())
+    hipLaunchKernelGGL(conv1x1_cm_bf3_kernel<false>, grid, dim3(256), 0, s, W, CI, in, bias, CO, CI, (int)N, (float *)nullptr, out_pm,
+                       addend_pm);
+  else
+    hipLaunchKernelGGL(conv1x1_cm_kernel<false>, grid, dim3(256), 0, s, W, CI, in, bias, CO, CI, (int)N, (float *)nullptr, out_pm,
+                       addend_pm);
+  SPACAP_CHECK_LAUNCH(what);
+  return SPACAP_OK;
+}
diff --git a/spacap3d_amd/csrc/elementwise.hip b/spacap3d_amd/csrc/elementwise.hip
--- a/spacap3d_amd/csrc/elementwise.hip
+++ b/spacap3d_amd/csrc/elementwise.hip
@@ -356,6 +356,94 @@
 }
 
 namespace {
+constexpr int GLUE_MAX = 48;
+struct GlueJob {
+  const char *src;
+  char *dst;
+  long n, imm;
+  int block0, kind, w, ld, c0, vec;
+};
+struct GlueTable {
+  int njobs, pad;
+  GlueJob job[GLUE_MAX];
+};
+__global__ __launch_bounds__(256) void glue_batched_kernel(const GlueTable T) {
+  int lo = 0, hi = T.njobs - 1;
+  while (lo < hi) {
+    const int mid = (lo + hi + 1) >> 1;
+    if (T.job[mid].block0 <= (int)blockIdx.x) lo = mid; else hi = mid - 1;
+  }
+  const GlueJob J = T.job[lo];
+  const long blk = (long)((int)blockIdx.x - J.block0);
+  if (J.kind == SPACAP_GLUE_COPY) {
+    const long beg = blk * CPJ_BLOCK_BYTES, end = min(J.n, beg + CPJ_BLOCK_BYTES);
+    if (J.vec) {
+      for (long o = beg + 16 * threadIdx.x; o < end; o += 16 * 256)
+        *reinterpret_cast<f32x4 *>(J.dst + o) = *reinterpret_cast<const f32x4 *>(J.src + o);
+    } else {
+      for (long o = beg + threadIdx.x; o < end; o += 256) J.dst[o] = J.src[o];
+    }
+  } else if (J.kind == SPACAP_GLUE_ADD_I64) {
+    long long *d = reinterpret_cast<long long *>(J.dst);
+    const long beg = blk * (CPJ_BLOCK_BYTES / 8), end = min(J.n, beg + CPJ_BLOCK_BYTES / 8);
+    for (long i = beg + threadIdx.x; i < end; i += 256) d[i] += (long long)J.imm;
+  } else if (J.kind == SPACAP_GLUE_ADD_F32) {
+    float *d = reinterpret_cast<float *>(J.dst);
+    const long beg = blk * (CPJ_BLOCK_BYTES / 4), end = min(J.n, beg + CPJ_BLOCK_BYTES / 4);
+    for (long i = beg + threadIdx.x; i < end; i += 256) d[i] += (float)J.imm;
+  } else {
+    const unsigned *sp = reinterpret_cast<const unsigned *>(J.src);
+    unsigned *d = reinterpret_cast<unsigned *>(J.dst);
+    const long beg = blk * (CPJ_BLOCK_BYTES / 4), end = min(J.n, beg + CPJ_BLOCK_BYTES / 4);
+    for (long i = beg + threadIdx.x; i < end; i += 256) {
+      const long r = i / J.w;
+      d[i] = sp[r * J.ld + J.c0 + (int)(i - r * J.w)];
+    }
+  }
+}
+}
+extern "C" int spacap_glue_batched(const spacap_glue_job *jobs, int njobs, spacap_stream_t stream) {
+  const char *what = "spacap_glue_batched";
+  SPACAP_REQUIRE(njobs >= 0 && (njobs == 0 || jobs), "%s: bad arguments", what);
+  hipStream_t s = spacap::as_stream(stream);
+  int i = 0;
+  while (i < njobs) {
+    GlueTable T;
+    T.njobs = 0, T.pad = 0;
+    long blocks = 0;
+    for (; i < njobs && T.njobs < GLUE_MAX; ++i) {
+      const spacap_glue_job &in = jobs[i];
+      SPACAP_REQUIRE(in.kind >= SPACAP_GLUE_COPY && in.kind <= SPACAP_GLUE_COLS_32 && in.n >= 0, "%s: job %d: bad kind or size", what, i);
+      if (in.n == 0) continue;
+      const bool reads = in.kind == SPACAP_GLUE_COPY || in.kind == SPACAP_GLUE_COLS_32;
+      SPACAP_REQUIRE(in.dst && (!reads || in.src), "%s: job %d: null pointer", what, i);
+      const uintptr_t ps = reinterpret_cast<uintptr_t>(in.src), pd = reinterpret_cast<uintptr_t>(in.dst);
+      long per = CPJ_BLOCK_BYTES;
+      if (in.kind == SPACAP_GLUE_ADD_I64) {
+        SPACAP_REQUIRE((pd & 7) == 0, "%s: job %d: unaligned int64 words", what, i);
+        per = CPJ_BLOCK_BYTES / 8;
+      } else if (in.kind == SPACAP_GLUE_ADD_F32) {
+        SPACAP_REQUIRE((pd & 3) == 0, "%s: job %d: unaligned floats", what, i);
+        per = CPJ_BLOCK_BYTES / 4;
+      } else if (in.kind == SPACAP_GLUE_COLS_32) {
+        SPACAP_REQUIRE(in.w >= 1 && in.c0 >= 0 && in.ld >= in.c0 + in.w && in.n % in.w == 0 && ((ps | pd) & 3) == 0,
+                       "%s: job %d: bad column window (w=%d, ld=%d, c0=%d, n=%ld)", what, i, in.w, in.ld, in.c0, in.n);
+        per = CPJ_BLOCK_BYTES / 4;
+      }
+      GlueJob &J = T.job[T.njobs++];
+      J.src = static_cast<const char *>(in.src), J.dst = static_cast<char *>(in.dst), J.n = in.n, J.imm = in.imm;
+      J.block0 = (int)blocks, J.kind = in.kind, J.w = in.w, J.ld = in.ld, J.c0 = in.c0;
+      J.vec = ((ps | pd | (uintptr_t)in.n) & 15) == 0;
+      blocks += (in.n + per - 1) / per;
+      SPACAP_REQUIRE(blocks < 2147483647L, "%s: too many blocks", what);
+    }
+    if (T.njobs) hipLaunchKernelGGL(glue_batched_kernel, dim3((unsigned)blocks), dim3(256), 0, s, T);
+  }
+  SPACAP_CHECK_LAUNCH(what);
+  return SPACAP_OK;
+}
+
+namespace {
 __global__ void delay_kernel(unsigned long long ticks) {
   const unsigned long long t0 = wall_clock64();
   while (wall_clock64() - t0 < ticks) __builtin_amdgcn_s_sleep(8);
diff --git a/spacap3d_amd/csrc/interpolate.hip b/spacap3d_amd/csrc/interpolate.hip
--- a/spacap3d_amd/csrc/interpolate.hip
+++ b/spacap3d_amd/csrc/interpolate.hip
@@ -63,6 +63,28 @@
   out[i * 3 + 0] = p[0], out[i * 3 + 1] = p[1], out[i * 3 + 2] = p[2];
 }
 
+constexpr int GXG_SPAN = 2048;
+__global__ __launch_bounds__(256) void gather_xyz_grad_kernel(const float *__restrict__ g, long sb, long sj, long sc,
+                                                              const int32_t *__restrict__ idx, int N, int m, float *__restrict__ dxyz) {
+  const int b = blockIdx.y, n0 = blockIdx.x * GXG_SPAN, n1 = min(N, n0 + GXG_SPAN);
+  float *__restrict__ out = dxyz + (size_t)b * N * 3;
+  for (int i = n0 * 3 + threadIdx.x; i < n1 * 3; i += 256) out[i] = 0.f;
+  __syncthreads();
+  const int32_t *__restrict__ id = idx + (size_t)b * m;
+  const float *__restrict__ gb = g + b * sb;
+  for (int j = threadIdx.x; j < m; j += 256) {
+    const int a = id[j];
+    if (a < n0 || a >= n1) continue;
+    bool first = true;
+    for (int k = 0; k < j && first; ++k) first = id[k] != a;
+    if (!first) continue;
+    float x = 0.f + gb[j * sj], y = 0.f + gb[j * sj + sc], z = 0.f + gb[j * sj + 2 * sc];
+    for (int k = j + 1; k < m; ++k)
+      if (id[k] == a) x += gb[k * sj], y += gb[k * sj + sc], z += gb[k * sj + 2 * sc];
+    out[a * 3 + 0] = x, out[a * 3 + 1] = y, out[a * 3 + 2] = z;
+  }
+}
+
 constexpr int CHUNK = 8;
 
 __global__ __launch_bounds__(256) void three_interpolate_kernel(const float *__restrict__ points,
@@ -284,6 +306,19 @@
   return SPACAP_OK;
 }
 
+extern "C" int spacap_gather_xyz_grad_f32(const float *g, long g_sb, long g_sj, long g_sc, const int32_t *idx, int B, int N, int m,
+                                          float *dxyz, spacap_stream_t stream) {
+  const char *what = "spacap_gather_xyz_grad_f32";
+  SPACAP_REQUIRE(B >= 0 && N >= 0 && m >= 0 && B <= 65535 && (long)N * 3 < (1L << 31) && (long)m * 3 < (1L << 31) && g_sb >= 0 &&
+                     g_sj >= 0 && g_sc >= 0, "%s: bad sizes or strides", what);
+  if (B == 0 || N == 0) return SPACAP_OK;
+  SPACAP_REQUIRE(dxyz && (m == 0 || (g && idx)), "%s: null pointer", what);
+  hipLaunchKernelGGL(gather_xyz_grad_kernel, dim3((unsigned)((N + GXG_SPAN - 1) / GXG_SPAN), B), dim3(256), 0, spacap::as_stream(stream), g,
+                     g_sb, g_sj, g_sc, idx, N, m, dxyz);
+  SPACAP_CHECK_LAUNCH(what);
+  return SPACAP_OK;
+}
+
 extern "C" int spacap_three_interpolate_f32(const float *points, const int32_t *idx, const float *weight,
                                             int B, int C, int m, int n, float *out,
                                             spacap_stream_t stream) {
diff --git a/spacap3d_amd/csrc/losses.hip b/spacap3d_amd/csrc/losses.hip
--- a/spacap3d_amd/csrc/losses.hip
+++ b/spacap3d_amd/csrc/losses.hip
@@ -222,7 +222,7 @@
 }
 
 __global__ __launch_bounds__(256) void det_vote_kernel(const float *__restrict__ seed_xyz, const float *__restrict__ vote_xyz,
-                                                       const int32_t *__restrict__ seed_inds,
+                                                       const int32_t *__restrict__ seed_inds, int seed_ld,
                                                        const float *__restrict__ vote_label,
                                                        const int64_t *__restrict__ vote_mask, int NS, int N,
                                                        float *__restrict__ dvote, float *__restrict__ part) {
@@ -231,7 +231,7 @@
   float num = 0.f, cnt = 0.f;
   for (int s = threadIdx.x; s < NS; s += 256) {
     const size_t bs = (size_t)b * NS + s;
-    const int p = seed_inds[bs];
+    const int p = seed_inds[(size_t)b * seed_ld + s];
     const float m = (float)vote_mask[(size_t)b * N + p];
     const float *vl = vote_label + ((size_t)b * N + p) * 9, *sx = seed_xyz + bs * 3, *vx = vote_xyz + bs * 3;
     float best = INFINITY;
@@ -405,17 +405,17 @@
 
 extern "C" int spacap_det_npart(void) { return NPARTL; }
 
-extern "C" int spacap_det_losses_fwd_f32(
-    const float *net, const float *center, const float *agg_xyz, const float *gt_center, const float *box_mask,
+namespace {
+int det_losses_fwd(
+    const char *what, const float *net, const float *center, const float *agg_xyz, const float *gt_center, const float *box_mask,
     const int64_t *heading_cls_label, const float *heading_res_label, const int64_t *size_cls_label,
     const float *size_res_label, const int64_t *sem_cls_label, const float *mean_size, const float *seed_xyz,
-    const float *vote_xyz, const int32_t *seed_inds, const float *vote_label, const int64_t *vote_mask, int B, int K,
+    const float *vote_xyz, const int32_t *seed_inds, int seed_ld, const float *vote_label, const int64_t *vote_mask, int B, int K,
     int M, int NSEED, int N, int NH, int NS, int NC, float near_thr, float far_thr, float w0, float w1,
     int64_t *obj_label, float *obj_mask, int64_t *assignment, float *dnet_num, float *dcenter_num, float *dvote_num,
     float *part, float *losses, float *inv_den, spacap_stream_t stream) {
-  const char *what = "spacap_det_losses_fwd_f32";
-  SPACAP_REQUIRE(B >= 1 && K >= 1 && M >= 1 && M <= MAXM && NSEED >= 1 && NH >= 1 && NS >= 1 && NC >= 1 && B <= 65535,
-                 "%s: bad sizes", what);
+  SPACAP_REQUIRE(B >= 1 && K >= 1 && M >= 1 && M <= MAXM && NSEED >= 1 && NH >= 1 && NS >= 1 && NC >= 1 && B <= 65535 &&
+                     seed_ld >= NSEED, "%s: bad sizes", what);
   SPACAP_REQUIRE(net && center && agg_xyz && gt_center && box_mask && heading_cls_label && heading_res_label &&
                      size_cls_label && size_res_label && sem_cls_label && mean_size && seed_xyz && vote_xyz && seed_inds &&
                      vote_label && vote_mask && obj_label && obj_mask && assignment && dnet_num && dcenter_num &&
@@ -440,11 +440,35 @@
     hipLaunchKernelGGL(det_proposal_kernel<false>, dim3(B), dim3(DET_THREADS), lds, s, A);
   }
   float *vpart = part + (size_t)B * NPARTL;
-  hipLaunchKernelGGL(det_vote_kernel, dim3(B), dim3(256), 0, s, seed_xyz, vote_xyz, seed_inds, vote_label, vote_mask, NSEED, N,
-                     dvote_num, vpart);
+  hipLaunchKernelGGL(det_vote_kernel, dim3(B), dim3(256), 0, s, seed_xyz, vote_xyz, seed_inds, seed_ld, vote_label, vote_mask,
+                     NSEED, N, dvote_num, vpart);
   hipLaunchKernelGGL(det_finalize_kernel, dim3(1), dim3(64), 0, s, part, vpart, B, losses, inv_den);
   SPACAP_CHECK_LAUNCH(what);
   return SPACAP_OK;
+}
+}
+
+#define DET_FWD_PARAMS_A                                                                                                          \
+  const float *net, const float *center, const float *agg_xyz, const float *gt_center, const float *box_mask,                     \
+      const int64_t *heading_cls_label, const float *heading_res_label, const int64_t *size_cls_label,                            \
+      const float *size_res_label, const int64_t *sem_cls_label, const float *mean_size, const float *seed_xyz,                   \
+      const float *vote_xyz, const int32_t *seed_inds
+#define DET_FWD_PARAMS_B                                                                                                          \
+  const float *vote_label, const int64_t *vote_mask, int B, int K, int M, int NSEED, int N, int NH, int NS, int NC,               \
+      float near_thr, float far_thr, float w0, float w1, int64_t *obj_label, float *obj_mask, int64_t *assignment,                \
+      float *dnet_num, float *dcenter_num, float *dvote_num, float *part, float *losses, float *inv_den, spacap_stream_t stream
+#define DET_FWD_ARGS_A                                                                                                            \
+  net, center, agg_xyz, gt_center, box_mask, heading_cls_label, heading_res_label, size_cls_label, size_res_label, sem_cls_label, \
+      mean_size, seed_xyz, vote_xyz, seed_inds
+#define DET_FWD_ARGS_B                                                                                                            \
+  vote_label, vote_mask, B, K, M, NSEED, N, NH, NS, NC, near_thr, far_thr, w0, w1, obj_label, obj_mask, assignment, dnet_num,     \
+      dcenter_num, dvote_num, part, losses, inv_den, stream
+
+extern "C" int spacap_det_losses_fwd_f32(DET_FWD_PARAMS_A, DET_FWD_PARAMS_B) {
+  return det_losses_fwd("spacap_det_losses_fwd_f32", DET_FWD_ARGS_A, NSEED, DET_FWD_ARGS_B);
+}
+extern "C" int spacap_det_losses_fwd_ld_f32(DET_FWD_PARAMS_A, int seed_inds_ld, DET_FWD_PARAMS_B) {
+  return det_losses_fwd("spacap_det_losses_fwd_ld_f32", DET_FWD_ARGS_A, seed_inds_ld, DET_FWD_ARGS_B);
 }
 
 extern "C" int spacap_det_losses_bwd_f32(const float *dnet_num, const float *dcenter_num, const float *dvote_num,
diff --git a/spacap3d_amd/csrc/proposal_decode.hip b/spacap3d_amd/csrc/proposal_decode.hip
--- a/spacap3d_amd/csrc/proposal_decode.hip
+++ b/spacap3d_amd/csrc/proposal_decode.hip
@@ -10,7 +10,8 @@
                                                                   float *__restrict__ nt, float *__restrict__ center,
                                                                   float *__restrict__ hres, float *__restrict__ sres,
                                                                   double *__restrict__ corners, int64_t *__restrict__ bbox_mask,
-                                                                  int64_t *__restrict__ sem_cls, int64_t *__restrict__ size_cls) {
+                                                                  int64_t *__restrict__ sem_cls, int64_t *__restrict__ size_cls,
+                                                                  uint8_t *__restrict__ mask_u8) {
   extern __shared__ float s_x[];
   const int b = blockIdx.y, k0 = blockIdx.x * 64, tid = threadIdx.x;
   const int CH = 5 + 2 * NH + 4 * NS + NC, LD = CH + 1, nk = min(64, K - k0);
@@ -25,6 +26,7 @@
     const float *row = s_x + tid * LD;
     const size_t p = (size_t)b * K + k0 + tid;
     bbox_mask[p] = row[1] > row[0] ? 1 : 0;
+    if (mask_u8) mask_u8[p] = row[1] > row[0] ? 1 : 0;
 #pragma unroll
     for (int d = 0; d < 3; ++d) {
       const float c = agg_xyz[p * 3 + d] + row[2 + d];
@@ -88,11 +90,11 @@
 
 }
 
-extern "C" int spacap_proposal_decode_fwd_f32(const float *net, const float *agg_xyz, const float *mean_size,
-                                              const double *mean_size_f64, int B, int K, int NH, int NS, int NC, float *nt, float *center, float *heading_res, float *size_res,
-                                              double *corners, int64_t *bbox_mask, int64_t *sem_cls, int64_t *size_cls,
-                                              spacap_stream_t stream) {
-  const char *what = "spacap_proposal_decode_fwd_f32";
+namespace {
+int proposal_decode_fwd(const char *what, const float *net, const float *agg_xyz, const float *mean_size, const double *mean_size_f64,
+                        int B, int K, int NH, int NS, int NC, float *nt, float *center, float *heading_res, float *size_res,
+                        double *corners, int64_t *bbox_mask, int64_t *sem_cls, int64_t *size_cls, uint8_t *mask_u8,
+                        spacap_stream_t stream) {
   SPACAP_REQUIRE(B >= 0 && K >= 1 && NH >= 1 && NS >= 1 && NC >= 1, "%s: bad sizes", what);
   if (B == 0) return SPACAP_OK;
   SPACAP_REQUIRE(net && agg_xyz && mean_size && nt && center && heading_res && size_res && corners && bbox_mask && sem_cls && size_cls,
@@ -101,9 +103,29 @@
   SPACAP_REQUIRE((size_t)64 * (CH + 1) * sizeof(float) <= 64 * 1024, "%s: too many channels (%d)", what, CH);
   hipLaunchKernelGGL(proposal_decode_fwd_kernel, dim3((K + 63) / 64, B), dim3(256), (size_t)(64 * (CH + 1) + 256) * sizeof(float),
                      spacap::as_stream(stream), net, agg_xyz, mean_size,
-                     mean_size_f64, K, NH, NS, NC, nt, center, heading_res, size_res, corners, bbox_mask, sem_cls, size_cls);
-  SPACAP_CHECK_LAUNCH(what);
-  return SPACAP_OK;
+                     mean_size_f64, K, NH, NS, NC, nt, center, heading_res, size_res, corners, bbox_mask, sem_cls, size_cls, mask_u8);
+  SPACAP_CHECK_LAUNCH(what);
+  return SPACAP_OK;
+}
+}
+
+extern "C" int spacap_proposal_decode_fwd_f32(const float *net, const float *agg_xyz, const float *mean_size,
+                                              const double *mean_size_f64, int B, int K, int NH, int NS, int NC, float *nt, float *center, float *heading_res, float *size_res,
+                                              double *corners, int64_t *bbox_mask, int64_t *sem_cls, int64_t *size_cls,
+                                              spacap_stream_t stream) {
+  return proposal_decode_fwd("spacap_proposal_decode_fwd_f32", net, agg_xyz, mean_size, mean_size_f64, B, K, NH, NS, NC, nt, center,
+                             heading_res, size_res, corners, bbox_mask, sem_cls, size_cls, nullptr, stream);
+}
+
+extern "C" int spacap_proposal_decode_fwd_mask_f32(const float *net, const float *agg_xyz, const float *mean_size,
+                                                   const double *mean_size_f64, int B, int K, int NH, int NS, int NC, float *nt,
+                                                   float *center, float *heading_res, float *size_res, double *corners,
+                                                   int64_t *bbox_mask, int64_t *sem_cls, int64_t *size_cls, uint8_t *bbox_mask_u8,
+                                                   spacap_stream_t stream) {
+  const char *what = "spacap_proposal_decode_fwd_mask_f32";
+  SPACAP_REQUIRE(bbox_mask_u8 != nullptr || B == 0, "%s: null pointer", what);
+  return proposal_decode_fwd(what, net, agg_xyz, mean_size, mean_size_f64, B, K, NH, NS, NC, nt, center, heading_res, size_res,
+                             corners, bbox_mask, sem_cls, size_cls, bbox_mask_u8, stream);
 }
 
 extern "C" int spacap_proposal_decode_bwd_f32(const float *g_nt, const float *g_center, const float *g_heading_res,
diff --git a/spacap3d_amd/detector.py b/spacap3d_amd/detector.py
--- a/spacap3d_amd/detector.py
+++ b/spacap3d_amd/detector.py
@@ -72,7 +72,9 @@
         self.fp2 = PointnetFPModule(mlp=[256 + 256, 256, 256])
 
     @staticmethod
-    def _break_up_pc(pc):
+    def _break_up_pc(pc, split=None):
+        if split is not None and split[0] is pc:
+            return split[1], split[2]
         xyz = pc[..., :3].contiguous()
         if pc.size(-1) <= 3:
             return xyz, None
@@ -105,7 +107,7 @@
         return levels
 
     def forward(self, data_dict):
-        xyz, features = self._break_up_pc(data_dict["point_clouds"])
+        xyz, features = self._break_up_pc(data_dict["point_clouds"], data_dict.get("_pc_split"))
         pyr = tuple(data_dict.get("fps_pyramid") or ())
         pyr = pyr + (None,) * (19 - len(pyr))
         if pyr[0] is None and xyz.is_cuda and self.overlap_sampling and not xyz.requires_grad:
diff --git a/spacap3d_amd/engine.py b/spacap3d_amd/engine.py
--- a/spacap3d_amd/engine.py
+++ b/spacap3d_amd/engine.py
@@ -18,6 +18,19 @@
         dev = torch.device("cuda", key[1])
         _STREAMS[key] = {r: torch.cuda.Stream(device=dev) for r in ("side", "capture", "comm", "wgrad", "relation")}
     return _STREAMS[key][role]
+
+
+def _cloud_xyz(pc, out=None):
+    if pc.is_cuda and pc.dim() == 3 and pc.dtype == torch.float32 and pc.is_contiguous() and pc.shape[-1] >= 3:
+        from . import _native as nv
+        if out is None:
+            out = torch.empty(pc.shape[0], pc.shape[1], 3, dtype=pc.dtype, device=pc.device)
+        nv.glue_batched([(nv.GLUE_COLS_32, out, pc, 0, 3, 0)], pc.device)
+        return out
+    if out is None:
+        return pc[..., :3].contiguous()
+    out.copy_(pc[..., :3], non_blocking=True)
+    return out
 
 
 class Trainer:
@@ -43,6 +56,7 @@
         self._capture_stream = None
         self.last_losses = {}
         self._bn_counters = None
+        self._head_bumped = False
         self._grad_slots = {}
         self.grad_scale = 1.0
         self._recapture = False
@@ -98,7 +112,7 @@
                 self._prefetch_graph_obj, self._prefetch_graph_key = g, key
                 self.side_stream.wait_stream(cur)
             with torch.cuda.stream(self.side_stream), torch.no_grad():
-                self._prefetch_in.copy_(pc[..., :3], non_blocking=True)
+                _cloud_xyz(pc, out=self._prefetch_in)
                 skew = int(self.prefetch_skew_us)
                 if skew > 0:
                     from ._native import check, lib
@@ -109,7 +123,7 @@
             next_data["_fps_prefetch"] = (self._prefetch_out, ev)
             return
         with torch.cuda.stream(self.side_stream), torch.no_grad():
-            pyr = fn(pc[..., :3].contiguous())
+            pyr = fn(_cloud_xyz(pc))
             ev = torch.cuda.Event()
             ev.record(self.side_stream)
         next_data["_fps_prefetch"] = (pyr, ev)
@@ -257,11 +271,11 @@
 
     def _core(self, data_dict, with_optimizer=True):
         pc = data_dict["point_clouds"]
+        self._head_bumped = False
         if pc.is_cuda:
-            from .attention import advance_rng
-            advance_rng(pc.device)
+            data_dict = self._step_head(data_dict, pc)
         self.bucket.zero()
-        if self._bn_counters is not None:
+        if self._bn_counters is not None and not pc.is_cuda:
             self._bn_counters.add_(1)
         self._overlap_armed = self._overlap_possible(pc)
         if pc.is_cuda and (self.fork_relation and self.use_relation and not self._overlap_armed) != getattr(self, "_fork_on", False):
@@ -309,6 +323,30 @@
                                                        "cap_loss", "relation_loss") if k in d and torch.is_tensor(d[k])}
         return d["loss"].detach()
 
+    def _step_head(self, data_dict, pc):
+        from . import _native as nv
+        from .attention import rng_state
+        from .optim import FlatAdam
+        jobs = [(nv.GLUE_ADD_I64, rng_state(pc.device), None, 1, 0, 0)]
+        if self._bn_counters is not None:
+            jobs.append((nv.GLUE_ADD_I64, self._bn_counters, None, 1, 0, 0))
+        if isinstance(self.optimizer, FlatAdam):
+            jobs.append((nv.GLUE_ADD_F32, self.optimizer.step_t, None, 1, 0, 0))
+            self._head_bumped = True
+        C = pc.shape[-1]
+        if pc.dim() == 3 and pc.dtype == torch.float32 and pc.is_contiguous() and not pc.requires_grad and C in (3, 4):
+            B, N = pc.shape[0], pc.shape[1]
+            xyz = torch.empty(B, N, 3, dtype=pc.dtype, device=pc.device)
+            jobs.append((nv.GLUE_COLS_32, xyz, pc, 0, 3, 0))
+            feats = None
+            if C == 4:
+                feats = torch.empty(B, 1, N, dtype=pc.dtype, device=pc.device)
+                jobs.append((nv.GLUE_COLS_32, feats, pc, 0, 1, 3))
+            data_dict = dict(data_dict)
+            data_dict["_pc_split"] = (pc, xyz, feats)
+        nv.glue_batched(jobs, pc.device)
+        return data_dict
+
     def _seed_grad(self, loss):
         one = getattr(self, "_one", None)
         if one is None or one.device != loss.device or one.dtype != loss.dtype or one.shape != loss.shape:
@@ -330,7 +368,7 @@
         scale = self.bucket.all_reduce(sources=sources, force_pack=self.split_optimizer or flat, average=not flat)
         self.grad_scale = scale
         if flat:
-            self.optimizer.step(grad_scale=scale)
+            self.optimizer.step(grad_scale=scale, bump=not self._head_bumped)
         else:
             self.optimizer.step()
 
@@ -409,7 +447,7 @@
         if multi or self.force_comm_wait:
             main.wait_stream(self._comm_stream)
         self.grad_scale = 1.0 / dist.get_world_size() if multi else 1.0
-        self.optimizer.step(grad_scale=self.grad_scale, skip_word=err)
+        self.optimizer.step(grad_scale=self.grad_scale, skip_word=err, bump=not self._head_bumped)
         self._err_host.copy_(err, non_blocking=True)
         self._err_event = torch.cuda.Event()
         self._err_event.record(main)
diff --git a/spacap3d_amd/ext.py b/spacap3d_amd/ext.py
--- a/spacap3d_amd/ext.py
+++ b/spacap3d_amd/ext.py
@@ -114,6 +114,32 @@
         out = torch.empty(B, m, 3, dtype=torch.float32, device=xyz.device)
         check(lib.spacap_gather_xyz_f32(xyz.data_ptr(), idx.data_ptr(), B, N, m, out.data_ptr(), _stream(xyz)), "gather_xyz")
     return out
+
+
+def gather_xyz_grad(grad_out, idx, n):
+    _chk_contig(idx, "idx")
+    _chk_float(grad_out, "grad_out"); _chk_int(idx, "idx")
+    _chk_gpu(grad_out, "grad_out"); _chk_gpu(idx, "idx", grad_out)
+    B, m, _ = grad_out.shape
+    with torch.cuda.device(grad_out.device):
+        out = torch.empty(B, int(n), 3, dtype=torch.float32, device=grad_out.device)
+        check(lib.spacap_gather_xyz_grad_f32(grad_out.data_ptr(), *grad_out.stride(), idx.data_ptr(), B, int(n), m, out.data_ptr(),
+                                             _stream(grad_out)), "gather_xyz_grad")
+    return out
+
+
+class GatherXyz(torch.autograd.Function):
+
+    @staticmethod
+    def forward(ctx, xyz, idx):
+        ctx.save_for_backward(idx)
+        ctx.n = xyz.shape[1]
+        return gather_xyz(xyz, idx)
+
+    @staticmethod
+    def backward(ctx, g):
+        (idx,) = ctx.saved_tensors
+        return gather_xyz_grad(g, idx, ctx.n), None
 
 
 def three_interpolate(points, idx, weight):
diff --git a/spacap3d_amd/fused_losses.py b/spacap3d_amd/fused_losses.py
--- a/spacap3d_amd/fused_losses.py
+++ b/spacap3d_amd/fused_losses.py
@@ -29,13 +29,16 @@
             inv_den = torch.empty(4, **f32)
             args = [c(agg_xyz), c(gt_center[:, :, 0:3]), c(box_mask), c(heading_cls_label), c(heading_res_label),
                     c(size_cls_label), c(size_res_label), c(sem_cls_label), c(mean_size), c(seed_xyz)]
-            si, vl, vm = c(seed_inds.to(torch.int32)), c(vote_label), c(vote_mask)
-            check(lib.spacap_det_losses_fwd_f32(
-                net.data_ptr(), center.data_ptr(), *[a.data_ptr() for a in args], vote_xyz.data_ptr(), si.data_ptr(),
+            vl, vm = c(vote_label), c(vote_mask)
+            si = seed_inds.to(torch.int32)
+            if not (si.dim() == 2 and si.stride(1) == 1 and si.stride(0) >= NSEED):
+                si = c(si)
+            check(lib.spacap_det_losses_fwd_ld_f32(
+                net.data_ptr(), center.data_ptr(), *[a.data_ptr() for a in args], vote_xyz.data_ptr(), si.data_ptr(), si.stride(0),
                 vl.data_ptr(), vm.data_ptr(), B, K, M, NSEED, N, int(NH), int(NS), int(NC), float(near_thr), float(far_thr),
                 float(w0), float(w1), obj_label.data_ptr(), obj_mask.data_ptr(), assignment.data_ptr(), dnet_n.data_ptr(),
                 dcen_n.data_ptr(), dvote_n.data_ptr(), part.data_ptr(), losses.data_ptr(), inv_den.data_ptr(),
-                torch.cuda.current_stream(dev).cuda_stream), "spacap_det_losses_fwd_f32")
+                torch.cuda.current_stream(dev).cuda_stream), "spacap_det_losses_fwd_ld_f32")
         ctx.save_for_backward(dnet_n, dcen_n, dvote_n, inv_den)
         ctx.meta = (B, K, NSEED, int(NH), int(NS), int(NC))
         ctx.mark_non_differentiable(obj_label, obj_mask, assignment)
@@ -120,7 +123,7 @@
         B, W, V = logits.shape
         ids = lang_ids.contiguous()
         assert ids.dtype == torch.int64 and ids.shape[0] == B and ids.shape[1] >= W + 1
-        g8 = good.to(torch.uint8).contiguous()
+        g8 = good.contiguous().view(torch.uint8) if good.dtype == torch.bool else good.to(torch.uint8).contiguous()
         dev = logits.device
         with torch.cuda.device(dev):
             logp = torch.empty_like(logits)
@@ -170,16 +173,17 @@
             hres, sres = torch.empty(B, K, NH, **f32), torch.empty(B, K, NS, 3, **f32)
             corners = torch.empty(B, K, 8, 3, dtype=torch.float64, device=dev)
             bm, sem, sc = torch.empty(B, K, **i64), torch.empty(B, K, **i64), torch.empty(B, K, **i64)
-            check(lib.spacap_proposal_decode_fwd_f32(net.data_ptr(), agg.data_ptr(), msa.data_ptr(),
-                                                     mean_size_f64.contiguous().data_ptr() if mean_size_f64 is not None else None, B, K, int(NH), int(NS), int(NC),
-                                                     nt.data_ptr(), center.data_ptr(), hres.data_ptr(), sres.data_ptr(),
-                                                     corners.data_ptr(), bm.data_ptr(), sem.data_ptr(), sc.data_ptr(),
-                                                     torch.cuda.current_stream(dev).cuda_stream), "spacap_proposal_decode_fwd_f32")
+            bm8 = torch.empty(B, K, dtype=torch.uint8, device=dev)
+            check(lib.spacap_proposal_decode_fwd_mask_f32(net.data_ptr(), agg.data_ptr(), msa.data_ptr(),
+                                                          mean_size_f64.contiguous().data_ptr() if mean_size_f64 is not None else None, B, K, int(NH), int(NS), int(NC),
+                                                          nt.data_ptr(), center.data_ptr(), hres.data_ptr(), sres.data_ptr(),
+                                                          corners.data_ptr(), bm.data_ptr(), sem.data_ptr(), sc.data_ptr(), bm8.data_ptr(),
+                                                          torch.cuda.current_stream(dev).cuda_stream), "spacap_proposal_decode_fwd_mask_f32")
         ctx.save_for_backward(msa)
         ctx.meta = (B, K, CH, int(NH), int(NS), int(NC))
-        ctx.mark_non_differentiable(corners, bm, sem, sc)
-        ctx.set_materialize_grads(False)
-        return nt, center, hres, sres, corners, bm, sem, sc
+        ctx.mark_non_differentiable(corners, bm, sem, sc, bm8)
+        ctx.set_materialize_grads(False)
+        return nt, center, hres, sres, corners, bm, sem, sc, bm8
 
     @staticmethod
     def backward(ctx, g_nt, g_center, g_hres, g_sres, *_):
@@ -198,7 +202,9 @@
 
 
 def proposal_decode(net, agg_xyz, mean_size, mean_size_f64, NH, NS):
-    return ProposalDecode.apply(net, agg_xyz, mean_size, mean_size_f64, NH, NS)
+    out = ProposalDecode.apply(net, agg_xyz, mean_size, mean_size_f64, NH, NS)
+    out[5]._spacap_u8 = out[8]
+    return out[:8]
 
 
 class LossTail(Function):
diff --git a/spacap3d_amd/linear.py b/spacap3d_amd/linear.py
--- a/spacap3d_amd/linear.py
+++ b/spacap3d_amd/linear.py
@@ -204,20 +204,24 @@
 
     @staticmethod
     def backward(ctx, g):
+        return Conv1x1._backward(ctx, g, ctx.needs_input_grad)
+
+    @staticmethod
+    def _backward(ctx, g, needs):
         x, weight = ctx.saved_tensors
         B, CI = x.shape[0], x.shape[1]
         CO = weight.shape[0]
         N = x.numel() // (B * CI)
         g = g.contiguous()
         dx = None
-        if ctx.needs_input_grad[0]:
+        if needs[0]:
             dx = conv1x1_cm(1, weight, g, None, CI)
             if dx is None:
                 dx = torch.ops.aten.convolution_backward(g, x, weight, None, [1] * (x.dim() - 2), [0] * (x.dim() - 2),
                                                          [1] * (x.dim() - 2), False, [0] * (x.dim() - 2), 1,
                                                          [True, False, False])[0]
-        if not ctx.needs_input_grad[1]:
-            db = g.sum(dim=[0] + list(range(2, g.dim()))) if (ctx.has_bias and ctx.needs_input_grad[2]) else None
+        if not needs[1]:
+            db = g.sum(dim=[0] + list(range(2, g.dim()))) if (ctx.has_bias and needs[2]) else None
             return dx, None, db
         if int(lib.spacap_conv1x1_wgrad_slabs(B, CO, CI, N)):
             part = conv1x1_wgrad_partials(g, x, B, CO, CI, N, deferrable=True, with_bias=ctx.has_bias)
@@ -231,6 +235,41 @@
                                                      [False, True, False])[1]
         db = g.sum(dim=[0] + list(range(2, g.dim()))) if ctx.has_bias else None
         return dx, dw, db
+
+
+class Conv1x1AddPM(Function):
+
+    @staticmethod
+    def forward(ctx, x, weight, bias, res):
+        ctx.save_for_backward(x, weight)
+        ctx.has_bias = bias is not None
+        B, CI, N = x.shape
+        CO = weight.shape[0]
+        with torch.cuda.device(x.device):
+            out = torch.empty(B, N, CO, dtype=torch.float32, device=x.device)
+            check(lib.spacap_conv1x1_cm_pm_f32(2 if CONV_FWD_EXACT_F32 else 0, weight.data_ptr(), x.data_ptr(),
+                                               bias.data_ptr() if bias is not None else None, res.data_ptr(), B, CI, CO, N,
+                                               out.data_ptr(), torch.cuda.current_stream(x.device).cuda_stream),
+                  "spacap_conv1x1_cm_pm_f32")
+        return out
+
+    @staticmethod
+    def backward(ctx, g):
+        dx, dw, db = Conv1x1._backward(ctx, g.transpose(1, 2), ctx.needs_input_grad)
+        return dx, dw, db, g
+
+
+def conv1x1_add_pm(x, conv, res):
+    if not (x.is_cuda and x.dtype == torch.float32 and x.dim() == 3 and x.is_contiguous() and res.is_contiguous()
+            and res.dtype == torch.float32 and isinstance(conv, torch.nn.Conv1d) and conv.kernel_size == (1,)
+            and conv.weight.is_contiguous() and torch.is_grad_enabled()):
+        return None
+    B, CI, N = x.shape
+    CO = conv.out_channels
+    if res.shape != (B, N, CO) or not lib.spacap_conv1x1_cm_supported(CI, CO, N) or x.data_ptr() % 16 or res.data_ptr() % 16 \
+            or int(lib.spacap_conv1x1_wgrad_slabs(B, CO, CI, N)) == 0:
+        return None
+    return Conv1x1AddPM.apply(x, conv.weight, conv.bias, res)
 
 
 CONV_FWD_EXACT_F32 = False
diff --git a/spacap3d_amd/optim.py b/spacap3d_amd/optim.py
--- a/spacap3d_amd/optim.py
+++ b/spacap3d_amd/optim.py
@@ -21,9 +21,10 @@
         self.step_t = torch.zeros((), dtype=torch.float32, device=flat_g.device)
 
     @torch.no_grad()
-    def step(self, grad_scale=1.0, skip_word=None):
+    def step(self, grad_scale=1.0, skip_word=None, bump=True):
         dev = self.flat_p.device
-        self.step_t += 1
+        if bump:
+            self.step_t += 1
         with torch.cuda.device(dev):
             check(lib.spacap_adam_flat_f32(self.flat_p.data_ptr(), self.bucket.flat.data_ptr(), self.m.data_ptr(),
                                            self.v.data_ptr(), self.flat_p.numel(), self.lr, self.betas[0], self.betas[1],
diff --git a/spacap3d_amd/pointnet2_modules.py b/spacap3d_amd/pointnet2_modules.py
--- a/spacap3d_amd/pointnet2_modules.py
+++ b/spacap3d_amd/pointnet2_modules.py
@@ -93,6 +93,9 @@
             if not xyz.requires_grad and inds.dtype == torch.int32:
                 from . import ext
                 new_xyz = ext.gather_xyz(xyz.contiguous(), inds.contiguous())
+            elif inds.dtype == torch.int32 and xyz.dtype == torch.float32:
+                from . import ext
+                new_xyz = ext.GatherXyz.apply(xyz.contiguous(), inds.contiguous())
             else:
                 new_xyz = torch.gather(xyz, 1, inds.long().unsqueeze(-1).expand(-1, -1, 3))
         else:
diff --git a/spacap3d_amd/transformer_captioner.py b/spacap3d_amd/transformer_captioner.py
--- a/spacap3d_amd/transformer_captioner.py
+++ b/spacap3d_amd/transformer_captioner.py
@@ -231,7 +231,12 @@
             def c(m, v):
                 y = conv(v, m) if conv is not None else None
                 return m(v) if y is None else y
-            t = c(h[3], ops().bn_relu_train(c(h[0], t), h[1]))
+            u = ops().bn_relu_train(c(h[0], t), h[1])
+            fused = getattr(ops(), "conv1x1_add_pm", None)
+            y = fused(u, h[3], x) if fused is not None else None
+            if y is not None:
+                return y
+            t = c(h[3], u)
         elif t.is_cuda and not torch.is_grad_enabled() and getattr(ops(), "conv1x1", None) is not None:
             conv = ops().conv1x1
 
@@ -443,6 +448,9 @@
         src_pos = self._src_pos(ep)
         prep = getattr(ops(), "caption_prep", None) if (src.is_cuda and self.early_guide and self.model.encoder is not None) else None
         src_mask = ep["bbox_mask"].unsqueeze(1)
+        bm8 = getattr(ep["bbox_mask"], "_spacap_u8", None)
+        if bm8 is not None:
+            src_mask._spacap_u8 = bm8.unsqueeze(1)
         x0 = out_full = None
         if prep is not None:
             memory = self.model.encode(src, src_pos, src_mask)
```

After: 1170 scenes/s (median of 6 runs). About the same (+0.4%).
